# intel/pailliercryptolib

Measured on AMD Instinct MI355X. Metric: 2048-bit modexps/sec (encrypt+decrypt), higher is better.
Workload: dtype u64

## Files before the change

pailliercryptolib_amd/csrc/capi.cpp:

```cpp
#include "pgpu.h"

#include <hip/hip_runtime_api.h>

#include <algorithm>
#include <atomic>
#include <chrono>
#include <cstdio>
#include <cstdlib>
#include <cstring>
#include <deque>
#include <list>
#include <map>
#include <set>
#include <memory>
#include <mutex>
#include <string>
#include <vector>

#include "ipcl/bignum.h"
#include "kargs.hpp"
#include "launch.hpp"
#include "policy.hpp"
#include "runtime.hpp"

// ... 328 lines not shown
    const char* e = std::getenv("PGPU_FB_WINDOW");
    int v = e ? std::atoi(e) : kFbDefaultW;
    g_fb_window.store((v < 0 || v > kFbMaxW) ? kFbDefaultW : v);
    if (e) g_fb_window_explicit.store(true);
  }
  return g_fb_window.load();
}
int masked_fb_window() {
  static const int w = [] {
    const char* e = std::getenv("PGPU_FB_MASKED_WINDOW");
    return e ? std::max(1, std::min(kFbMaskedMaxW, std::atoi(e))) : 4;
  }();
  return w;
}
constexpr size_t kFbGrowAfter = 4096;

std::atomic<bool> g_timing{false};
struct TimerScope {
  rt::Device& d;
  hipStream_t s;
  bool on;
  rt::TimedLaunch t{};
  TimerScope(rt::Device& dev, hipStream_t st, int kind, int form = 0) : d(dev), s(st), on(g_timing.load()) {
    if (!on) return;
    t.kind = kind;
    t.form = form;
    t.stream = st;
    t.e0 = d.pool_event();
    t.e1 = d.pool_event();
    (void)hipEventRecord(t.e0, s);
  }
  void set_form(int form) { t.form = form; }
  void stop() {
    if (!on) return;
    (void)hipEventRecord(t.e1, s);
    std::lock_guard<std::mutex> lk(d.mu);
    if (d.timed.size() < 65536) d.timed.push_back(t);
  }
};

size_t modexp_waves(size_t count, int parity_waves, int ipw) {
  return parity_waves ? 2 * ((count / 2 + ipw - 1) / ipw) : (count + ipw - 1) / ipw;
}
unsigned blocks_for(size_t count, const GeoInfo& g) {
  return (unsigned)((count + (size_t)g.ipw() * pgpu::kWavesPerWG - 1) / ((size_t)g.ipw() * pgpu::kWavesPerWG));
}

GeoInfo latency_geo(const GeoInfo& geo) {
  static const bool allow = [] { const char* e = std::getenv("PGPU_LATENCY_GEO"); return !e || std::atoi(e) != 0; }();
  if (!allow) return geo;
  if (geo.G == 8 && geo.K == 9) return GeoInfo{16, 5};
  if (geo.G == 8 && geo.K == 14) return GeoInfo{16, 7};
  return geo;
}
bool use_latency_geo(const GeoInfo& lat, const GeoInfo& geo, size_t instances) {
  return lat.G != geo.G && (instances + lat.ipw() - 1) / lat.ipw() <= kSimds;
}

constexpr size_t kMinWavesForWide = 256 * 4;
GeoInfo launch_geo(const GeoInfo& geo, size_t count) {
  static const bool allow = [] { const char* e = std::getenv("PGPU_WIDE"); return !e || std::atoi(e) != 0; }();
  if (!allow || geo.K != 9 || geo.G < 4) return geo;
  GeoInfo wide{geo.G / 2, 18};
  size_t waves = (count + wide.ipw() - 1) / wide.ipw();
  static const size_t min_waves = [] {
    const char* e = std::getenv("PGPU_WIDE_MIN_WAVES");
    return e && std::atol(e) > 0 ? (size_t)std::atol(e) : kMinWavesForWide;
  }();
  return waves >= min_waves ? wide : geo;
}

std::atomic<int> g_row_source{-2};
bool use_regrows(const GeoInfo& geo, size_t waves) {
  int mode = g_row_source.load();
  if (mode == -2) {
    const char* e = std::getenv("PGPU_REGROWS");
    mode = e ? (std::atoi(e) != 0 ? 1 : 0) : -1;
    g_row_source.store(mode);
  }
  if (!pgpu::modexp_has_regrows(geo.G, geo.K)) return false;
  if (mode >= 0) return mode != 0;
  return waves <= kSimds;
}

uint64_t* g_wave_clocks = nullptr;

std::atomic<bool> g_packed_decrypt{[] {
  const char* e = std::getenv("PGPU_PACKED_DECRYPT");
  return !(e && std::atoi(e) == 0);
}()};
std::atomic<int> g_ct_gather{[] {
  const char* e = std::getenv("PGPU_CT_GATHER");
  return e && std::atoi(e) != 0 ? 1 : 0;
}()};
bool pair_rows_enabled() {
  static const bool on = [] {
    const char* e = std::getenv("PGPU_PAIR_ROWS");
    return !(e && std::atoi(e) == 0);
  }();
  return on;
}
std::atomic<int> g_hensel{-2};
bool hensel_enabled() {
  int mode = g_hensel.load();
  if (mode == -2) {
    const char* e = std::getenv("PGPU_HENSEL");
    mode = (e && std::atoi(e) == 0) ? 0 : 1;
    g_hensel.store(mode);
  }
  return mode != 0;
}

struct SchedRef {
  const uint16_t* p[2] = {nullptr, nullptr};
  int len[2] = {0, 0};
  int w = 0;
};
int run_modexp(rt::Device& d, pgpu::ModexpArgs& a, const GeoInfo& ctx_geo, hipStream_t s,
               const SchedRef* sched = nullptr, rt::StreamWork* held = nullptr) {
  const GeoInfo geo = launch_geo(ctx_geo, a.count);
  size_t entries;
  a.parity_waves = 0;
  if (sched && sched->p[0]) {
    a.parity_waves = a.nctx == 2;
    a.window = sched->w;
    for (int i = 0; i < 2; ++i) {
      a.sched[i] = sched->p[a.nctx == 2 ? i : 0];
      a.sched_len[i] = sched->len[a.nctx == 2 ? i : 0];
    }
    entries = (size_t)1 << (a.window - 1);
  } else {
    a.window = pick_window(a.exp_bits);
    entries = (size_t)1 << a.window;
  }
  const size_t waves = modexp_waves(a.count, a.parity_waves, geo.ipw());
  const size_t padded = (waves + pgpu::kWavesPerWG - 1) / pgpu::kWavesPerWG * pgpu::kWavesPerWG * geo.ipw();
  rt::StreamWork& w = held ? *held : d.work_for(s);
  std::unique_lock<std::mutex> lk(w.mu, std::defer_lock);
  if (!held) lk.lock();
  RC_TRY(w.table.ensure(padded * (entries + 1) * geo.L() * sizeof(uint32_t), s));
  a.table = (uint32_t*)w.table.p;
  a.wave_clocks = g_wave_clocks;
  TimerScope t(d, s, PGPU_KERNEL_MODEXP);
  const unsigned blocks = (unsigned)((waves + pgpu::kWavesPerWG - 1) / pgpu::kWavesPerWG);
  if (!pgpu::launch_modexp(geo.G, geo.K, use_regrows(geo, waves), a, blocks, s))
    return fail(PGPU_ERR_UNSUPPORTED, "modexp kernel geometry not compiled");
  HIP_TRY(hipGetLastError());
  t.stop();
  return PGPU_OK;
}

}

struct FbTable {
  void* p = nullptr;
  int w = 0, nwin = 0;
  hipEvent_t ready = nullptr;
  size_t bytes = 0;
  uint64_t tick = 0;
  int pins = 0;
  double build_ms = 0;
  hipEvent_t t0 = nullptr;
};
struct pgpu_pubkey {
  int n_words = 0;
  BigNumber n;
  bool djn = false;
  std::shared_ptr<ModCtx> nsq;
  rt::Replicated d_hs;
  rt::Replicated d_n;
  ExpSchedule sched_n;
  mutable std::mutex mu;
  mutable std::vector<std::list<FbTable>> fb;
  mutable size_t fb_elems = 0;
  struct PubForm {
    int H = 0, K = 0, chunk_words = 0, nchunks = 0;
    int n_words = 0;
    BigNumber n;
    rt::Replicated pub;
    rt::Replicated full;
    uint32_t n0inv = 0, n0inv_full = 0;
  };
  std::vector<std::shared_ptr<PubForm>> hforms;
  mutable std::vector<std::list<FbTable>> fbh;
  uint64_t gen = 0;
  ~pgpu_pubkey();
};

struct pgpu_privkey {
  uint64_t gen = 0;
  int n_words = 0;
  int pq_words = 0;
  GeoInfo geo_exp{};
  GeoInfo geo_crt{};
  std::shared_ptr<ModCtx> p2, q2;
  GeoInfo geo_lat{};
  std::shared_ptr<ModCtx> p2l, q2l;
  std::shared_ptr<ModCtx> cM, cQ;
  rt::Replicated d_exps;
  int exp_bits = 0;
  ExpSchedule sched[2];
  rt::Replicated d_crt32;
  rt::Replicated d_crt64;
  int nsq_rbits = 0;
  struct HenselSet {
    int H = 0, K = 0;
    int chunk_words = 0, nchunks = 0;
    rt::Replicated blob;
    uint32_t n0inv[2] = {0, 0};
    int pair_l2 = 0, pchunk_limbs = 0, pchunks = 0;
    int lb = pgpu::kLimbBits;
    size_t side_words() const { return (size_t)H * K * (6 + 4 * (size_t)nchunks + 3 * (size_t)pchunks); }
  };
  std::vector<std::unique_ptr<HenselSet>> hs;
  std::unique_ptr<HenselSet> hs_ps;
  std::shared_ptr<pgpu_pubkey::PubForm> conv_form;
};

struct pgpu_batch {
  size_t count = 0;
  int words = 0;
  int ndev = 1;
  bool replicated = false;
  std::vector<rt::DevMem> shard;
  std::shared_ptr<ModCtx> mont;
  int pair_l2 = 0;
  std::shared_ptr<const pgpu_pubkey::PubForm> pair_form;
  const uint32_t* prow(int d) const { return (const uint32_t*)shard[(size_t)d].p; }
  uint32_t* prow(int d) { return (uint32_t*)shard[(size_t)d].p; }
  uint64_t gen = 0;
  int lane = 0;
  uint64_t* ptr(int d) const { return (uint64_t*)shard[(size_t)d].p; }
  void bounds(int d, size_t* lo, size_t* hi) const {
    if (replicated) { *lo = 0; *hi = count; }
    else rt::shard_bounds(count, ndev, d, lo, hi);
  }
  struct XLane {
    hipEvent_t ready = nullptr;
    hipEvent_t reader[rt::kBatchLanes] = {};
  };
  mutable std::mutex xmu;
  mutable std::vector<XLane> xlane;
  ~pgpu_batch();
};

namespace {

std::atomic<int> g_next_thread_lane{0};
thread_local int t_batch_lane = -1;
thread_local bool t_lane_explicit = false;
std::atomic<int> g_host_adapt{[] { const char* e = std::getenv("PGPU_HOST_ADAPT"); return e && std::atoi(e) != 0 ? 1 : 0; }()};
bool host_adapt() { return g_host_adapt.load() != 0; }
int thread_batch_lane() {
  if (t_batch_lane < 0) t_batch_lane = g_next_thread_lane.fetch_add(1) % rt::kBatchLanes;
  return t_batch_lane;
}
int new_batch(size_t count, int words, std::unique_ptr<pgpu_batch>* out, int pair_l2 = 0, int lane = -1) {
  if (count == 0 || words <= 0) return fail(PGPU_ERR_INVALID_PARAM, "batch needs count > 0 and words > 0");
  std::unique_ptr<pgpu_batch> b(new pgpu_batch);
  b->count = count;
  b->words = words;
  b->gen = rt::pool_generation();
  b->lane = lane < 0 ? thread_batch_lane() : (lane % rt::kBatchLanes);
  b->replicated = count == 1 && rt::pool_size() > 1;
  b->ndev = b->replicated ? rt::pool_size() : rt::shard_devices(count);
  b->shard.resize((size_t)b->ndev);
  for (int d = 0; d < b->ndev; ++d) {
    size_t lo, hi;
    b->bounds(d, &lo, &hi);
    rt::Device& dev = rt::device(d);
    RC_TRY(b->shard[(size_t)d].alloc(dev, dev.bs(b->lane), (hi - lo) * (size_t)(pair_l2 ? pair_l2 : words) * 8));
  }
  b->pair_l2 = pair_l2;
  *out = std::move(b);
  return PGPU_OK;
}

bool same_domain(const std::shared_ptr<ModCtx>& batch_ctx, const std::shared_ptr<ModCtx>& key_ctx) {
  if (!batch_ctx || batch_ctx == key_ctx) return true;
  return batch_ctx->geo.L() == key_ctx->geo.L() && batch_ctx->geo.G == key_ctx->geo.G && batch_ctx->N == key_ctx->N;
}

int same_layout(const pgpu_batch* a, const pgpu_batch* b) {
  if (b->count == 1 && a->count != 1) return PGPU_OK;
  if (a->ndev != b->ndev || a->replicated != b->replicated)
    return fail(PGPU_ERR_INVALID_PARAM, "batches were sharded differently (pgpu_set_min_shard changed in between)");
  return PGPU_OK;
}

int lane_acquire(rt::Device& dev, const pgpu_batch* x, int lane) {
  if (!x || x->lane == lane) return PGPU_OK;
  hipEvent_t ready;
  {
    std::lock_guard<std::mutex> lk(x->xmu);
    if (x->xlane.size() < (size_t)rt::pool_size()) x->xlane.resize((size_t)rt::pool_size());
    pgpu_batch::XLane& xl = x->xlane[(size_t)dev.index];
    if (!xl.ready) {
      HIP_TRY(hipEventCreateWithFlags(&xl.ready, hipEventDisableTiming));
      HIP_TRY(hipEventRecord(xl.ready, dev.bs(x->lane)));
    }
    ready = xl.ready;
  }
  HIP_TRY(hipStreamWaitEvent(dev.bs(lane), ready, 0));
  return PGPU_OK;
}
int lane_release(rt::Device& dev, const pgpu_batch* x, int lane) {
  if (!x || x->lane == lane) return PGPU_OK;
  std::lock_guard<std::mutex> lk(x->xmu);
  if (x->xlane.size() < (size_t)rt::pool_size()) x->xlane.resize((size_t)rt::pool_size());
// ... 180 lines not shown
  a.chunk_words = f->chunk_words;
  a.nchunks = f->nchunks;
  a.exp = d_exp;
  a.exp_stride = exp_stride;
  a.exp_words = exp_words;
  a.exp_bits = exp_bits;
  size_t entries;
  if (sched && sched->p[0]) {
    a.sched = sched->p[0];
    a.sched_len = sched->len[0];
    a.window = sched->w;
    entries = (size_t)1 << (a.window - 1);
  } else {
    a.window = pick_window(exp_bits);
    entries = (size_t)1 << a.window;
  }
  a.final_mul = pgpu::FM_UNIT;
  a.ct_gather = (sched && sched->p[0]) ? 0 : g_ct_gather.load();
  a.out = d_out;
  a.out_stride = (size_t)sq.mod_words;
  a.count = count;
  const size_t ipw = 64 / (2 * (size_t)f->H);
  const size_t waves = (count + ipw - 1) / ipw;
  const unsigned blocks = (unsigned)((waves + pgpu::kWavesPerWG - 1) / pgpu::kWavesPerWG);
  rt::StreamWork& w = d.work_for(s);
  std::lock_guard<std::mutex> lk(w.mu);
  RC_TRY(w.table.ensure((size_t)blocks * pgpu::kWavesPerWG * ipw * entries * 2 * L2 * sizeof(uint32_t), s));
  a.table = (uint32_t*)w.table.p;
  TimerScope t(d, s, PGPU_KERNEL_MODEXP, PGPU_FORM_PAIRED);
  if (!pgpu::launch_hensel_modexp(f->H, f->K, a, blocks, s)) return fail(PGPU_ERR_UNSUPPORTED, "split-form modexp kernel not compiled");
  HIP_TRY(hipGetLastError());
  t.stop();
  return PGPU_OK;
}

int modexp_on(rt::Device& d, const uint64_t* d_base, size_t base_stride, const uint64_t* d_exp, size_t exp_stride,
              int exp_words, int exp_bits, const uint64_t* h_mod, int mod_words, uint64_t* d_out, size_t count,
              hipStream_t s, const SchedRef* sched, bool in_mont, bool out_mont, std::shared_ptr<ModCtx> ctx_in,
              size_t total_count = 0) {
  std::shared_ptr<ModCtx> ctx = ctx_in;
  if (!in_mont && !out_mont) {
    std::shared_ptr<SquareCtx> sq;
    RC_TRY(get_square_ctx(h_mod, mod_words, &sq));
    if (sq)
      return modexp_square_on(d, *sq, d_base, base_stride, d_exp, exp_stride, exp_words, exp_bits, d_out, count, s, sched,
                              std::max(count, total_count));
  }
  if (!ctx) RC_TRY(get_modctx(h_mod, mod_words, true, &ctx));
  GeoInfo run_geo = ctx->geo;
  const GeoInfo lat = latency_geo(ctx->geo);
  if (!in_mont && !out_mont && use_latency_geo(lat, ctx->geo, count)) {
    if (lat.L() != ctx->geo.L()) {
      std::vector<uint64_t> mw((size_t)mod_words);
      ctx->N.toLimbs64(mw.data(), mw.size());
      RC_TRY(get_modctx(mw.data(), mod_words, true, &ctx, true));
    }
    run_geo = lat;
  }
  pgpu::ModexpArgs a{};
  a.ctx[0] = a.ctx[1] = ctx->view(d.index, (in_mont ? VF_IN_MONT : 0) | (out_mont ? VF_OUT_MONT : 0));
  a.nctx = 1;
  a.base = d_base;
  a.base_stride = base_stride;
  a.base_words = mod_words;
  a.exp = d_exp;
  a.exp_stride = exp_stride;
  a.exp_per_ctx = 0;
  a.exp_words = exp_words;
  a.exp_bits = exp_bits;
  a.final_mul = out_mont ? pgpu::FM_CTX_CONST : pgpu::FM_UNIT;
  a.out = d_out;
  a.out_stride = (size_t)mod_words;
  a.count = count;
  return run_modexp(d, a, run_geo, s, sched);
}

std::mutex g_fb_mu;
std::set<const pgpu_pubkey*> g_fb_keys;
std::vector<size_t> g_fb_dev_bytes;
std::atomic<size_t> g_fb_dev_max{0}, g_fb_key_max{0};
std::atomic<uint64_t> g_fb_tick{0}, g_fb_evictions{0};
size_t fb_dev_max() {
  size_t v = g_fb_dev_max.load();
  if (v == 0) {
    const char* e = std::getenv("PGPU_FB_MAX_BYTES");
    v = e && std::atoll(e) > 0 ? (size_t)std::atoll(e) : (size_t)2 << 30;
    g_fb_dev_max.store(v);
  }
  return v;
}
size_t fb_key_max() {
  size_t v = g_fb_key_max.load();
  if (v == 0) {
    const char* e = std::getenv("PGPU_FB_KEY_MAX_BYTES");
    v = e && std::atoll(e) > 0 ? (size_t)std::atoll(e) : (size_t)512 << 20;
    g_fb_key_max.store(v);
  }
  return v;
}
size_t fb_table_bytes(int r_bits, int w, size_t entry_bytes) {
  return (size_t)std::max(1, (r_bits + w - 1) / w) * ((size_t)1 << w) * entry_bytes;
}
int fb_fit_window(int w_cfg, int r_bits, size_t entry_bytes) {
  int w = w_cfg;
  const size_t cap = std::min(fb_key_max(), fb_dev_max());
  while (w > 1 && fb_table_bytes(r_bits, w, entry_bytes) > cap) --w;
  return w;
}
void fb_free_table(FbTable& t) {
  if (t.ready) (void)hipEventDestroy(t.ready);
  if (t.t0) (void)hipEventDestroy(t.t0);
  if (t.p) (void)hipFree(t.p);
  t.p = nullptr;
}
void fb_make_room(int dev, size_t need) {
  if (g_fb_dev_bytes.size() <= (size_t)dev) g_fb_dev_bytes.resize((size_t)dev + 1, 0);
  while (g_fb_dev_bytes[(size_t)dev] + need > fb_dev_max()) {
    std::list<FbTable>* vlist = nullptr;
    std::list<FbTable>::iterator victim;
    for (const pgpu_pubkey* k : g_fb_keys)
      for (auto* lists : {&k->fb, &k->fbh}) {
        if (lists->size() <= (size_t)dev) continue;
        auto& l = (*lists)[(size_t)dev];
        for (auto it = l.begin(); it != l.end(); ++it)
          if (it->pins == 0 && (!vlist || it->tick < victim->tick)) {
            vlist = &l;
            victim = it;
          }
      }
    if (!vlist) return;
    g_fb_dev_bytes[(size_t)dev] -= std::min(g_fb_dev_bytes[(size_t)dev], victim->bytes);
    fb_free_table(*victim);
    vlist->erase(victim);
    g_fb_evictions.fetch_add(1);
  }
}
struct FbPin {
  FbTable* t = nullptr;
  FbPin() = default;
  FbPin(const FbPin&) = delete;
  FbPin& operator=(const FbPin&) = delete;
  ~FbPin() { release(); }
  void release() {
    if (!t) return;
    std::lock_guard<std::mutex> lk(g_fb_mu);
    --t->pins;
    t = nullptr;
  }
  const FbTable* operator->() const { return t; }
};

template <class Build>
int fb_table_get(const pgpu_pubkey* key, std::vector<std::list<FbTable>>& lists, rt::Device& d, int w, int nwin,
                 size_t entry_bytes, hipStream_t s, FbPin* out, Build build) {
  std::lock_guard<std::mutex> lk(g_fb_mu);
  if (lists.size() < (size_t)rt::pool_size()) lists.resize((size_t)rt::pool_size());
  auto& list = lists[(size_t)d.index];
  for (FbTable& t : list)
    if (t.w == w && t.nwin >= nwin) {
      HIP_TRY(hipStreamWaitEvent(s, t.ready, 0));
      t.tick = g_fb_tick.fetch_add(1) + 1;
      ++t.pins;
      out->t = &t;
      return PGPU_OK;
    }
  for (auto it = list.begin(); it != list.end();) {
    if (it->pins == 0 && (it->w <= kFbMaskedMaxW) == (w <= kFbMaskedMaxW)) {
      g_fb_dev_bytes.resize(std::max(g_fb_dev_bytes.size(), (size_t)d.index + 1), 0);
      g_fb_dev_bytes[(size_t)d.index] -= std::min(g_fb_dev_bytes[(size_t)d.index], it->bytes);
      fb_free_table(*it);
      it = list.erase(it);
    } else {
      ++it;
    }
  }
  FbTable t;
  t.w = w;
  t.nwin = nwin;
  t.bytes = (size_t)nwin * ((size_t)1 << w) * entry_bytes;
  fb_make_room(d.index, t.bytes);
  hipError_t e = hipMalloc(&t.p, t.bytes);
  if (e != hipSuccess) return fail(PGPU_ERR_HIP, std::string("fixed-base table: ") + hipGetErrorString(e));
  if (hipEventCreateWithFlags(&t.ready, hipEventDefault) != hipSuccess || hipEventCreateWithFlags(&t.t0, hipEventDefault) != hipSuccess) {
    fb_free_table(t);
    return fail(PGPU_ERR_HIP, "fixed-base table: event creation failed");
  }
  (void)hipEventRecord(t.t0, s);
  int rc = build(t);
  if (rc == PGPU_OK && hipGetLastError() != hipSuccess) rc = fail(PGPU_ERR_HIP, "fixed-base build launch failed");
  if (rc == PGPU_OK && hipEventRecord(t.ready, s) != hipSuccess) rc = fail(PGPU_ERR_HIP, "fixed-base table: event record failed");
  if (rc != PGPU_OK) {
    fb_free_table(t);
    return rc;
  }
  t.tick = g_fb_tick.fetch_add(1) + 1;
  t.pins = 1;
  g_fb_dev_bytes.resize(std::max(g_fb_dev_bytes.size(), (size_t)d.index + 1), 0);
  g_fb_dev_bytes[(size_t)d.index] += t.bytes;
  g_fb_keys.insert(key);
  list.push_back(t);
  out->t = &list.back();
  return PGPU_OK;
}

int fb_table_for(const pgpu_pubkey* key, rt::Device& d, int w, int nwin, hipStream_t s, FbPin* out) {
  const GeoInfo& geo = key->nsq->geo;
  return fb_table_get(key, key->fb, d, w, nwin, (size_t)geo.L() * sizeof(uint32_t), s, out, [&](FbTable& t) -> int {
    pgpu::FixedBaseBuildArgs b{};
    b.ctx = key->nsq->view(d.index);
    b.base = (const uint64_t*)key->d_hs.d[(size_t)d.index];
    b.table = (uint32_t*)t.p;
    b.nwin = nwin;
    b.w = w;
    if (!pgpu::launch_fb_build(geo.G, geo.K, b, blocks_for((size_t)nwin, geo), s))
      return fail(PGPU_ERR_UNSUPPORTED, "fixed-base build kernel geometry not compiled");
    return PGPU_OK;
  });
}

const pgpu_pubkey::PubForm* use_split_encrypt(const pgpu_pubkey* key, int m_words, size_t count) {
  if (key->hforms.empty() || !hensel_enabled() || 64 * m_words > key->n.BitSize()) return nullptr;
  const pgpu_pubkey::PubForm* f = key->hforms.back().get();
  if (!pgpu::hensel_fb_has(f->H, f->K)) return nullptr;
  if (g_hensel.load() >= 2) return f;
  const GeoInfo g = launch_geo(key->nsq->geo, count);
  const size_t ipw = 64 / (2 * (size_t)f->H);
  return (g.G <= 2 * f->H || (count + ipw - 1) / ipw >= kSimds) ? f : nullptr;
}
pgpu::HenselPubDev hensel_pub_view(const pgpu_pubkey::PubForm* f, int dev, bool base_mont = false) {
  const int L2 = f->H * f->K;
  const uint32_t* b = (const uint32_t*)f->pub.d[(size_t)dev];
  pgpu::HenselPubDev v{};
  v.nhat = b;
  v.n = b + L2;
  v.kr = b + 2 * L2;
  v.one = b + 3 * L2;
  v.conv = b + 5 * L2 + (base_mont ? (size_t)f->nchunks * 2 * L2 : 0);
  v.gm = b + (size_t)L2 * (5 + 4 * (size_t)f->nchunks);
  v.n0inv = f->n0inv;
  return v;
}
const pgpu_pubkey::PubForm* pair_form(const pgpu_pubkey* key) {
  if (key->hforms.empty() || !hensel_enabled() || !pair_rows_enabled()) return nullptr;
  const pgpu_pubkey::PubForm* f = key->hforms.back().get();
  return pgpu::pair_ops_has(f->H, f->K) ? f : nullptr;
}
int pair_l2(const pgpu_pubkey* key) {
  const pgpu_pubkey::PubForm* f = pair_form(key);
  return f ? f->H * f->K : 0;
}
std::shared_ptr<const pgpu_pubkey::PubForm> pair_form_shared(const pgpu_pubkey* key) {
  return pair_form(key) ? key->hforms.back() : nullptr;
}
pgpu::HenselFullDev hensel_full_view(const pgpu_pubkey* , const pgpu_pubkey::PubForm* f, int dev, bool out_mont) {
  const size_t LF = (size_t)2 * f->H * f->K;
  const uint32_t* b = (const uint32_t*)f->full.d[(size_t)dev];
  pgpu::HenselFullDev v{};
  v.n = b;
  v.nr = out_mont ? b + 2 * LF : b + LF;
  v.r2 = out_mont ? b + 3 * LF : nullptr;
  v.n0inv = f->n0inv_full;
  v.mod_words = 2 * f->n_words;
  return v;
}

const pgpu_pubkey::PubForm* split_modexp_form(const pgpu_pubkey* key, size_t count) {
  if (key->hforms.empty() || !hensel_enabled()) return nullptr;
  static const size_t max_waves = [] {
    const char* e = std::getenv("PGPU_SPLIT_MODEXP_MAX_WAVES");
    return e && std::atol(e) > 0 ? (size_t)std::atol(e) : ~(size_t)0;
  }();
  const pgpu_pubkey::PubForm* last = nullptr;
  for (const auto& f : key->hforms) {
    if (!pgpu::hensel_modexp_has(f->H, f->K)) continue;
    last = f.get();
    const size_t ipw = 64 / (2 * (size_t)f->H);
    if ((count + ipw - 1) / ipw <= kSimds) return last;
  }
  if (!last) return nullptr;
  const size_t ipw = 64 / (2 * (size_t)last->H);
  return (count + ipw - 1) / ipw > max_waves ? nullptr : last;
}
int wave_neighbours(rt::Device& dev, hipStream_t s) {
  int lane = -1;
  for (int k = 0; k < rt::kBatchLanes; ++k)
    if (dev.bs(k) == s) lane = k;
  if (lane < 0) return 0;
  static const int64_t window_ns = [] {
    const char* e = std::getenv("PGPU_LANE_ACTIVE_MS");
    return (int64_t)(e ? std::max(0, std::atoi(e)) : 50) * 1000000;
  }();
  const int64_t now = std::chrono::duration_cast<std::chrono::nanoseconds>(std::chrono::steady_clock::now().time_since_epoch()).count();
  dev.lane_fed_ns[lane].store(now, std::memory_order_relaxed);
  int busy = 0;
  for (int k = 0; k < rt::kBatchLanes; ++k) {
    if (k == lane) continue;
    const int64_t fed = std::max(dev.lane_fed_ns[k].load(std::memory_order_relaxed), dev.host_fed_ns[k].load(std::memory_order_relaxed));
    if ((fed != 0 && now - fed < window_ns) || hipStreamQuery(dev.bs(k)) == hipErrorNotReady) ++busy;
  }
  (void)hipGetLastError();
  return busy;
}
bool wave_n2_applies(const pgpu_pubkey::PubForm* form, size_t count) {
  const int L2 = form->H * form->K;
  return hensel_enabled() && pair_rows_enabled() && pgpu::hensel_modexp_wave_has(L2) && policy::modexp_wave_form_pays(count) &&
         pgpu::kLimbBits * L2 - (form->n.BitSize() + pgpu::kLimbBits) >= 10;
}
int modexp_split_on(rt::Device& d, const pgpu_pubkey* key, const pgpu_pubkey::PubForm* form, const uint64_t* d_base, size_t base_stride,
                    int base_words, bool base_mont, const uint64_t* d_exp, size_t exp_stride, int exp_words,
                    int exp_bits, const SchedRef* sched, int final_mul, const uint64_t* d_m, size_t m_stride,
                    int m_words, uint64_t* d_out, bool out_mont, size_t count, hipStream_t s,
                    const uint32_t* base_pair = nullptr, size_t base_pair_stride = 0, uint32_t* out_pair = nullptr) {
  const int H = form->H, K = form->K;
  pgpu::HenselModexpArgs a{};
  a.base_pair = base_pair;
  a.base_pair_stride = base_pair_stride;
  a.out_pair = out_pair;
  a.ctx = hensel_pub_view(form, d.index, base_mont);
  a.full = hensel_full_view(key, form, d.index, out_mont);
  a.base = d_base;
  a.base_stride = base_stride;
  a.base_words = base_words;
  a.chunk_words = form->chunk_words;
  a.nchunks = (base_words + form->chunk_words - 1) / form->chunk_words;
  a.exp = d_exp;
  a.exp_stride = exp_stride;
  a.exp_words = exp_words;
  a.exp_bits = exp_bits;
  size_t entries;
  if (sched && sched->p[0]) {
    a.sched = sched->p[0];
    a.sched_len = sched->len[0];
    a.window = sched->w;
    entries = (size_t)1 << (a.window - 1);
  } else {
    a.window = pick_window(exp_bits);
    entries = (size_t)1 << a.window;
  }
  a.final_mul = final_mul;
  a.ct_gather = (sched && sched->p[0]) ? 0 : g_ct_gather.load();
  a.fm_words = d_m;
  a.fm_stride = m_stride;
  a.fm_nwords = m_words;
  a.out = d_out;
  a.out_stride = (size_t)2 * key->n_words;
  a.count = count;
  if (base_pair && out_pair && !a.sched && final_mul == pgpu::FM_UNIT && wave_n2_applies(form, count) && a.window <= 5 &&
      (policy::wave_policy() == 2 || count * (size_t)(1 + wave_neighbours(d, s)) <= kSimds)) {
    TimerScope t(d, s, PGPU_KERNEL_MODEXP, PGPU_FORM_WAVE);
    if (!pgpu::launch_hensel_modexp_wave(H * K, a, s))
      return fail(PGPU_ERR_UNSUPPORTED, "wavefront-wide modexp kernel not compiled");
    HIP_TRY(hipGetLastError());
    t.stop();
    return PGPU_OK;
  }
  const bool seq = modexp_seq_form_pays(H, K, count) && base_pair && out_pair && !a.sched && final_mul == pgpu::FM_UNIT;
  const size_t ipw = seq ? 64 / (size_t)H : 64 / (2 * (size_t)H);
  const size_t waves = (count + ipw - 1) / ipw;
  const unsigned blocks = (unsigned)((waves + pgpu::kWavesPerWG - 1) / pgpu::kWavesPerWG);
  rt::StreamWork& w = d.work_for(s);
  std::lock_guard<std::mutex> lk(w.mu);
  RC_TRY(w.table.ensure((size_t)blocks * pgpu::kWavesPerWG * ipw * entries * 2 * H * K * sizeof(uint32_t), s));
  a.table = (uint32_t*)w.table.p;
  TimerScope t(d, s, PGPU_KERNEL_MODEXP, seq ? PGPU_FORM_SEQ : PGPU_FORM_PAIRED);
  if (seq) {
    if (!pgpu::launch_hensel_modexp_seq(H, K, a, blocks, s))
      return fail(PGPU_ERR_UNSUPPORTED, "sequential-halves modexp kernel not compiled");
  } else if (!pgpu::launch_hensel_modexp(H, K, a, blocks, s)) return fail(PGPU_ERR_UNSUPPORTED, "split-form modexp kernel not compiled");
  HIP_TRY(hipGetLastError());
  t.stop();
  return PGPU_OK;
}
int fb_table_for_split(const pgpu_pubkey* key, const pgpu_pubkey::PubForm* form, rt::Device& d, int w, int nwin,
                       hipStream_t s, FbPin* out) {
  const int H = form->H, K = form->K;
  return fb_table_get(key, key->fbh, d, w, nwin, (size_t)2 * H * K * sizeof(uint32_t), s, out, [&](FbTable& t) -> int {
    pgpu::HenselFbBuildArgs b{};
    b.ctx = hensel_pub_view(form, d.index);
    b.base = (const uint64_t*)key->d_hs.d[(size_t)d.index];
    b.base_words = 2 * key->n_words;
    b.chunk_words = form->chunk_words;
    b.nchunks = form->nchunks;
    b.table = (uint32_t*)t.p;
    b.nwin = nwin;
    b.w = w;
    const int ipw = 64 / (2 * H);
    const unsigned blocks = (unsigned)((((size_t)nwin + ipw - 1) / ipw + pgpu::kWavesPerWG - 1) / pgpu::kWavesPerWG);
    if (!pgpu::launch_hensel_fb_build(H, K, b, blocks, s))
      return fail(PGPU_ERR_UNSUPPORTED, "split-form fixed-base build kernel not compiled");
    return PGPU_OK;
  });
}

int encrypt_on(rt::Device& d, const pgpu_pubkey* key, const uint64_t* d_m, size_t m_stride, int m_words,
               const uint64_t* d_r, size_t r_stride, int r_words, int r_bits, uint64_t* d_c, size_t count,
               hipStream_t s, bool out_mont, size_t total_count, uint32_t* d_pair = nullptr, int busy_lanes = 0) {
  const int W = 2 * key->n_words;
  if (m_words <= 0 || m_words > W || m_stride < (size_t)m_words)
    return fail(PGPU_ERR_INVALID_PARAM, "plaintext width/stride invalid");
  if (r_words <= 0 || r_stride < (size_t)r_words)
    return fail(PGPU_ERR_INVALID_PARAM, "random width/stride invalid");
  if (key->djn && (r_bits < 0 || r_bits > 64 * r_words))
    return fail(PGPU_ERR_INVALID_PARAM, "r_bits/r_words inconsistent");
  const int vflags = out_mont ? VF_GM_MONT : VF_NONE;
  int fbw = fixed_base_window();
  const bool masked = key->djn && fbw > 0 && g_ct_gather.load() != 0;
  if (masked) fbw = masked_fb_window();
  if (key->djn && fbw > 0) {
    if (!masked) {
      std::lock_guard<std::mutex> lk(key->mu);
      if (fbw > 8 && !g_fb_window_explicit.load() && key->fb_elems + total_count < kFbGrowAfter) fbw = 8;
    }
    const GeoInfo& geo = key->nsq->geo;
    const pgpu_pubkey::PubForm* sform = d_pair ? pair_form(key) : use_split_encrypt(key, m_words, count);
    fbw = fb_fit_window(fbw, r_bits, sform ? (size_t)2 * sform->H * sform->K * sizeof(uint32_t) : (size_t)geo.L() * sizeof(uint32_t));
    const int nwin = std::max(1, (r_bits + fbw - 1) / fbw);
    FbPin tab;
    if (const pgpu_pubkey::PubForm* form = sform) {
      RC_TRY(fb_table_for_split(key, form, d, fbw, nwin, s, &tab));
      if (d_pair) {
        for (const auto& alt : key->hforms) {
          const size_t ipw_alt = 64 / (2 * (size_t)alt->H);
          if (alt->H * alt->K == form->H * form->K && alt->H > form->H && pgpu::hensel_fb_encrypt_has(alt->H, alt->K) &&
              (total_count + ipw_alt - 1) / ipw_alt <= kSimds) {
            form = alt.get();
            break;
          }
        }
      }
      pgpu::HenselFbArgs f{};
      f.ctx = hensel_pub_view(form, d.index);
      f.full = hensel_full_view(key, form, d.index, out_mont);
      f.table = (const uint32_t*)tab->p;
      f.nwin = nwin;
      f.w = fbw;
      f.exp = d_r;
      f.exp_stride = r_stride;
      f.exp_words = r_words;
      f.fm_words = d_m;
      f.fm_stride = m_stride;
      f.fm_nwords = m_words;
      f.out = d_c;
      f.out_stride = (size_t)W;
      f.count = count;
      f.out_pair = d_pair;
      f.ct_gather = masked ? 1 : 0;
      TimerScope t(d, s, PGPU_KERNEL_FB_ENCRYPT);
      if (d_pair && busy_lanes == 0 && wave_n2_applies(form, count) &&
          (policy::wave_policy() == 2 || count * (size_t)(1 + wave_neighbours(d, s)) <= kSimds)) {
        t.set_form(PGPU_FORM_WAVE);
        if (!pgpu::launch_hensel_fb_encrypt_wave(form->H * form->K, f, s))
          return fail(PGPU_ERR_UNSUPPORTED, "wavefront-wide fixed-base kernel not compiled");
        HIP_TRY(hipGetLastError());
        t.stop();
        return PGPU_OK;
      }
      const bool seq = d_pair && fb_encrypt_seq_pays(form->H, form->K, count, busy_lanes);
      t.set_form(seq ? PGPU_FORM_SEQ : PGPU_FORM_PAIRED);
      const int ipw = seq ? 64 / form->H : 64 / (2 * form->H);
      const unsigned blocks = (unsigned)(((count + ipw - 1) / ipw + pgpu::kWavesPerWG - 1) / pgpu::kWavesPerWG);
      if (seq) {
        const size_t seq_waves = (count + ipw - 1) / ipw;
        unsigned lds_pad = adaptive_cu_claim(seq_waves, busy_lanes);
        if (lds_pad && busy_lanes >= 3) lds_pad = pgpu::kLdsTotalFlag | 80000u;
        if (lds_pad) t.set_form(PGPU_FORM_SEQ | PGPU_FORM_CU_CLAIM);
        if (!pgpu::launch_hensel_fb_encrypt_seq(form->H, form->K, f, blocks, s, lds_pad))
          return fail(PGPU_ERR_UNSUPPORTED, "sequential-halves fixed-base kernel not compiled");
      } else if (!pgpu::launch_hensel_fb_encrypt(form->H, form->K, f, blocks, s))
        return fail(PGPU_ERR_UNSUPPORTED, "split-form fixed-base kernel not compiled");
      HIP_TRY(hipGetLastError());
      t.stop();
      return PGPU_OK;
    }
    RC_TRY(fb_table_for(key, d, fbw, nwin, s, &tab));
    pgpu::FixedBaseArgs f{};
    f.ctx = key->nsq->view(d.index, vflags);
    f.table = (const uint32_t*)tab->p;
    f.nwin = nwin;
    f.w = fbw;
    f.exp = d_r;
    f.exp_stride = r_stride;
    f.exp_words = r_words;
    f.fm_words = d_m;
    f.fm_stride = m_stride;
    f.fm_nwords = m_words;
    f.out = d_c;
    f.out_stride = (size_t)W;
    f.count = count;
    f.ct_gather = masked ? 1 : 0;
    TimerScope t(d, s, PGPU_KERNEL_FB_ENCRYPT);
    const GeoInfo lgeo = launch_geo(geo, count);
    if (!pgpu::launch_fb_encrypt(lgeo.G, lgeo.K, f, blocks_for(count, lgeo), s))
      return fail(PGPU_ERR_UNSUPPORTED, "fixed-base kernel geometry not compiled");
    HIP_TRY(hipGetLastError());
    t.stop();
    return PGPU_OK;
  }
  pgpu::ModexpArgs a{};
  a.ctx[0] = a.ctx[1] = key->nsq->view(d.index, vflags);
  a.nctx = 1;
  if (key->djn) {
    a.base = (const uint64_t*)key->d_hs.d[(size_t)d.index];
    a.base_stride = 0;
    a.base_words = W;
    a.exp = d_r;
    a.exp_stride = r_stride;
    a.exp_words = r_words;
    a.exp_bits = r_bits;
  } else {
    if (r_words > W) return fail(PGPU_ERR_INVALID_PARAM, "random wider than n^2");
    const pgpu_pubkey::PubForm* form = d_pair ? pair_form(key)
                                       : (64 * m_words <= key->n.BitSize() ? split_modexp_form(key, count) : nullptr);
    if (form) {
      SchedRef srn;
      if (key->sched_n.dev.bytes) {
        srn.p[0] = (const uint16_t*)key->sched_n.dev.d[(size_t)d.index];
        srn.len[0] = key->sched_n.len;
        srn.w = key->sched_n.w;
      }
      return modexp_split_on(d, key, form, d_r, r_stride, r_words, false,
                             (const uint64_t*)key->d_n.d[(size_t)d.index], 0, key->n_words, key->n.BitSize(),
                             srn.p[0] ? &srn : nullptr, pgpu::FM_PAILLIER_G, d_m, m_stride, m_words, d_c, out_mont,
                             count, s, nullptr, 0, d_pair);
    }
    a.base = d_r;
    a.base_stride = r_stride;
    a.base_words = r_words;
    a.exp = (const uint64_t*)key->d_n.d[(size_t)d.index];
    a.exp_stride = 0;
    a.exp_words = key->n_words;
    a.exp_bits = key->n.BitSize();
  }
  if (d_pair) return fail(PGPU_ERR_UNSUPPORTED, "pair-row output needs a split-form encrypt kernel");
  a.exp_per_ctx = 0;
  a.final_mul = pgpu::FM_PAILLIER_G;
  a.fm_words = d_m;
  a.fm_stride = m_stride;
  a.fm_nwords = m_words;
  a.out = d_c;
  a.out_stride = (size_t)W;
  a.count = count;
  SchedRef sr;
  if (!key->djn && key->sched_n.dev.bytes) {
    sr.p[0] = (const uint16_t*)key->sched_n.dev.d[(size_t)d.index];
    sr.len[0] = key->sched_n.len;
    sr.w = key->sched_n.w;
  }
  return run_modexp(d, a, key->nsq->geo, s, sr.p[0] ? &sr : nullptr);
}

const pgpu_privkey::HenselSet* pick_hensel(const pgpu_privkey* key, size_t count) {
  if (!hensel_enabled() || key->hs.empty()) return nullptr;
  const int mode = g_hensel.load();
  if (mode == 2) return key->hs.back().get();
  if (mode == 3) return key->hs.front().get();
  for (const auto& f : key->hs) {
    const size_t ipw = 64 / (2 * (size_t)f->H);
    if (2 * ((count + ipw - 1) / ipw) <= kSimds) return f.get();
  }
  return key->hs.back().get();
}

int busy_other_lanes(rt::Device& dev, int lane, bool force = false, size_t count = (size_t)-1) {
  const int rr_min = (!force && !t_lane_explicit) ? policy::rr_adapt() : 1;
  if (rr_min <= 0) return 0;
  static const int64_t window_ns = [] {
    const char* e = std::getenv("PGPU_LANE_ACTIVE_MS");
    return (int64_t)(e ? std::max(0, std::atoi(e)) : 50) * 1000000;
  }();
  const int64_t now = std::chrono::duration_cast<std::chrono::nanoseconds>(std::chrono::steady_clock::now().time_since_epoch()).count();
  dev.lane_fed_ns[lane % rt::kBatchLanes].store(now, std::memory_order_relaxed);
  int busy = 0;
  for (int k = 0; k < rt::kBatchLanes; ++k) {
    if (k == lane) continue;
    const int64_t fed = dev.lane_fed_ns[k].load(std::memory_order_relaxed);
    if ((fed != 0 && now - fed < window_ns) || hipStreamQuery(dev.bs(k)) == hipErrorNotReady) ++busy;
  }
  (void)hipGetLastError();
  if (!force && !t_lane_explicit && count < policy::kRrAdaptMinCount) return 0;
  return busy >= rr_min ? busy : 0;
}
int host_busy(rt::Device& dev, int lane, size_t count = (size_t)-1) {
  if (host_adapt()) return busy_other_lanes(dev, lane, true);
  const int k = policy::rr_adapt();
  if (k <= 0) return 0;
  static const int64_t window_ns = [] {
    const char* e = std::getenv("PGPU_LANE_ACTIVE_MS");
    return (int64_t)(e ? std::max(0, std::atoi(e)) : 50) * 1000000;
  }();
  const int64_t now = std::chrono::duration_cast<std::chrono::nanoseconds>(std::chrono::steady_clock::now().time_since_epoch()).count();
  dev.host_fed_ns[lane % rt::kBatchLanes].store(now, std::memory_order_relaxed);
  int busy = 0;
  for (int j = 0; j < rt::kBatchLanes; ++j) {
    if (j == lane % rt::kBatchLanes) continue;
    const int64_t fed = std::max(dev.host_fed_ns[j].load(std::memory_order_relaxed), dev.lane_fed_ns[j].load(std::memory_order_relaxed));
    if (fed != 0 && now - fed < window_ns) ++busy;
  }
  if (count < policy::kRrAdaptMinCount) return 0;
  return busy >= k ? busy : 0;
}

bool ps_form_pays(const pgpu_privkey* key, size_t count, int busy) {
  return key->hs_ps && hensel_enabled() && policy::ps_form_pays(count, busy, key->hs_ps->K);
}
bool wave_form_pays(const pgpu_privkey* key, size_t count, int busy) {
  return key->hs_ps && hensel_enabled() && pgpu::hensel_wave_has(key->hs_ps->K, key->hs_ps->lb) && policy::wave_form_pays(count, busy);
}
int words_to_pair_on(rt::Device& d, const pgpu_pubkey::PubForm* f, const uint64_t* words, size_t stride, int nwords,
                     bool src_mont, uint32_t* out, size_t count, hipStream_t s);
int decrypt_on(rt::Device& d, const pgpu_privkey* key, const uint64_t* d_c, uint64_t* d_m, size_t count,
               hipStream_t s, bool in_mont, const uint32_t* d_pair = nullptr, int in_pair_l2 = 0, int busy_lanes = 0) {
  const int nw = key->n_words;
  if (busy_lanes == 0 && key->hs_ps && hensel_enabled() && secret_policy() != PGPU_EXP_SLIDING &&
      (d_pair ? key->hs_ps->pair_l2 == in_pair_l2 : key->conv_form != nullptr)) {
    if (const size_t head = policy::ps_split_head(key->hs_ps->K, count)) {
      RC_TRY(decrypt_on(d, key, d_c, d_m, head, s, in_mont, d_pair, in_pair_l2, busy_lanes));
      return decrypt_on(d, key, d_c ? d_c + head * (size_t)2 * nw : nullptr, d_m + head * (size_t)nw, count - head, s, in_mont,
                        d_pair ? d_pair + head * (size_t)2 * in_pair_l2 : nullptr, in_pair_l2, busy_lanes);
    }
  }
  rt::StreamWork& w = d.work_for(s);
  std::lock_guard<std::mutex> lk(w.mu);
  RC_TRY(w.vbuf.ensure(2 * count * (size_t)nw * 8, s));
  const bool lat = use_latency_geo(key->geo_lat, key->geo_exp, 2 * count);
  const bool sliding = secret_policy() == PGPU_EXP_SLIDING && key->sched[0].dev.bytes;
  bool have_m = false;
  const pgpu_privkey::HenselSet* hset = pick_hensel(key, count);
// ... 917 lines not shown
```

pailliercryptolib_amd/csrc/hensel.hpp:

```cpp
#ifndef PAILLIERCRYPTOLIB_AMD_CSRC_HENSEL_HPP_
#define PAILLIERCRYPTOLIB_AMD_CSRC_HENSEL_HPP_

#include "kernels.hpp"

namespace pgpu {

template <int H, int K>
__device__ __forceinline__ void pair_row_source(uint32_t (&src)[K], const uint32_t (&v)[K]) {
#pragma unroll
  for (int j = 0; j < K; ++j) {
    if constexpr (H == 4)
      src[j] = (uint32_t)__builtin_amdgcn_update_dpp((int)v[j], (int)v[j], 0x114 , 0xf, 0xa, false);
    else
      src[j] = v[j];
  }
}
template <int H, int S>
__device__ __forceinline__ uint32_t pair_row(uint32_t src) {
  if constexpr (H == 8) return bcast_lane<16, S>(src);
  else return bcast_lane<4, S>(src);
}

template <int H, int K, bool SQR, bool UNITQ, int S>
__device__ __forceinline__ void pair_block(uint64_t (&LOWC)[K], uint64_t (&UPC)[K], const uint32_t (&mc)[K],
                                           const uint32_t (&md)[K], const uint32_t (&csrc)[K],
                                           const uint32_t (&asrc)[K], const uint32_t (&n)[K], uint32_t n0inv,
                                           uint32_t selB) {
  using GEO = Geo<H, K>;
  uint32_t crow[K];
#pragma unroll
  for (int r = 0; r < K; ++r) crow[r] = pair_row<H, S>(csrc[r]);
#pragma unroll
  for (int r = 0; r < K; ++r) {
#pragma unroll
    for (int j = 0; j < K; ++j) {
      const uint64_t p = (uint64_t)mc[j] * crow[r];
      if (r + j < K) LOWC[r + j] += p;
      else UPC[r + j - K] += p;
    }
  }
  if constexpr (!SQR) {
    uint32_t arow[K];
#pragma unroll
    for (int r = 0; r < K; ++r) arow[r] = pair_row<H, S>(asrc[r]);
#pragma unroll
    for (int r = 0; r < K; ++r) {
#pragma unroll
      for (int j = 0; j < K; ++j) {
        const uint64_t p = (uint64_t)md[j] * arow[r];
        if (r + j < K) LOWC[r + j] += p;
        else UPC[r + j - K] += p;
      }
    }
  }
  mont_reduce_rows<GEO, UNITQ, true, true>(LOWC, UPC, n, n0inv, selB);
}

template <int H, int K, bool SQR, bool UNITQ, int S>
__device__ __forceinline__ void pair_blocks(uint64_t (&c0)[K], uint64_t (&c1)[K], const uint32_t (&mc)[K],
                                            const uint32_t (&md)[K], const uint32_t (&csrc)[K],
                                            const uint32_t (&asrc)[K], const uint32_t (&n)[K], uint32_t n0inv,
                                            uint32_t selB) {
  if constexpr (S < H) {
    pair_block<H, K, SQR, UNITQ, S>(c0, c1, mc, md, csrc, asrc, n, n0inv, selB);
    pair_block<H, K, SQR, UNITQ, S + 1>(c1, c0, mc, md, csrc, asrc, n, n0inv, selB);
    pair_blocks<H, K, SQR, UNITQ, S + 2>(c0, c1, mc, md, csrc, asrc, n, n0inv, selB);
  }
}
template <int H, int K, bool SQR, bool UNITQ>
__device__ __forceinline__ void pairmul(uint32_t (&r)[K], const uint32_t (&own)[K], const uint32_t (&m)[K],
                                        const uint32_t (&n)[K], uint32_t n0inv, uint32_t halfB, uint32_t selB) {
  static_assert(3 * K + 6 < 64, "a column of half B receives 3K products (+ relaxed limbs): must stay below 2^64");
  static_assert(H == 2 || H == 4 || H == 8, "two halves inside one 16-lane DPP row");
  using GEO = Geo<H, K>;
  uint64_t c0[K], c1[K];
  uint32_t mc[K], md[K], csrc[K], asrc[K];
  const uint32_t maskB = 0u - halfB;
  pair_row_source<H, K>(asrc, own);
  if constexpr (!SQR) pair_row_source<H, K>(csrc, m);
#pragma unroll
  for (int j = 0; j < K; ++j) {
    c0[j] = 0;
    c1[j] = 0;
    mc[j] = SQR ? own[j] << halfB : own[j];
    md[j] = SQR ? 0 : m[j] & maskB;
  }
  if constexpr (SQR) pair_blocks<H, K, SQR, UNITQ, 0>(c0, c1, mc, md, asrc, asrc, n, n0inv, selB);
  else pair_blocks<H, K, SQR, UNITQ, 0>(c0, c1, mc, md, csrc, asrc, n, n0inv, selB);
  montmul_finish<GEO>(r, c0);
}

template <class GEO>
__device__ __forceinline__ uint32_t sub_limbs(uint32_t (&d)[GEO::K], const uint32_t (&r)[GEO::K],
                                              const uint32_t (&s)[GEO::K], int x, int lane) {
  constexpr int K = GEO::K, G = GEO::G;
  const int top_lane = (lane / G) * G + (G - 1);
  uint32_t b = 0;
#pragma unroll
  for (int j = 0; j < K; ++j) {
    uint32_t t = r[j] - s[j] - b;
    d[j] = t & kLimbMask;
    b = t >> 31;
  }
  uint32_t top_borrow = b;
  for (;;) {
    uint32_t bin = dpp_from_prev(b);
    if (x == 0) bin = 0;
    if (__ballot(bin != 0) == 0) break;
    b = bin;
#pragma unroll
    for (int j = 0; j < K; ++j) {
      uint32_t t = d[j] - b;
      d[j] = t & kLimbMask;
      b = t >> 31;
    }
    top_borrow |= b;
  }
  return (uint32_t)__shfl((int)top_borrow, top_lane);
}

template <int H, int K, int MINW = (K <= 14 ? 2 : 1)>
__global__ __launch_bounds__(kWGThreads, MINW) void hensel_decrypt_kernel(HenselArgs A) {
  using HG = Geo<H, K>;
  constexpr int GS = 2 * H, IPW = kWave / GS, L2 = H * K, LQ = 2 * H * K, W64 = HG::W64;
  raise_wave_priority();
  __shared__ uint32_t bl_[kWavesPerWG][IPW][L2];
  __shared__ uint64_t io_[kWavesPerWG][IPW][W64 + 1];
  const int lane = threadIdx.x % kWave, wv = threadIdx.x / kWave;
  auto& bl = bl_[wv];
  auto& io = io_[wv];
  const int grp = lane / GS, xg = lane % GS, x = xg % H;
  const uint32_t halfB = (uint32_t)(xg / H);
  uint32_t selB = xg == H ? 1u : 0u;
  asm("" : "+v"(selB));
  const size_t wave_id = (size_t)blockIdx.x * kWavesPerWG + wv;
  const int side = __builtin_amdgcn_readfirstlane((int)(wave_id & 1));
  const size_t first_elem = (wave_id >> 1) * IPW;
  size_t elem = first_elem + grp;
  if (elem >= A.count) elem = A.count - 1;
#define HCTX(field) (side ? A.ctx[1].field : A.ctx[0].field)

  uint32_t n[K], own[K], mreg[K];
#pragma unroll
  for (int j = 0; j < K; ++j) n[j] = HCTX(nhat)[x * K + j];
  uint32_t n0inv = 0;

  const bool sched_mode = A.sched[0] != nullptr;
  const uint16_t* sch = side ? A.sched[1] : A.sched[0];
  const int nsteps = side ? A.sched_len[1] : A.sched_len[0];
  const int w = A.window;
  const int tsize = sched_mode ? 1 << (w - 1) : 1 << w;
  uint32_t* tbl = A.table + (wave_id * IPW + grp) * (size_t)tsize * LQ + xg * K;
  const uint64_t* ep = A.exp + (size_t)side * A.exp_stride;
  const int nwin = (A.exp_bits + w - 1) / w;
  auto digit = [&](int i) -> int {
    int bit = i * w;
    int word = bit >> 6, sh = bit & 63;
    uint64_t v = (word < A.exp_words) ? ep[word] >> sh : 0;
    if (sh + w > 64 && word + 1 < A.exp_words) v |= ep[word + 1] << (64 - sh);
    return (int)(v & (uint64_t)(tsize - 1));
  };

  uint32_t acc[K];
#pragma unroll
  for (int j = 0; j < K; ++j) acc[j] = 0;
  if (A.ct_pair) {
    const uint32_t* row = A.ct_pair + elem * A.ct_pair_stride + (size_t)halfB * A.pair_l2;
    const uint32_t* pconv = HCTX(pconv);
    const uint32_t* pcb = HCTX(pcb);
    const int trips = A.pchunks + ((sched_mode && tsize > 1) ? 1 : 0);
#pragma unroll 1
    for (int i = 0; i < trips; ++i) {
      if (i < A.pchunks) {
        const int first = i * A.pchunk_limbs;
        uint32_t z[K], cb[K], tb[K];
#pragma unroll
        for (int j = 0; j < K; ++j) {
          const int li = x * K + j;
          z[j] = (li < A.pchunk_limbs && first + li < A.pair_l2) ? row[first + li] : 0u;
          cb[j] = pcb[(size_t)i * L2 + x * K + j];
          mreg[j] = pconv[(size_t)i * LQ + xg * K + j];
          own[j] = halfB ? 0u : z[j];
        }
        montmul_reg<HG, false, true>(tb, z, cb, n, 0);
        pairmul<H, K, false, true>(own, own, mreg, n, n0inv, halfB, selB);
#pragma unroll
        for (int j = 0; j < K; ++j) own[j] += halfB ? tb[j] : 0u;
        add_normalise<HG>(acc, own);
      } else {
#pragma unroll
        for (int j = 0; j < K; ++j) own[j] = mreg[j] = acc[j];
        pairmul<H, K, false, true>(own, own, mreg, n, n0inv, halfB, selB);
      }
    }
  } else {
    const uint64_t* row = A.ct + elem * A.ct_stride;
    const uint32_t* conv = HCTX(conv);
    const int trips = A.nchunks + ((sched_mode && tsize > 1) ? 1 : 0);
#pragma unroll 1
    for (int i = 0; i < trips; ++i) {
      if (i < A.nchunks) {
        wave_lds_sync();
        const int first = i * A.chunk_words;
        const int words = min(A.chunk_words, A.ct_words - first);
        for (int t = xg; t <= W64; t += GS) io[grp][t] = (t < words) ? row[first + t] : 0;
        wave_lds_sync();
#pragma unroll
        for (int j = 0; j < K; ++j) {
          own[j] = halfB ? 0u : limb_from_words(io[grp], x * K + j);
          mreg[j] = conv[(size_t)i * LQ + xg * K + j];
        }
      } else {
#pragma unroll
        for (int j = 0; j < K; ++j) own[j] = mreg[j] = acc[j];
      }
      pairmul<H, K, false, true>(own, own, mreg, n, n0inv, halfB, selB);
      if (i < A.nchunks) add_normalise<HG>(acc, own);
    }
  }

  {
    int e;
    if (sched_mode) {
#pragma unroll
      for (int j = 0; j < K; ++j) {
        tbl[j] = acc[j];
        mreg[j] = own[j];
        own[j] = acc[j];
      }
      e = 1;
    } else {
#pragma unroll
      for (int j = 0; j < K; ++j) {
        tbl[LQ + j] = acc[j];
        tbl[j] = HCTX(one)[xg * K + j];
        mreg[j] = own[j] = acc[j];
      }
      e = 2;
    }
#pragma unroll 1
    for (; e < tsize; ++e) {
      pairmul<H, K, false, true>(own, own, mreg, n, n0inv, halfB, selB);
#pragma unroll
      for (int j = 0; j < K; ++j) tbl[(size_t)e * LQ + j] = own[j];
    }
  }

  int win;
  bool any = true;
  if (sched_mode) {
    if (nsteps == 0) any = false;
    win = 1;
  } else {
    if (nwin == 0) any = false;
    win = nwin - 2;
  }
  if (any) {
    const int d0 = sched_mode ? (__builtin_amdgcn_readfirstlane((int)sch[0]) & 63) - 1 : digit(nwin - 1);
    load_table_entry<K>(own, tbl, d0, tsize, LQ, A.ct_gather != 0);
  } else {
#pragma unroll
    for (int j = 0; j < K; ++j) own[j] = HCTX(one)[xg * K + j];
  }
#ifndef PGPU_PHASE_PAD
#define PGPU_PHASE_PAD 0
#endif
  if constexpr ((PGPU_PHASE_PAD & 2) != 0) asm volatile(".p2align 6");
  if constexpr ((PGPU_PHASE_PAD & 1) != 0) asm volatile("s_nop 0");
#pragma unroll 1
  for (;;) {
    int nsq, idx;
    if (sched_mode) {
      if (!any || win >= nsteps) break;
      const int st = __builtin_amdgcn_readfirstlane((int)sch[win++]);
      nsq = st >> 6;
      idx = (st & 63) - 1;
    } else {
      if (!any || win < 0) break;
      nsq = w;
      idx = digit(win--);
    }
    const bool mul = !sched_mode || idx >= 0;
    if (mul) load_table_entry<K>(mreg, tbl, idx, tsize, LQ, A.ct_gather != 0);
#pragma unroll 1
    for (int i = 0; i < nsq; ++i) pairmul<H, K, true, true>(own, own, own, n, n0inv, halfB, selB);
    if (mul) pairmul<H, K, false, true>(own, own, mreg, n, n0inv, halfB, selB);
  }

  {
#pragma unroll
    for (int j = 0; j < K; ++j) {
      n[j] = HCTX(n)[x * K + j];
      mreg[j] = HCTX(kr)[x * K + j];
    }
    n0inv = HCTX(n0inv);
    uint32_t kb[K];
    montmul_reg<HG, false, false>(kb, own, mreg, n, n0inv);
#pragma unroll
    for (int j = 0; j < K; ++j) {
      if (halfB) own[j] = kb[j];
      mreg[j] = halfB ? 0u : HCTX(h)[x * K + j];
    }
    pairmul<H, K, false, false>(own, own, mreg, n, n0inv, halfB, selB);
  }
  full_normalise<HG>(own, x);
  uint32_t d[K];
  const uint32_t below = sub_limbs<HG>(d, own, n, x, lane);
  const uint32_t jflag = (uint32_t)__shfl((int)(below ^ 1u), (lane / GS) * GS);
  if (!below) {
#pragma unroll
    for (int j = 0; j < K; ++j) own[j] = d[j];
  }
  (void)sub_limbs<HG>(d, n, own, x, lane);
  if (x == 0) d[0] += jflag;
  full_normalise<HG>(d, x);
  const uint32_t small = sub_limbs<HG>(own, d, n, x, lane);
  if (small) {
#pragma unroll
    for (int j = 0; j < K; ++j) own[j] = d[j];
  }
  wave_lds_sync();
  if (halfB) {
#pragma unroll
    for (int j = 0; j < K; ++j) bl[grp][x * K + j] = own[j];
  }
  wave_lds_sync();
  const int ow = A.out_words;
  for (int t = lane; t < IPW * ow; t += kWave) {
    const int gg = t / ow, ww = t % ow;
    const size_t oe = first_elem + gg;
    if (oe < A.count) A.out[(2 * oe + side) * A.out_stride + ww] = ww < W64 ? word_from_limbs(bl[gg], L2, ww) : 0;
  }
#undef HCTX
}

template <int D>
__device__ __forceinline__ uint32_t dpp_from_above(uint32_t v) {
  return (uint32_t)__builtin_amdgcn_update_dpp(0, (int)v, 0x100 + D , 0xf, 0xf, true);
}

template <int K>
__device__ __forceinline__ void load_pair_row(uint32_t (&v)[K], const uint32_t* __restrict__ row, int xg) {
  const uint32_t* p = row + xg * K;
  if constexpr (K % 2 == 0) {
    const uint2* q = reinterpret_cast<const uint2*>(p);
#pragma unroll
    for (int j = 0; j < K / 2; ++j) {
      const uint2 t = q[j];
      v[2 * j] = t.x;
      v[2 * j + 1] = t.y;
    }
  } else {
#pragma unroll
    for (int j = 0; j < K; ++j) v[j] = p[j];
  }
}
template <int K>
__device__ __forceinline__ void store_pair_row(uint32_t* __restrict__ row, const uint32_t (&v)[K], int xg) {
  uint32_t* p = row + xg * K;
  if constexpr (K % 2 == 0) {
    uint2* q = reinterpret_cast<uint2*>(p);
#pragma unroll
    for (int j = 0; j < K / 2; ++j) q[j] = make_uint2(v[2 * j], v[2 * j + 1]);
  } else {
#pragma unroll
    for (int j = 0; j < K; ++j) p[j] = v[j];
  }
}

template <int H, int K>
__device__ __forceinline__ void pair_times_gm(uint32_t (&own)[K], const HenselPubDev& C, const uint64_t* mwords, int x,
                                              uint32_t halfB) {
  using HG = Geo<H, K>;
  uint32_t n[K], mv[K], cg[K], u[K], av[K], v[K];
#pragma unroll
  for (int j = 0; j < K; ++j) {
    n[j] = C.n[x * K + j];
    cg[j] = C.gm[x * K + j];
    mv[j] = limb_from_words(mwords, x * K + j);
  }
  montmul_reg<HG, false, false>(u, mv, cg, n, C.n0inv);
#pragma unroll
  for (int j = 0; j < K; ++j) {
    const uint32_t below = dpp_from_below<H>(own[j]);
    av[j] = halfB ? below : own[j];
  }
  montmul_reg<HG, false, false>(v, u, av, n, C.n0inv);
#pragma unroll
  for (int j = 0; j < K; ++j) v[j] = halfB ? v[j] : 0u;
  add_normalise<HG>(own, v);
}

template <int H, int K>
__device__ __forceinline__ void pair_from_words(uint32_t (&own)[K], const uint64_t* row, int nwords, int chunk_words,
                                                int nchunks, const uint32_t* conv, uint64_t* iorow,
                                                const uint32_t (&n)[K], uint32_t halfB, uint32_t selB, int xg) {
  using HG = Geo<H, K>;
  constexpr int GS = 2 * H, LQ = 2 * H * K, W64 = HG::W64;
  const int x = xg % H;
  uint32_t acc[K], mreg[K];
#pragma unroll
  for (int j = 0; j < K; ++j) acc[j] = 0;
#pragma unroll 1
  for (int i = 0; i < nchunks; ++i) {
    wave_lds_sync();
    const int first = i * chunk_words;
    const int words = min(chunk_words, nwords - first);
    for (int t = xg; t <= W64; t += GS) iorow[t] = (t < words) ? row[first + t] : 0;
    wave_lds_sync();
#pragma unroll
    for (int j = 0; j < K; ++j) {
      own[j] = halfB ? 0u : limb_from_words(iorow, x * K + j);
      mreg[j] = conv[(size_t)i * LQ + xg * K + j];
    }
    pairmul<H, K, false, true>(own, own, mreg, n, 0, halfB, selB);
    add_normalise<HG>(acc, own);
  }
#pragma unroll
  for (int j = 0; j < K; ++j) own[j] = acc[j];
}

template <int H, int K>
__device__ __forceinline__ void pair_exit_store(uint32_t (&own)[K], const HenselPubDev& C, const HenselFullDev& F,
                                                bool with_gm, const uint64_t* fm_words, size_t fm_stride, int fm_nwords,
                                                uint64_t* out, size_t out_stride, size_t first_inst, size_t count,
                                                uint32_t (*bl)[2 * H * K], uint64_t (*io)[Geo<2 * H, K>::W64 + 1],
                                                uint32_t (*rows)[2 * H * K], int lane, int grp, int xg, uint32_t halfB,
                                                uint32_t selB) {
  using HG = Geo<H, K>;
  using FG = Geo<2 * H, K>;
  constexpr int GS = 2 * H;
  const int x = xg % H;
  for (int t = lane; t < FG::L; t += kWave) {
    rows[0][t] = F.nr[t];
    rows[1][t] = F.r2 ? F.r2[t] : 0;
  }
  if (with_gm) stage_words<FG>(io, fm_words, fm_stride, 0, fm_nwords, first_inst, count, 1, lane);
  uint32_t n[K], mreg[K];
#pragma unroll
  for (int j = 0; j < K; ++j) {
    n[j] = C.n[x * K + j];
    mreg[j] = C.kr[x * K + j];
  }
  const uint32_t n0inv = C.n0inv;
  {
    uint32_t kb[K];
    montmul_reg<HG, false, false>(kb, own, mreg, n, n0inv);
#pragma unroll
    for (int j = 0; j < K; ++j)
      if (halfB) own[j] = kb[j];
  }
  wave_lds_sync();
  uint32_t d[K], e[K];
  if (with_gm) {
#pragma unroll
    for (int j = 0; j < K; ++j) {
      e[j] = limb_from_words(io[grp], x * K + j);
      d[j] = 2 * n[j];
    }
    full_normalise<HG>(d, x);
    (void)sub_limbs<HG>(mreg, d, e, x, lane);
  } else {
#pragma unroll
    for (int j = 0; j < K; ++j) mreg[j] = 0;
  }
#pragma unroll
  for (int j = 0; j < K; ++j)
    if (!halfB) mreg[j] = (xg == 0 && j == 0) ? 1u : 0u;
  pairmul<H, K, false, false>(own, own, mreg, n, n0inv, halfB, selB);
  full_normalise<HG>(own, x);
  const uint32_t below = sub_limbs<HG>(d, own, n, x, lane);
  const uint32_t jflag = (uint32_t)__shfl((int)(below ^ 1u), (lane / GS) * GS);
  if (!below) {
#pragma unroll
    for (int j = 0; j < K; ++j) own[j] = d[j];
  }
  (void)sub_limbs<HG>(d, n, own, x, lane);
  if (x == 0) d[0] += jflag;
  full_normalise<HG>(d, x);
  const uint32_t small = sub_limbs<HG>(e, d, n, x, lane);
  uint32_t X[K], Y[K], nf[K];
#pragma unroll
  for (int j = 0; j < K; ++j) {
    const uint32_t bc = small ? d[j] : e[j];
    const uint32_t down = dpp_from_above<H>(bc);
    X[j] = halfB ? 0u : own[j];
    Y[j] = halfB ? 0u : down;
    nf[j] = F.n[xg * K + j];
  }
  wave_lds_sync();
  uint32_t t[K];
  montmul<FG, false, false>(t, Y, rows[0], nf, F.n0inv);
  if (F.r2) {
    uint32_t u[K];
    montmul<FG, false, false>(u, X, rows[1], nf, F.n0inv);
    add_normalise<FG>(t, u);
  } else {
    add_normalise<FG>(t, X);
  }
  store_canonical<FG>(t, nf, F.mod_words, bl, io, out, out_stride, first_inst, count, lane, grp, xg);
}

template <int H, int K>
__global__ __launch_bounds__(kWGThreads, K <= 14 ? 2 : 1) void hensel_fb_build_kernel(HenselFbBuildArgs A) {
  using HG = Geo<H, K>;
  constexpr int GS = 2 * H, IPW = kWave / GS, LQ = 2 * H * K, W64 = HG::W64;
  __shared__ uint64_t io_[kWavesPerWG][IPW][W64 + 1];
  const int lane = threadIdx.x % kWave, wv = threadIdx.x / kWave;
  auto& io = io_[wv];
  const int grp = lane / GS, xg = lane % GS, x = xg % H;
  const uint32_t halfB = (uint32_t)(xg / H);
  uint32_t selB = xg == H ? 1u : 0u;
  asm("" : "+v"(selB));
  const size_t first_inst = ((size_t)blockIdx.x * kWavesPerWG + wv) * IPW;
  size_t inst = first_inst + grp;
  const bool live = inst < (size_t)A.nwin;
  if (!live) inst = (size_t)A.nwin - 1;
  uint32_t n[K], own[K], mreg[K];
#pragma unroll
  for (int j = 0; j < K; ++j) n[j] = A.ctx.nhat[x * K + j];
  pair_from_words<H, K>(own, A.base, A.base_words, A.chunk_words, A.nchunks, A.ctx.conv, io[grp], n, halfB, selB, xg);
  const int tsize = 1 << A.w;
  const int my_sq = A.w * (int)inst;
  size_t last = first_inst + IPW - 1;
  if (last >= (size_t)A.nwin) last = (size_t)A.nwin - 1;
  const int wave_sq = A.w * (int)last;
#pragma unroll 1
  for (int step = 1; step <= wave_sq; ++step) {
    uint32_t r[K];
    pairmul<H, K, true, true>(r, own, own, n, 0, halfB, selB);
    if (step <= my_sq) {
#pragma unroll
      for (int j = 0; j < K; ++j) own[j] = r[j];
    }
  }
  uint32_t* row = A.table + inst * (size_t)tsize * LQ + xg * K;
  if (live) {
#pragma unroll
    for (int j = 0; j < K; ++j) {
      row[j] = A.ctx.one[xg * K + j];
      row[LQ + j] = own[j];
    }
  }
#pragma unroll
  for (int j = 0; j < K; ++j) mreg[j] = own[j];
#pragma unroll 1
  for (int d = 2; d < tsize; ++d) {
    pairmul<H, K, false, true>(own, own, mreg, n, 0, halfB, selB);
    if (live) {
#pragma unroll
      for (int j = 0; j < K; ++j) row[(size_t)d * LQ + j] = own[j];
    }
  }
}

template <int H, int K>
__global__ __launch_bounds__(kWGThreads, K <= 14 ? 2 : 1) void hensel_fb_encrypt_kernel(HenselFbArgs A) {
  using HG = Geo<H, K>;
  using FG = Geo<2 * H, K>;
  constexpr int GS = 2 * H, IPW = kWave / GS, LQ = 2 * H * K;
  raise_wave_priority();
  __shared__ uint32_t bl_[kWavesPerWG][IPW][FG::L];
  __shared__ uint64_t io_[kWavesPerWG][IPW][FG::W64 + 1];
  __shared__ uint32_t rows_[kWavesPerWG][2][FG::L];
  const int lane = threadIdx.x % kWave, wv = threadIdx.x / kWave;
  auto& bl = bl_[wv];
  auto& io = io_[wv];
  auto& rows = rows_[wv];
  const int grp = lane / GS, xg = lane % GS, x = xg % H;
  const uint32_t halfB = (uint32_t)(xg / H);
  uint32_t selB = xg == H ? 1u : 0u;
  asm("" : "+v"(selB));
  const size_t first_inst = ((size_t)blockIdx.x * kWavesPerWG + wv) * IPW;
  size_t inst = first_inst + grp;
  if (inst >= A.count) inst = A.count - 1;
  uint32_t n[K], own[K], mreg[K], nxt[K];
#pragma unroll
  for (int j = 0; j < K; ++j) n[j] = A.ctx.nhat[x * K + j];
  const int w = A.w, tsize = 1 << w;
  const uint64_t* ep = A.exp + inst * A.exp_stride;
  auto digit = [&](int i) -> int {
    int bit = i * w;
    int word = bit >> 6, sh = bit & 63;
    uint64_t v = (word < A.exp_words) ? ep[word] >> sh : 0;
    if (sh + w > 64 && word + 1 < A.exp_words) v |= ep[word + 1] << (64 - sh);
    return (int)(v & (uint64_t)(tsize - 1));
  };
  auto load_entry = [&](uint32_t (&dst)[K], int i) {
    load_table_entry<K>(dst, A.table + (size_t)i * tsize * LQ + xg * K, digit(i), tsize, LQ, A.ct_gather != 0);
  };
  load_entry(own, 0);
  if (A.nwin > 1) load_entry(mreg, 1);
#pragma unroll 1
  for (int i = 1; i < A.nwin; ++i) {
    if (i + 1 < A.nwin) load_entry(nxt, i + 1);
    pairmul<H, K, false, true>(own, own, mreg, n, 0, halfB, selB);
#pragma unroll
    for (int j = 0; j < K; ++j) mreg[j] = nxt[j];
  }
  if (A.out_pair) {
    stage_words<FG>(io, A.fm_words, A.fm_stride, 0, A.fm_nwords, first_inst, A.count, 1, lane);
    wave_lds_sync();
    pair_times_gm<H, K>(own, A.ctx, io[grp], x, halfB);
    if (first_inst + grp < A.count) store_pair_row<K>(A.out_pair + inst * (size_t)LQ, own, xg);
    return;
  }
  pair_exit_store<H, K>(own, A.ctx, A.full, true, A.fm_words, A.fm_stride, A.fm_nwords, A.out, A.out_stride, first_inst,
                        A.count, bl, io, rows, lane, grp, xg, halfB, selB);
}

#ifndef PGPU_HM_WAVES18
#define PGPU_HM_WAVES18 2
#endif
template <int H, int K>
__global__ __launch_bounds__(kWGThreads, K <= 14 ? 2 : PGPU_HM_WAVES18) void hensel_modexp_kernel(HenselModexpArgs A) {
  using HG = Geo<H, K>;
  using FG = Geo<2 * H, K>;
  constexpr int GS = 2 * H, IPW = kWave / GS, LQ = 2 * H * K;
  raise_wave_priority();
  __shared__ uint32_t bl_[kWavesPerWG][IPW][FG::L];
  __shared__ uint64_t io_[kWavesPerWG][IPW][FG::W64 + 1];
  __shared__ uint32_t rows_[kWavesPerWG][2][FG::L];
  const int lane = threadIdx.x % kWave, wv = threadIdx.x / kWave;
  auto& bl = bl_[wv];
  auto& io = io_[wv];
  auto& rows = rows_[wv];
  const int grp = lane / GS, xg = lane % GS, x = xg % H;
  const uint32_t halfB = (uint32_t)(xg / H);
  uint32_t selB = xg == H ? 1u : 0u;
  asm("" : "+v"(selB));
  const size_t wave_id = (size_t)blockIdx.x * kWavesPerWG + wv;
  const size_t first_inst = wave_id * IPW;
  size_t inst = first_inst + grp;
  if (inst >= A.count) inst = A.count - 1;
  uint32_t n[K], own[K], mreg[K];
#pragma unroll
  for (int j = 0; j < K; ++j) n[j] = A.ctx.nhat[x * K + j];

  const bool sched_mode = A.sched != nullptr;
  const uint16_t* sch = A.sched;
  const int nsteps = A.sched_len;
  const int w = A.window;
  const int tsize = sched_mode ? 1 << (w - 1) : 1 << w;
  uint32_t* tbl = A.table + (wave_id * IPW + grp) * (size_t)tsize * LQ + xg * K;
  const uint64_t* ep = A.exp + inst * A.exp_stride;
  const int nwin = (A.exp_bits + w - 1) / w;
  auto digit = [&](int i) -> int {
    int bit = i * w;
    int word = bit >> 6, sh = bit & 63;
    uint64_t v = (word < A.exp_words) ? ep[word] >> sh : 0;
    if (sh + w > 64 && word + 1 < A.exp_words) v |= ep[word + 1] << (64 - sh);
    return (int)(v & (uint64_t)(tsize - 1));
  };

  if (A.base_pair) load_pair_row<K>(own, A.base_pair + inst * A.base_pair_stride, xg);
  else pair_from_words<H, K>(own, A.base + inst * A.base_stride, A.base_words, A.chunk_words, A.nchunks, A.ctx.conv,
                             io[grp], n, halfB, selB, xg);
  {
    int e;
    if (sched_mode) {
#pragma unroll
      for (int j = 0; j < K; ++j) tbl[j] = own[j];
      if (tsize > 1) pairmul<H, K, false, true>(mreg, own, own, n, 0, halfB, selB);
      e = 1;
    } else {
#pragma unroll
      for (int j = 0; j < K; ++j) {
        tbl[LQ + j] = own[j];
        tbl[j] = A.ctx.one[xg * K + j];
        mreg[j] = own[j];
      }
      e = 2;
    }
#pragma unroll 1
    for (; e < tsize; ++e) {
      pairmul<H, K, false, true>(own, own, mreg, n, 0, halfB, selB);
#pragma unroll
      for (int j = 0; j < K; ++j) tbl[(size_t)e * LQ + j] = own[j];
    }
  }
  int win;
  bool any = true;
  if (sched_mode) {
    if (nsteps == 0) any = false;
    win = 1;
  } else {
    if (nwin == 0) any = false;
    win = nwin - 2;
  }
  if (any) {
    const int d0 = sched_mode ? (__builtin_amdgcn_readfirstlane((int)sch[0]) & 63) - 1 : digit(nwin - 1);
    load_table_entry<K>(own, tbl, d0, tsize, LQ, A.ct_gather != 0);
  } else {
#pragma unroll
    for (int j = 0; j < K; ++j) own[j] = A.ctx.one[xg * K + j];
  }
#pragma unroll 1
  for (;;) {
    int nsq, idx;
    if (sched_mode) {
      if (!any || win >= nsteps) break;
      const int st = __builtin_amdgcn_readfirstlane((int)sch[win++]);
      nsq = st >> 6;
      idx = (st & 63) - 1;
    } else {
      if (!any || win < 0) break;
      nsq = w;
      idx = digit(win--);
    }
    const bool mul = !sched_mode || idx >= 0;
    if (mul) load_table_entry<K>(mreg, tbl, idx, tsize, LQ, A.ct_gather != 0);
#pragma unroll 1
    for (int i = 0; i < nsq; ++i) pairmul<H, K, true, true>(own, own, own, n, 0, halfB, selB);
    if (mul) pairmul<H, K, false, true>(own, own, mreg, n, 0, halfB, selB);
  }
  if (A.out_pair) {
    if (A.final_mul == FM_PAILLIER_G) {
      wave_lds_sync();
      stage_words<FG>(io, A.fm_words, A.fm_stride, 0, A.fm_nwords, first_inst, A.count, 1, lane);
      wave_lds_sync();
      pair_times_gm<H, K>(own, A.ctx, io[grp], xg % H, halfB);
    }
    if (first_inst + grp < A.count) store_pair_row<K>(A.out_pair + inst * (size_t)LQ, own, xg);
    return;
  }
  pair_exit_store<H, K>(own, A.ctx, A.full, A.final_mul == FM_PAILLIER_G, A.fm_words, A.fm_stride, A.fm_nwords, A.out,
                        A.out_stride, first_inst, A.count, bl, io, rows, lane, grp, xg, halfB, selB);
}

template <int H, int K>
__global__ __launch_bounds__(kWGThreads, 2) void pair_ops_kernel(PairOpsArgs A) {
  using HG = Geo<H, K>;
  using FG = Geo<2 * H, K>;
  constexpr int GS = 2 * H, IPW = kWave / GS, LQ = 2 * H * K;
  raise_wave_priority();
  __shared__ uint32_t bl_[kWavesPerWG][IPW][FG::L];
  __shared__ uint64_t io_[kWavesPerWG][IPW][FG::W64 + 1];
  __shared__ uint32_t rows_[kWavesPerWG][2][FG::L];
  const int lane = threadIdx.x % kWave, wv = threadIdx.x / kWave;
  auto& bl = bl_[wv];
  auto& io = io_[wv];
  auto& rows = rows_[wv];
  const int grp = lane / GS, xg = lane % GS, x = xg % H;
  const uint32_t halfB = (uint32_t)(xg / H);
  uint32_t selB = xg == H ? 1u : 0u;
  asm("" : "+v"(selB));
  const size_t first_inst = ((size_t)blockIdx.x * kWavesPerWG + wv) * IPW;
  size_t inst = first_inst + grp;
  const bool live = inst < A.count;
  if (!live) inst = A.count - 1;
  uint32_t own[K];
  if (A.op == PO_MUL) {
    uint32_t n[K], mreg[K];
    load_pair_row<K>(own, A.a + inst * (size_t)LQ, xg);
    load_pair_row<K>(mreg, A.b + inst * A.b_stride, xg);
#pragma unroll
    for (int j = 0; j < K; ++j) n[j] = A.ctx.nhat[x * K + j];
    pairmul<H, K, false, true>(own, own, mreg, n, 0, halfB, selB);
    if (live) store_pair_row<K>(A.out + inst * (size_t)LQ, own, xg);
  } else if (A.op == PO_TIMES_GM) {
    load_pair_row<K>(own, A.a + inst * (size_t)LQ, xg);
// ... 22 lines not shown
```

pailliercryptolib_amd/csrc/hensel_seq.hpp:

```cpp
#ifndef PAILLIERCRYPTOLIB_AMD_CSRC_HENSEL_SEQ_HPP_
#define PAILLIERCRYPTOLIB_AMD_CSRC_HENSEL_SEQ_HPP_

#include "hensel_q.hpp"

namespace pgpu {

template <int G, int K, bool SQR, bool UNITQ, int S, bool QLDS = false>
__device__ __forceinline__ void seq_a_blocks(uint64_t (&c0)[K], uint64_t (&c1)[K], const uint32_t (&a)[K],
                                             const uint32_t (&a2)[K], const uint32_t (&n)[K], uint32_t n0inv,
                                             const uint32_t (&m)[K], uint32_t (&qd)[QLDS ? 1 : G][K], uint32_t* qs = nullptr) {
  using HG = Geo<G, K>;
  if constexpr (S < G) {
    uint32_t b[K];
#pragma unroll
    for (int r = 0; r < K; ++r) b[r] = bcast_lane<G, S>(m[r]);
#pragma unroll
    for (int r = 0; r < K; ++r) {
#pragma unroll
      for (int j = 0; j < K; ++j) {
        uint64_t p;
        if constexpr (SQR) {
          if (j > r) continue;
          p = (uint64_t)(j < r ? a2[j] : a[j]) * b[r];
        } else {
          p = (uint64_t)a[j] * b[r];
        }
        if (r + j < K) c0[r + j] += p;
        else c1[r + j - K] += p;
      }
    }
    if constexpr (QLDS) {
      uint32_t qrec[K];
      mont_reduce_rows_q<HG, UNITQ, 1>(c0, c1, n, n0inv, qrec, 0u);
      ab_store20<K>(qs + S * kAbPad, qrec);
    } else {
      mont_reduce_rows_q<HG, UNITQ, 1>(c0, c1, n, n0inv, qd[S], 0u);
    }
    seq_a_blocks<G, K, SQR, UNITQ, S + 1, QLDS>(c1, c0, a, a2, n, n0inv, m, qd, qs);
  }
}

template <int G, int K, bool SQR, bool UNITQ, int S, bool QLDS = false>
__device__ __forceinline__ void seq_b_blocks(uint64_t (&c0)[K], uint64_t (&c1)[K], const uint32_t (&mc)[K],
                                             const uint32_t (&md)[K], const uint32_t (&a)[K], const uint32_t (&c)[K],
                                             const uint32_t (&n)[K], uint32_t n0inv, uint32_t (&qd)[QLDS ? 1 : G][K],
                                             uint32_t sel0, const uint32_t* qs = nullptr) {
  using HG = Geo<G, K>;
  if constexpr (S < G) {
    uint32_t row[K];
#pragma unroll
    for (int r = 0; r < K; ++r) row[r] = bcast_lane<G, S>(SQR ? a[r] : c[r]);
#pragma unroll
    for (int r = 0; r < K; ++r) {
#pragma unroll
      for (int j = 0; j < K; ++j) {
        const uint64_t p = (uint64_t)mc[j] * row[r];
        if (r + j < K) c0[r + j] += p;
        else c1[r + j - K] += p;
      }
    }
    if constexpr (!SQR) {
#pragma unroll
      for (int r = 0; r < K; ++r) row[r] = bcast_lane<G, S>(a[r]);
#pragma unroll
      for (int r = 0; r < K; ++r) {
#pragma unroll
        for (int j = 0; j < K; ++j) {
          const uint64_t p = (uint64_t)md[j] * row[r];
          if (r + j < K) c0[r + j] += p;
          else c1[r + j - K] += p;
        }
      }
    }
    if constexpr (QLDS) {
      uint32_t qin[K];
      ab_load20<K>(qin, qs + S * kAbPad);
      mont_reduce_rows_q<HG, UNITQ, 2>(c0, c1, n, n0inv, qin, sel0);
    } else {
      mont_reduce_rows_q<HG, UNITQ, 2>(c0, c1, n, n0inv, qd[S], sel0);
    }
    seq_b_blocks<G, K, SQR, UNITQ, S + 1, QLDS>(c1, c0, mc, md, a, c, n, n0inv, qd, sel0, qs);
  }
}

template <int G, int K, bool SQR, bool UNITQ, bool QLDS = false>
__device__ __forceinline__ void seq_pairmul(uint32_t (&a)[K], uint32_t (&b)[K], const uint32_t (&c)[K],
                                            const uint32_t (&d)[K], const uint32_t (&n)[K], uint32_t n0inv, uint32_t sel0,
                                            uint32_t* qs = nullptr, uint32_t* ts = nullptr) {
  static_assert(3 * K + 6 < 64, "a column receives 3K products (+ relaxed limbs): must stay below 2^64");
  static_assert(G % 2 == 0, "blocks alternate between the two accumulator sets and end in the first");
  using HG = Geo<G, K>;
  uint32_t qd[QLDS ? 1 : G][K];
  uint32_t t[K];
  {
    uint64_t c0[K], c1[K];
    uint32_t a2[K];
#pragma unroll
    for (int j = 0; j < K; ++j) {
      c0[j] = 0;
      c1[j] = 0;
      a2[j] = SQR ? a[j] << 1 : 0;
    }
    seq_a_blocks<G, K, SQR, UNITQ, 0, QLDS>(c0, c1, a, a2, n, n0inv, c, qd, qs);
    montmul_finish<HG>(t, c0);
    if constexpr (QLDS) {
      if (ts) ab_store20<K>(ts, t);
    }
  }
  {
    uint64_t c0[K], c1[K];
    uint32_t mc[K], md[K];
#pragma unroll
    for (int j = 0; j < K; ++j) {
      c0[j] = 0;
      c1[j] = 0;
      mc[j] = SQR ? b[j] << 1 : b[j];
      md[j] = SQR ? 0u : d[j];
    }
    seq_b_blocks<G, K, SQR, UNITQ, 0, QLDS>(c0, c1, mc, md, a, c, n, n0inv, qd, sel0, qs);
    montmul_finish<HG>(b, c0);
  }
  if constexpr (QLDS) {
    if (ts) {
      ab_load20<K>(a, ts);
      return;
    }
  }
#pragma unroll
  for (int j = 0; j < K; ++j) a[j] = t[j];
}

template <int G, int K, int MINW = 2>
__global__ __launch_bounds__(kWGThreads, MINW) void hensel_decrypt_seq_kernel(HenselArgs A) {
  using HG = Geo<G, K>;
  constexpr int IPW = kWave / G, L2 = G * K, LQ = 2 * L2, W64 = HG::W64;
  raise_wave_priority();
  __shared__ uint32_t bl_[kWavesPerWG][IPW][L2];
  const int lane = threadIdx.x % kWave, wv = threadIdx.x / kWave;
  auto& bl = bl_[wv];
  const int grp = lane / G, x = lane % G;
  uint32_t sel0 = x == 0 ? 1u : 0u;
  asm("" : "+v"(sel0));
  const size_t wave_id = (size_t)blockIdx.x * kWavesPerWG + wv;
  const int side = __builtin_amdgcn_readfirstlane((int)(wave_id & 1));
  const size_t first_elem = (wave_id >> 1) * IPW;
  size_t elem = first_elem + grp;
  if (elem >= A.count) elem = A.count - 1;
#define HCTX(field) (side ? A.ctx[1].field : A.ctx[0].field)
  uint32_t n[K], a[K], b[K], ma[K], mb[K];
#pragma unroll
  for (int j = 0; j < K; ++j) n[j] = HCTX(nhat)[x * K + j];
  const int w = A.window, tsize = 1 << w;
  uint32_t* tbl = A.table + (wave_id * IPW + grp) * (size_t)tsize * LQ + x * K;
  const uint64_t* ep = A.exp + (size_t)side * A.exp_stride;
  const int nwin = (A.exp_bits + w - 1) / w;
  auto digit = [&](int i) -> int {
    int bit = i * w;
    int word = bit >> 6, sh = bit & 63;
    uint64_t v = (word < A.exp_words) ? ep[word] >> sh : 0;
    if (sh + w > 64 && word + 1 < A.exp_words) v |= ep[word + 1] << (64 - sh);
    return (int)(v & (uint64_t)(tsize - 1));
  };
  const bool gather = A.ct_gather != 0;

  {
    const uint32_t* row = A.ct_pair + elem * A.ct_pair_stride;
    uint32_t acc_a[K], acc_b[K];
#pragma unroll
    for (int j = 0; j < K; ++j) acc_a[j] = acc_b[j] = 0;
#pragma unroll 1
    for (int i = 0; i < A.pchunks; ++i) {
      const int first = i * A.pchunk_limbs;
      uint32_t zb[K], cb[K], tb[K];
#pragma unroll
      for (int j = 0; j < K; ++j) {
        const int li = x * K + j;
        const bool in = li < A.pchunk_limbs && first + li < A.pair_l2;
        a[j] = in ? row[first + li] : 0u;
        zb[j] = in ? row[A.pair_l2 + first + li] : 0u;
        b[j] = 0;
        cb[j] = HCTX(pcb)[(size_t)i * L2 + x * K + j];
        ma[j] = HCTX(pconv)[(size_t)i * LQ + x * K + j];
        mb[j] = HCTX(pconv)[(size_t)i * LQ + L2 + x * K + j];
      }
      montmul_reg<HG, false, true>(tb, zb, cb, n, 0);
      seq_pairmul<G, K, false, true>(a, b, ma, mb, n, 0, sel0);
#pragma unroll
      for (int j = 0; j < K; ++j) b[j] += tb[j];
      add_normalise<HG>(acc_a, a);
      add_normalise<HG>(acc_b, b);
    }
#pragma unroll
    for (int j = 0; j < K; ++j) {
      a[j] = ma[j] = acc_a[j];
      b[j] = mb[j] = acc_b[j];
    }
  }
#pragma unroll
  for (int j = 0; j < K; ++j) {
    tbl[(size_t)LQ + j] = a[j];
    tbl[(size_t)LQ + L2 + j] = b[j];
    tbl[j] = HCTX(one)[x * K + j];
    tbl[L2 + j] = HCTX(one)[L2 + x * K + j];
  }
#pragma unroll 1
  for (int e = 2; e < tsize; ++e) {
    seq_pairmul<G, K, false, true>(a, b, ma, mb, n, 0, sel0);
#pragma unroll
    for (int j = 0; j < K; ++j) {
      tbl[(size_t)e * LQ + j] = a[j];
      tbl[(size_t)e * LQ + L2 + j] = b[j];
    }
  }
  int win = nwin - 2;
  if (nwin > 0) {
    const int d0 = digit(nwin - 1);
    load_table_entry<K>(a, tbl, d0, tsize, LQ, gather);
    load_table_entry<K>(b, tbl + L2, d0, tsize, LQ, gather);
  } else {
#pragma unroll
    for (int j = 0; j < K; ++j) {
      a[j] = HCTX(one)[x * K + j];
      b[j] = HCTX(one)[L2 + x * K + j];
    }
  }
#pragma unroll 1
  for (; nwin > 0 && win >= 0; --win) {
    const int idx = digit(win);
    load_table_entry<K>(ma, tbl, idx, tsize, LQ, gather);
    load_table_entry<K>(mb, tbl + L2, idx, tsize, LQ, gather);
#pragma unroll 1
    for (int i = 0; i < w; ++i) seq_pairmul<G, K, true, true>(a, b, a, b, n, 0, sel0);
    seq_pairmul<G, K, false, true>(a, b, ma, mb, n, 0, sel0);
  }
  uint32_t np[K];
#pragma unroll
  for (int j = 0; j < K; ++j) {
    np[j] = HCTX(n)[x * K + j];
    ma[j] = HCTX(kr)[x * K + j];
  }
  const uint32_t n0 = HCTX(n0inv);
  {
    uint32_t kb[K];
    montmul_reg<HG, false, false>(kb, b, ma, np, n0);
#pragma unroll
    for (int j = 0; j < K; ++j) {
      b[j] = kb[j];
      ma[j] = HCTX(h)[x * K + j];
      mb[j] = 0;
    }
  }
  seq_pairmul<G, K, false, false>(a, b, ma, mb, np, n0, sel0);
  full_normalise<HG>(a, x);
  uint32_t d[K];
  const uint32_t below_a = sub_limbs<HG>(d, a, np, x, lane);
  const uint32_t jflag = below_a ^ 1u;
  full_normalise<HG>(b, x);
  const uint32_t below = sub_limbs<HG>(d, b, np, x, lane);
  if (!below) {
#pragma unroll
    for (int j = 0; j < K; ++j) b[j] = d[j];
  }
  (void)sub_limbs<HG>(d, np, b, x, lane);
  if (x == 0) d[0] += jflag;
  full_normalise<HG>(d, x);
  const uint32_t small = sub_limbs<HG>(b, d, np, x, lane);
  if (small) {
#pragma unroll
    for (int j = 0; j < K; ++j) b[j] = d[j];
  }
  wave_lds_sync();
#pragma unroll
// ... 13 lines not shown
  constexpr int IPW = kWave / G, L2 = G * K, LQ = 2 * L2;
  raise_wave_priority();
  __shared__ __attribute__((aligned(16))) uint32_t qs_[kWavesPerWG][IPW][G * kAbPad];
  __shared__ __attribute__((aligned(16))) uint32_t ts_[kWavesPerWG][kWave][kAbPad];
  const int lane = threadIdx.x % kWave, wv = threadIdx.x / kWave;
  const int grp = lane / G, x = lane % G;
  uint32_t* qs = qs_[wv][grp];
  uint32_t* ts = ts_[wv][lane];
  uint32_t sel0 = x == 0 ? 1u : 0u;
  asm("" : "+v"(sel0));
  const size_t wave_id = (size_t)blockIdx.x * kWavesPerWG + wv;
  const size_t first_inst = wave_id * IPW;
  size_t inst = first_inst + grp;
  if (inst >= A.count) inst = A.count - 1;
  uint32_t n[K], a[K], b[K], ma[K], mb[K];
#pragma unroll
  for (int j = 0; j < K; ++j) n[j] = A.ctx.nhat[x * K + j];
  const int w = A.window, tsize = 1 << w;
  uint32_t* tbl = A.table + (wave_id * IPW + grp) * (size_t)tsize * LQ + x * K;
  const uint64_t* ep = A.exp + inst * A.exp_stride;
  const int nwin = (A.exp_bits + w - 1) / w;
  auto digit = [&](int i) -> int {
    int bit = i * w;
    int word = bit >> 6, sh = bit & 63;
    uint64_t v = (word < A.exp_words) ? ep[word] >> sh : 0;
    if (sh + w > 64 && word + 1 < A.exp_words) v |= ep[word + 1] << (64 - sh);
    return (int)(v & (uint64_t)(tsize - 1));
  };
  const bool gather = A.ct_gather != 0;
  {
    const uint32_t* row = A.base_pair + inst * A.base_pair_stride;
    load_pair_row<K>(a, row, x);
    load_pair_row<K>(b, row + L2, x);
  }
#pragma unroll
  for (int j = 0; j < K; ++j) {
    ma[j] = a[j];
    mb[j] = b[j];
    tbl[(size_t)LQ + j] = a[j];
    tbl[(size_t)LQ + L2 + j] = b[j];
    tbl[j] = A.ctx.one[x * K + j];
    tbl[L2 + j] = A.ctx.one[L2 + x * K + j];
  }
#pragma unroll 1
  for (int e = 2; e < tsize; ++e) {
    seq_pairmul<G, K, false, true, true>(a, b, ma, mb, n, 0, sel0, qs, ts);
#pragma unroll
    for (int j = 0; j < K; ++j) {
      tbl[(size_t)e * LQ + j] = a[j];
      tbl[(size_t)e * LQ + L2 + j] = b[j];
    }
  }
  int win = nwin - 2;
  if (nwin > 0) {
    const int d0 = digit(nwin - 1);
    load_table_entry<K>(a, tbl, d0, tsize, LQ, gather);
    load_table_entry<K>(b, tbl + L2, d0, tsize, LQ, gather);
  } else {
#pragma unroll
    for (int j = 0; j < K; ++j) {
      a[j] = A.ctx.one[x * K + j];
      b[j] = A.ctx.one[L2 + x * K + j];
    }
  }
#pragma unroll 1
  for (; nwin > 0 && win >= 0; --win) {
    const int idx = digit(win);
    load_table_entry<K>(ma, tbl, idx, tsize, LQ, gather);
    load_table_entry<K>(mb, tbl + L2, idx, tsize, LQ, gather);
#pragma unroll 1
    for (int i = 0; i < w; ++i) seq_pairmul<G, K, true, true, true>(a, b, a, b, n, 0, sel0, qs, ts);
    seq_pairmul<G, K, false, true, true>(a, b, ma, mb, n, 0, sel0, qs, ts);
  }
  if (first_inst + grp < A.count) {
    uint32_t* out = A.out_pair + inst * (size_t)LQ;
    store_pair_row<K>(out, a, x);
    store_pair_row<K>(out + L2, b, x);
  }
}

template <int G, int K>
__global__ __launch_bounds__(kWGThreads, 2) void pair_mul_seq_kernel(PairOpsArgs A) {
  constexpr int IPW = kWave / G, L2 = G * K, LQ = 2 * L2;
  raise_wave_priority();
  __shared__ __attribute__((aligned(16))) uint32_t qs_[kWavesPerWG][IPW][G * kAbPad];
  __shared__ __attribute__((aligned(16))) uint32_t ts_[kWavesPerWG][kWave][kAbPad];
  const int lane = threadIdx.x % kWave, wv = threadIdx.x / kWave;
  const int grp = lane / G, x = lane % G;
  uint32_t* qs = qs_[wv][grp];
  uint32_t* ts = ts_[wv][lane];
  uint32_t sel0 = x == 0 ? 1u : 0u;
  asm("" : "+v"(sel0));
  size_t inst = ((size_t)blockIdx.x * kWavesPerWG + wv) * IPW + grp;
  const bool live = inst < A.count;
  if (!live) inst = A.count - 1;
  uint32_t n[K], a[K], b[K], c[K], d[K];
  const uint32_t* ra = A.a + inst * (size_t)LQ;
  const uint32_t* rb = A.b + inst * A.b_stride;
  load_pair_row<K>(a, ra, x);
  load_pair_row<K>(b, ra + L2, x);
  load_pair_row<K>(c, rb, x);
  load_pair_row<K>(d, rb + L2, x);
#pragma unroll
  for (int j = 0; j < K; ++j) n[j] = A.ctx.nhat[x * K + j];
  seq_pairmul<G, K, false, true, true>(a, b, c, d, n, 0, sel0, qs, ts);
  if (live) {
    uint32_t* out = A.out + inst * (size_t)LQ;
    store_pair_row<K>(out, a, x);
    store_pair_row<K>(out + L2, b, x);
  }
}

template <int G, int K, int MINW = 2>
__global__ __launch_bounds__(kWGThreads, MINW) void hensel_fb_encrypt_seq_kernel(HenselFbArgs A) {
  using HG = Geo<G, K>;
  constexpr int IPW = kWave / G, L2 = G * K, LQ = 2 * L2;
  raise_wave_priority();
  __shared__ __attribute__((aligned(16))) uint32_t qs_[kWavesPerWG][IPW][G * kAbPad];
  __shared__ __attribute__((aligned(16))) uint32_t ts_[kWavesPerWG][kWave][kAbPad];
  __shared__ uint64_t io_[kWavesPerWG][IPW][HG::W64 + 1];
  const int lane = threadIdx.x % kWave, wv = threadIdx.x / kWave;
  const int grp = lane / G, x = lane % G;
  uint32_t* qs = qs_[wv][grp];
  uint32_t* ts = ts_[wv][lane];
  auto& io = io_[wv];
  uint32_t sel0 = x == 0 ? 1u : 0u;
  asm("" : "+v"(sel0));
  const size_t first_inst = ((size_t)blockIdx.x * kWavesPerWG + wv) * IPW;
  size_t inst = first_inst + grp;
  if (inst >= A.count) inst = A.count - 1;
  uint32_t n[K], a[K], b[K], ma[K], mb[K];
#pragma unroll
  for (int j = 0; j < K; ++j) n[j] = A.ctx.nhat[x * K + j];
  const int w = A.w, tsize = 1 << w;
  const uint64_t* ep = A.exp + inst * A.exp_stride;
  auto digit = [&](int i) -> int {
    int bit = i * w;
    int word = bit >> 6, sh = bit & 63;
    uint64_t v = (word < A.exp_words) ? ep[word] >> sh : 0;
    if (sh + w > 64 && word + 1 < A.exp_words) v |= ep[word + 1] << (64 - sh);
    return (int)(v & (uint64_t)(tsize - 1));
  };
  auto load_entry = [&](uint32_t (&da)[K], uint32_t (&db)[K], int i) {
    if (A.ct_gather) {
      const uint32_t* wb = A.table + (size_t)i * tsize * LQ + x * K;
      load_table_entry<K>(da, wb, digit(i), tsize, LQ, true);
      load_table_entry<K>(db, wb + L2, digit(i), tsize, LQ, true);
      return;
    }
    const uint32_t* e = A.table + ((size_t)i * tsize + digit(i)) * LQ;
    load_pair_row<K>(da, e, x);
    load_pair_row<K>(db, e + L2, x);
  };
  load_entry(a, b, 0);
  if (A.nwin > 1) load_entry(ma, mb, 1);
#pragma unroll 1
  for (int i = 1; i < A.nwin; ++i) {
    uint32_t na[K], nb[K];
    if (i + 1 < A.nwin) load_entry(na, nb, i + 1);
    seq_pairmul<G, K, false, true, true>(a, b, ma, mb, n, 0, sel0, qs, ts);
#pragma unroll
    for (int j = 0; j < K; ++j) {
      ma[j] = na[j];
      mb[j] = nb[j];
    }
  }
  stage_words<HG>(io, A.fm_words, A.fm_stride, 0, A.fm_nwords, first_inst, A.count, 1, lane);
  wave_lds_sync();
  {
    uint32_t mv[K], u[K], v[K];
#pragma unroll
    for (int j = 0; j < K; ++j) {
      n[j] = A.ctx.n[x * K + j];
      ma[j] = A.ctx.gm[x * K + j];
      mv[j] = limb_from_words(io[grp], x * K + j);
    }
    montmul_reg<HG, false, false>(u, mv, ma, n, A.ctx.n0inv);
    montmul_reg<HG, false, false>(v, u, a, n, A.ctx.n0inv);
    add_normalise<HG>(b, v);
  }
  if (first_inst + grp < A.count) {
    uint32_t* out = A.out_pair + inst * (size_t)LQ;
    store_pair_row<K>(out, a, x);
    store_pair_row<K>(out + L2, b, x);
  }
}

}

#endif
```

pailliercryptolib_amd/csrc/hensel_wave_n2.hpp:

```cpp
#ifndef PAILLIERCRYPTOLIB_AMD_CSRC_HENSEL_WAVE_N2_HPP_
#define PAILLIERCRYPTOLIB_AMD_CSRC_HENSEL_WAVE_N2_HPP_

#include "hensel_wave.hpp"

namespace pgpu {

template <int LPL>
struct WaveCtxN {
  uint32_t nl[LPL];
  uint32_t e0, maskv, onev;
};

template <int LPL, int I>
__device__ __forceinline__ uint32_t wvn_limb(const uint32_t (&x)[LPL]) {
  return (uint32_t)__builtin_amdgcn_readlane((int)x[I % LPL], I / LPL);
}

template <int LPL, int LB>
__device__ __forceinline__ void wvn_finish(uint32_t (&r)[LPL], const uint64_t (&acc)[LPL]) {
  r[0] = ((uint32_t)acc[0] & ((1u << LB) - 1)) + wv_up((uint32_t)(acc[LPL - 1] >> LB));
#pragma unroll
  for (int j = 1; j < LPL; ++j) r[j] = ((uint32_t)acc[j] & ((1u << LB) - 1)) + (uint32_t)(acc[j - 1] >> LB);
}

#define WV_PIN __builtin_amdgcn_sched_barrier(0)
template <int L2, int LPL, int LB, bool SQR, bool WIDEQ>
__device__ __forceinline__ void wvn_pairop(uint32_t (&a)[LPL], uint32_t (&b)[LPL], const uint32_t (&cm)[LPL],
                                           const uint32_t (&dm)[LPL], const WaveCtxN<LPL>& c) {
  uint64_t acc1[LPL], acc2[LPL];
  uint32_t m1[LPL], m2[LPL], a0[LPL], b0[LPL], lo1[LPL], lo2[LPL];
#pragma unroll
  for (int j = 0; j < LPL; ++j) {
    acc1[j] = acc2[j] = 0;
    a0[j] = a[j];
    b0[j] = b[j];
    m1[j] = SQR ? a[j] : cm[j];
    m2[j] = SQR ? b[j] << 1 : dm[j];
    lo1[j] = lo2[j] = 0;
  }
  uint32_t sa[L2 + 2], sb[L2 + 2];
  sa[0] = wvn_limb<LPL, 0>(a0);
  sa[1] = wvn_limb<LPL, (L2 > 1 ? 1 : 0)>(a0);
  if constexpr (!SQR) {
    sb[0] = wvn_limb<LPL, 0>(b0);
    sb[1] = wvn_limb<LPL, (L2 > 1 ? 1 : 0)>(b0);
  }
  WV_PIN;
#pragma unroll
  for (int j = 0; j < LPL; ++j) wv_mac(acc1[j], sa[0], m1[j]);
  WV_PIN;
  ps_static_for<L2>([&](auto ic) __attribute__((always_inline)) {
    constexpr int i = decltype(ic)::value;
    uint32_t q1, t1 = 0;
    if constexpr (WIDEQ) {
      q1 = (uint32_t)__builtin_amdgcn_readfirstlane((int)(uint32_t)acc1[0]);
      asm volatile("" : "+v"(acc2[0]) : "s"(q1));
    } else {
      t1 = (uint32_t)acc1[0] & c.maskv;
    }
    WV_PIN;
    if constexpr (i > 0) {
#pragma unroll
      for (int j = 0; j < LPL; ++j) wv_mac(acc2[j], lo2[(j + 1) % LPL], c.onev);
      WV_PIN;
    }
    if constexpr (!WIDEQ) {
      q1 = (uint32_t)__builtin_amdgcn_readfirstlane((int)t1);
      asm volatile("" : "+v"(acc2[0]) : "s"(q1));
      WV_PIN;
    }
#pragma unroll
    for (int j = 0; j < LPL; ++j) wv_mac(acc2[j], sa[i], m2[j]);
    WV_PIN;
    if constexpr (!SQR) {
#pragma unroll
      for (int j = 0; j < LPL; ++j) wv_mac(acc2[j], sb[i], m1[j]);
      WV_PIN;
    }
    wv_mac(acc2[0], q1, c.e0);
    WV_PIN;
#pragma unroll
    for (int j = 0; j < LPL; ++j) wv_mac(acc1[j], q1, c.nl[j]);
    WV_PIN;
    uint32_t q2, t2 = 0;
    if constexpr (WIDEQ) {
      q2 = (uint32_t)__builtin_amdgcn_readfirstlane((int)(uint32_t)acc2[0]);
      asm volatile("" : "+v"(acc1[0]) : "s"(q2));
    } else {
      t2 = (uint32_t)acc2[0] & c.maskv;
    }
    WV_PIN;
    if constexpr (i + 2 < L2) {
      sa[i + 2] = wvn_limb<LPL, (i + 2 < L2 ? i + 2 : 0)>(a0);
      if constexpr (!SQR) sb[i + 2] = wvn_limb<LPL, (i + 2 < L2 ? i + 2 : 0)>(b0);
    }
    WV_PIN;
    if constexpr (!WIDEQ) {
      q2 = (uint32_t)__builtin_amdgcn_readfirstlane((int)t2);
      asm volatile("" : "+v"(acc1[0]) : "s"(q2));
      WV_PIN;
    }
    lo1[0] = wv_down_and((uint32_t)acc1[0], c.maskv);
#pragma unroll
    for (int j = 1; j < LPL; ++j) lo1[j] = (uint32_t)acc1[j] & c.maskv;
    WV_PIN;
#pragma unroll
    for (int j = 0; j < LPL; ++j) acc1[j] >>= LB;
    WV_PIN;
#pragma unroll
    for (int j = 0; j < LPL; ++j) wv_mac(acc2[j], q2, c.nl[j]);
    WV_PIN;
#pragma unroll
    for (int j = 0; j < LPL; ++j) wv_mac(acc1[j], lo1[(j + 1) % LPL], c.onev);
    WV_PIN;
    if constexpr (i + 1 < L2) {
#pragma unroll
      for (int j = 0; j < LPL; ++j) wv_mac(acc1[j], sa[i + 1], m1[j]);
      WV_PIN;
    }
    lo2[0] = wv_down_and((uint32_t)acc2[0], c.maskv);
#pragma unroll
    for (int j = 1; j < LPL; ++j) lo2[j] = (uint32_t)acc2[j] & c.maskv;
    WV_PIN;
#pragma unroll
    for (int j = 0; j < LPL; ++j) acc2[j] >>= LB;
    WV_PIN;
  });
#pragma unroll
  for (int j = 0; j < LPL; ++j) wv_mac(acc2[j], lo2[(j + 1) % LPL], c.onev);
  wvn_finish<LPL, LB>(a, acc1);
  wvn_finish<LPL, LB>(b, acc2);
}
#undef WV_PIN

template <int LPL>
constexpr size_t wvn_table_words(size_t entries) { return entries * 2 * LPL * kWave; }

template <int L2, int LPL, bool WIDEQ>
__global__ __launch_bounds__(kWGThreads, 1) void hensel_modexp_wave_kernel(HenselModexpArgs A) {
  constexpr int LB = kLimbBits, NL = L2 / LPL;
  static_assert(L2 % LPL == 0 && NL < kWave, "LPL limbs per lane and a zero lane above them");
  raise_wave_priority();
  extern __shared__ uint32_t wvn_tbl_[];
  const int lane = threadIdx.x % kWave, wv = threadIdx.x / kWave;
  const size_t inst = (size_t)blockIdx.x * kWavesPerWG + wv;
  if (inst >= A.count) return;
  const bool in = lane < NL;
  const int lk = in ? lane : 0;
  WaveCtxN<LPL> c;
#pragma unroll
  for (int j = 0; j < LPL; ++j) c.nl[j] = in ? A.ctx.nhat[lk * LPL + j] : 0u;
  c.e0 = lane == 0 ? 1u : 0u;
  c.maskv = (1u << LB) - 1;
  c.onev = 1;
  asm("" : "+v"(c.maskv), "+v"(c.onev), "+v"(c.e0));
  const int w = A.window, tsize = 1 << w;
  uint32_t* tbl = wvn_tbl_ + (size_t)wv * wvn_table_words<LPL>((size_t)tsize) + lane;
  const uint64_t* ep = A.exp + inst * A.exp_stride;
  const int nwin = (A.exp_bits + w - 1) / w;
  auto digit = [&](int i) -> int {
    int bit = i * w;
    int word = bit >> 6, sh = bit & 63;
    uint64_t v = (word < A.exp_words) ? ep[word] >> sh : 0;
    if (sh + w > 64 && word + 1 < A.exp_words) v |= ep[word + 1] << (64 - sh);
    return __builtin_amdgcn_readfirstlane((int)(v & (uint64_t)(tsize - 1)));
  };
  const bool gather = A.ct_gather != 0;
  auto entry_load = [&](uint32_t (&x)[LPL], uint32_t (&y)[LPL], int e) {
    if (!gather) {
#pragma unroll
      for (int j = 0; j < LPL; ++j) {
        x[j] = tbl[((size_t)e * 2 * LPL + j) * kWave];
        y[j] = tbl[((size_t)e * 2 * LPL + LPL + j) * kWave];
      }
      return;
    }
    uint32_t ev = (uint32_t)e;
    asm("" : "+v"(ev));
#pragma unroll
    for (int j = 0; j < LPL; ++j) x[j] = y[j] = 0;
    for (int t = 0; t < tsize; ++t) {
      const bool sel = ev == (uint32_t)t;
#pragma unroll
      for (int j = 0; j < LPL; ++j) {
        const uint32_t tx = tbl[((size_t)t * 2 * LPL + j) * kWave], ty = tbl[((size_t)t * 2 * LPL + LPL + j) * kWave];
        x[j] = sel ? tx : x[j];
        y[j] = sel ? ty : y[j];
      }
    }
  };
  auto entry_store = [&](int e, const uint32_t (&x)[LPL], const uint32_t (&y)[LPL]) {
#pragma unroll
    for (int j = 0; j < LPL; ++j) {
      tbl[((size_t)e * 2 * LPL + j) * kWave] = x[j];
      tbl[((size_t)e * 2 * LPL + LPL + j) * kWave] = y[j];
    }
  };
  uint32_t a[LPL], b[LPL], ba[LPL], bb[LPL];
  {
    const uint32_t* row = A.base_pair + inst * A.base_pair_stride;
#pragma unroll
    for (int j = 0; j < LPL; ++j) {
      a[j] = ba[j] = in ? row[lk * LPL + j] : 0u;
      b[j] = bb[j] = in ? row[L2 + lk * LPL + j] : 0u;
    }
  }
  entry_store(1, a, b);
  {
    uint32_t oa[LPL], ob[LPL];
#pragma unroll
    for (int j = 0; j < LPL; ++j) {
      oa[j] = in ? A.ctx.one[lk * LPL + j] : 0u;
      ob[j] = in ? A.ctx.one[L2 + lk * LPL + j] : 0u;
    }
    entry_store(0, oa, ob);
  }
#pragma unroll 1
  for (int e = 2; e < tsize; ++e) {
    wvn_pairop<L2, LPL, LB, false, WIDEQ>(a, b, ba, bb, c);
    entry_store(e, a, b);
  }
  entry_load(a, b, nwin > 0 ? digit(nwin - 1) : 0);
  uint32_t ma[LPL], mb[LPL];
#pragma unroll 1
  for (int win = nwin - 2; win >= 1; --win) {
    const int d = digit(win);
#pragma unroll 1
    for (int i = 0; i < w; ++i) wvn_pairop<L2, LPL, LB, true, WIDEQ>(a, b, a, b, c);
    entry_load(ma, mb, d);
    wvn_pairop<L2, LPL, LB, false, WIDEQ>(a, b, ma, mb, c);
  }
  if (nwin >= 2) {
    const int d = digit(0);
#pragma unroll 1
    for (int i = 0; i < w; ++i) wvn_pairop<L2, LPL, LB, true, WIDEQ>(a, b, a, b, c);
    entry_load(ma, mb, d);
  } else {
    entry_load(ma, mb, 0);
  }
  wvn_pairop<L2, LPL, LB, false, false>(a, b, ma, mb, c);
  if (in) {
    uint32_t* out = A.out_pair + inst * (size_t)(2 * L2);
#pragma unroll
    for (int j = 0; j < LPL; ++j) {
      out[lk * LPL + j] = a[j];
      out[L2 + lk * LPL + j] = b[j];
    }
  }
}

template <int L2, int LPL, int LB>
__device__ __forceinline__ void wvn_montmul_true(uint32_t (&r)[LPL], const uint32_t (&x)[LPL], const uint32_t (&y)[LPL],
                                                 const uint32_t (&n)[LPL], uint32_t n0inv, uint32_t maskv, uint32_t onev) {
  uint64_t acc[LPL];
#pragma unroll
  for (int j = 0; j < LPL; ++j) acc[j] = 0;
  ps_static_for<L2>([&](auto ic) __attribute__((always_inline)) {
    constexpr int i = decltype(ic)::value;
    const uint32_t sx = wvn_limb<LPL, i>(x);
#pragma unroll
    for (int j = 0; j < LPL; ++j) wv_mac(acc[j], sx, y[j]);
    const uint32_t q = (uint32_t)__builtin_amdgcn_readfirstlane((int)(((uint32_t)acc[0] * n0inv) & maskv));
#pragma unroll
    for (int j = 0; j < LPL; ++j) wv_mac(acc[j], q, n[j]);
    uint32_t lo[LPL];
    lo[0] = wv_down_and((uint32_t)acc[0], maskv);
#pragma unroll
    for (int j = 1; j < LPL; ++j) lo[j] = (uint32_t)acc[j] & maskv;
#pragma unroll
    for (int j = 0; j < LPL; ++j) {
      acc[j] >>= LB;
      wv_mac(acc[j], lo[(j + 1) % LPL], onev);
    }
  });
  wvn_finish<LPL, LB>(r, acc);
}

template <int L2, int LPL, bool WIDEQ>
__global__ __launch_bounds__(kWGThreads, 1) void hensel_fb_encrypt_wave_kernel(HenselFbArgs A) {
  constexpr int LB = kLimbBits, NL = L2 / LPL;
  static_assert(L2 % LPL == 0 && NL < kWave, "LPL limbs per lane and a zero lane above them");
  raise_wave_priority();
  const int lane = threadIdx.x % kWave, wv = threadIdx.x / kWave;
  const size_t inst = (size_t)blockIdx.x * kWavesPerWG + wv;
  if (inst >= A.count) return;
  const bool in = lane < NL;
  const int lk = in ? lane : 0;
  WaveCtxN<LPL> c;
#pragma unroll
  for (int j = 0; j < LPL; ++j) c.nl[j] = in ? A.ctx.nhat[lk * LPL + j] : 0u;
  c.e0 = lane == 0 ? 1u : 0u;
  c.maskv = (1u << LB) - 1;
  c.onev = 1;
  asm("" : "+v"(c.maskv), "+v"(c.onev), "+v"(c.e0));
  const int w = A.w, tsize = 1 << w;
  const uint64_t* ep = A.exp + inst * A.exp_stride;
  auto digit = [&](int i) -> int {
    int bit = i * w;
    int word = bit >> 6, sh = bit & 63;
    uint64_t v = (word < A.exp_words) ? ep[word] >> sh : 0;
    if (sh + w > 64 && word + 1 < A.exp_words) v |= ep[word + 1] << (64 - sh);
    return __builtin_amdgcn_readfirstlane((int)(v & (uint64_t)(tsize - 1)));
  };
  const bool gather = A.ct_gather != 0;
  auto load_entry = [&](uint32_t (&x)[LPL], uint32_t (&y)[LPL], int i) {
    const uint32_t* win = A.table + (size_t)i * tsize * (2 * L2);
    const int d = digit(i);
    if (!gather) {
      const uint32_t* row = win + (size_t)d * (2 * L2);
#pragma unroll
      for (int j = 0; j < LPL; ++j) {
        x[j] = in ? row[lk * LPL + j] : 0u;
        y[j] = in ? row[L2 + lk * LPL + j] : 0u;
      }
      return;
    }
    uint32_t dv = (uint32_t)d;
    asm("" : "+v"(dv));
#pragma unroll
    for (int j = 0; j < LPL; ++j) x[j] = y[j] = 0;
    for (int t = 0; t < tsize; ++t) {
      const uint32_t* row = win + (size_t)t * (2 * L2);
      const bool sel = dv == (uint32_t)t;
#pragma unroll
      for (int j = 0; j < LPL; ++j) {
        const uint32_t tx = in ? row[lk * LPL + j] : 0u, ty = in ? row[L2 + lk * LPL + j] : 0u;
        x[j] = sel ? tx : x[j];
        y[j] = sel ? ty : y[j];
      }
    }
  };
  uint32_t a[LPL], b[LPL], ma[LPL], mb[LPL], na[LPL], nb[LPL];
  load_entry(a, b, 0);
  if (A.nwin > 1) load_entry(ma, mb, 1);
#pragma unroll 1
  for (int i = 1; i + 1 < A.nwin; ++i) {
    load_entry(na, nb, i + 1);
    wvn_pairop<L2, LPL, LB, false, WIDEQ>(a, b, ma, mb, c);
#pragma unroll
    for (int j = 0; j < LPL; ++j) {
      ma[j] = na[j];
      mb[j] = nb[j];
    }
  }
  if (A.nwin > 1) wvn_pairop<L2, LPL, LB, false, false>(a, b, ma, mb, c);
  {
    uint32_t nt[LPL], gm[LPL], mv[LPL], u[LPL], v[LPL];
    const uint64_t* mw = A.fm_words + inst * A.fm_stride;
#pragma unroll
    for (int j = 0; j < LPL; ++j) {
      nt[j] = in ? A.ctx.n[lk * LPL + j] : 0u;
      gm[j] = in ? A.ctx.gm[lk * LPL + j] : 0u;
      const int bit = (lk * LPL + j) * LB, word = bit >> 6, sh = bit & 63;
      uint64_t val = (in && word < A.fm_nwords) ? mw[word] >> sh : 0;
      if (in && sh > 64 - LB && word + 1 < A.fm_nwords) val |= mw[word + 1] << (64 - sh);
      mv[j] = (uint32_t)val & c.maskv;
    }
    wvn_montmul_true<L2, LPL, LB>(u, mv, gm, nt, A.ctx.n0inv, c.maskv, c.onev);
    wvn_montmul_true<L2, LPL, LB>(v, u, a, nt, A.ctx.n0inv, c.maskv, c.onev);
    uint32_t cy[LPL];
#pragma unroll
    for (int j = 0; j < LPL; ++j) {
      b[j] += v[j];
      cy[j] = b[j] >> LB;
      b[j] &= c.maskv;
    }
    b[0] += wv_up(cy[LPL - 1]);
#pragma unroll
    for (int j = 1; j < LPL; ++j) b[j] += cy[j - 1];
  }
  if (in) {
    uint32_t* out = A.out_pair + inst * (size_t)(2 * L2);
#pragma unroll
    for (int j = 0; j < LPL; ++j) {
      out[lk * LPL + j] = a[j];
      out[L2 + lk * LPL + j] = b[j];
    }
  }
}

}

#endif
```

pailliercryptolib_amd/csrc/k_hensel.hip:

```cpp
#include "hensel_seq.hpp"
#include "launch.hpp"
#if defined(PGPU_PART) && (PGPU_PART == 31 || PGPU_PART == 33 || PGPU_PART == 34)
#include "hensel_ps.hpp"
#endif
#if defined(PGPU_PART) && PGPU_PART == 35
#include "hensel_wave.hpp"
#endif
#if defined(PGPU_PART) && (PGPU_PART == 36 || PGPU_PART == 37)
#include "hensel_wave_n2.hpp"
#endif
#if defined(PGPU_PART) && PGPU_PART >= 38 && PGPU_PART <= 40
#include "hensel_matvec.hpp"
#endif

#ifndef PGPU_PART
#error "compile with -DPGPU_PART=0..40 (15 and 30 are retired)"
#endif

namespace pgpu {

#define PGPU_HENSEL_ONE(h, k)                                                                             \
  if (H == h && K == k) {                                                                                 \
    hipLaunchKernelGGL((hensel_decrypt_kernel<h, k>), dim3(blocks), dim3(kWGThreads), PGPU_PLACE_PAD((hensel_decrypt_kernel<h, k>), blocks), s, a);           \
    return true;                                                                                          \
  }

#if PGPU_PART == 0
bool launch_hensel_part0(int H, int K, const HenselArgs& a, unsigned blocks, hipStream_t s) {
  PGPU_HENSEL_ONE(2, 19) PGPU_HENSEL_ONE(2, 10) PGPU_HENSEL_ONE(4, 5)
  return false;
}
#elif PGPU_PART == 1
bool launch_hensel_part1(int H, int K, const HenselArgs& a, unsigned blocks, hipStream_t s) {
#if PGPU_WITH_4096
  PGPU_HENSEL_ONE(4, 18)
#endif
  PGPU_HENSEL_ONE(4, 14) PGPU_HENSEL_ONE(4, 10)
  return false;
}
#elif PGPU_PART == 3 || PGPU_PART == 4 || PGPU_PART == 10 || PGPU_PART == 22
#if PGPU_PART == 22
#define PGPU_FB_H 8
#define PGPU_FB_K 18
#define PGPU_FB_NAME(f) f##_part22
#elif PGPU_PART == 3
#define PGPU_FB_H 4
#define PGPU_FB_K 18
#define PGPU_FB_NAME(f) f##_part3
#elif PGPU_PART == 4
#define PGPU_FB_H 8
#define PGPU_FB_K 14
#define PGPU_FB_NAME(f) f##_part4
#else
#define PGPU_FB_H 2
#define PGPU_FB_K 19
#define PGPU_FB_NAME(f) f##_part10
#endif
bool PGPU_FB_NAME(launch_hensel_fb_build)(int H, int K, const HenselFbBuildArgs& a, unsigned blocks, hipStream_t s) {
  if (H == PGPU_FB_H && K == PGPU_FB_K) {
    hipLaunchKernelGGL((hensel_fb_build_kernel<PGPU_FB_H, PGPU_FB_K>), dim3(blocks), dim3(kWGThreads), 0, s, a);
    return true;
  }
  return false;
}
bool PGPU_FB_NAME(launch_hensel_fb_encrypt)(int H, int K, const HenselFbArgs& a, unsigned blocks, hipStream_t s) {
  if (H == PGPU_FB_H && K == PGPU_FB_K) {
    hipLaunchKernelGGL((hensel_fb_encrypt_kernel<PGPU_FB_H, PGPU_FB_K>), dim3(blocks), dim3(kWGThreads), PGPU_PLACE_PAD((hensel_fb_encrypt_kernel<PGPU_FB_H, PGPU_FB_K>), blocks), s, a);
    return true;
  }
  return false;
}
#elif PGPU_PART == 11 || PGPU_PART == 12 || PGPU_PART == 13 || PGPU_PART == 24 || PGPU_PART == 25
#if PGPU_PART == 25
#define PGPU_PO_H 8
#define PGPU_PO_K 9
#define PGPU_PO_NAME launch_pair_ops_part25
#elif PGPU_PART == 24
#define PGPU_PO_H 8
#define PGPU_PO_K 18
#define PGPU_PO_NAME launch_pair_ops_part24
#elif PGPU_PART == 11
#define PGPU_PO_H 4
#define PGPU_PO_K 18
#define PGPU_PO_NAME launch_pair_ops_part11
#elif PGPU_PART == 12
#define PGPU_PO_H 2
#define PGPU_PO_K 19
#define PGPU_PO_NAME launch_pair_ops_part12
#else
#define PGPU_PO_H 8
#define PGPU_PO_K 14
#define PGPU_PO_NAME launch_pair_ops_part13
#endif
bool PGPU_PO_NAME(int H, int K, const PairOpsArgs& a, unsigned blocks, hipStream_t s) {
  if (H == PGPU_PO_H && K == PGPU_PO_K) {
    hipLaunchKernelGGL((pair_ops_kernel<PGPU_PO_H, PGPU_PO_K>), dim3(blocks), dim3(kWGThreads), 0, s, a);
    return true;
  }
  return false;
}
#elif PGPU_PART == 16
bool launch_hensel_seq_part16(int G, int K, const HenselArgs& a, unsigned blocks, hipStream_t s, unsigned lds_pad) {
  if (G == 4 && K == 14) {
    const bool once = PGPU_LDS_ATTR_ONCE((hensel_decrypt_seq_kernel<4, 14>), 128 * 1024);
    if (lds_pad && !once) return false;
    hipLaunchKernelGGL((hensel_decrypt_seq_kernel<4, 14>), dim3(blocks), dim3(kWGThreads), lds_pad, s, a);
    return true;
  }
  return false;
}
#elif PGPU_PART == 17
bool launch_hensel_seq_part17(int G, int K, const HenselArgs& a, unsigned blocks, hipStream_t s, unsigned lds_pad) {
  if (G == 2 && K == 19) {
    const bool once = PGPU_LDS_ATTR_ONCE((hensel_decrypt_seq_kernel<2, 19>), 128 * 1024);
    if (lds_pad && !once) return false;
    hipLaunchKernelGGL((hensel_decrypt_seq_kernel<2, 19>), dim3(blocks), dim3(kWGThreads), lds_pad, s, a);
    return true;
  }
  return false;
}
#elif PGPU_PART == 32
bool launch_hensel_seq_w1_part32(int G, int K, const HenselArgs& a, unsigned blocks, hipStream_t s, unsigned lds_pad) {
  if (G == 2 && K == 19 && lds_pad) {
    const bool once = PGPU_LDS_ATTR_ONCE((hensel_decrypt_seq_kernel<2, 19, 1>), 128 * 1024);
    if (!once) return false;
    hipLaunchKernelGGL((hensel_decrypt_seq_kernel<2, 19, 1>), dim3(blocks), dim3(kWGThreads), lds_pad, s, a);
    return true;
  }
  return false;
}
#elif PGPU_PART == 18
bool launch_hensel_modexp_seq_part18(int G, int K, const HenselModexpArgs& a, unsigned blocks, hipStream_t s) {
  if (G == 4 && K == 18) {
    hipLaunchKernelGGL((hensel_modexp_seq_kernel<4, 18>), dim3(blocks), dim3(kWGThreads), 0, s, a);
    return true;
  }
  return false;
}
#elif PGPU_PART == 19
bool launch_pair_mul_seq_part19(int G, int K, const PairOpsArgs& a, unsigned blocks, hipStream_t s) {
  if (G == 4 && K == 18) {
    hipLaunchKernelGGL((pair_mul_seq_kernel<4, 18>), dim3(blocks), dim3(kWGThreads), 0, s, a);
    return true;
  }
  return false;
}
#elif PGPU_PART == 20
bool launch_hensel_fb_encrypt_seq_part20(int G, int K, const HenselFbArgs& a, unsigned blocks, hipStream_t s, unsigned lds_pad) {
  if (G == 4 && K == 18) {
    unsigned dyn = lds_pad;
    static const unsigned own = [] {
      hipFuncAttributes fa{};
      return hipFuncGetAttributes(&fa, (const void*)hensel_fb_encrypt_seq_kernel<4, 18>) == hipSuccess ? (unsigned)fa.sharedSizeBytes : 0u;
    }();
    if (lds_pad & kLdsTotalFlag) {
      const unsigned total = lds_pad & ~kLdsTotalFlag;
      dyn = own && total > own ? total - own : 0;
    }
    const bool once = PGPU_LDS_ATTR_ONCE((hensel_fb_encrypt_seq_kernel<4, 18>), 96 * 1024);
    const bool once1 = PGPU_LDS_ATTR_ONCE((hensel_fb_encrypt_seq_kernel<4, 18, 1>), 96 * 1024);
    if (dyn && (!once || !once1)) return false;
    static const bool w1 = [] { const char* e = getenv("PGPU_SEQ_W1"); return !e || atoi(e) != 0; }();
    if (w1 && dyn + own > 82000u && !(lds_pad & kLdsTotalFlag))
      hipLaunchKernelGGL((hensel_fb_encrypt_seq_kernel<4, 18, 1>), dim3(blocks), dim3(kWGThreads), dyn, s, a);
    else
      hipLaunchKernelGGL((hensel_fb_encrypt_seq_kernel<4, 18>), dim3(blocks), dim3(kWGThreads), dyn, s, a);
    return true;
  }
  return false;
}
#elif PGPU_PART == 21
bool launch_hensel_fb_encrypt_seq_part21(int G, int K, const HenselFbArgs& a, unsigned blocks, hipStream_t s) {
  if (G == 8 && K == 14) {
    hipLaunchKernelGGL((hensel_fb_encrypt_seq_kernel<8, 14>), dim3(blocks), dim3(kWGThreads), 0, s, a);
    return true;
  }
  return false;
}
#elif PGPU_PART == 26
bool launch_hensel_modexp_seq_part26(int G, int K, const HenselModexpArgs& a, unsigned blocks, hipStream_t s) {
  if (G == 8 && K == 14) {
    hipLaunchKernelGGL((hensel_modexp_seq_kernel<8, 14>), dim3(blocks), dim3(kWGThreads), 0, s, a);
    return true;
  }
  return false;
}
#elif PGPU_PART == 27
bool launch_pair_mul_seq_part27(int G, int K, const PairOpsArgs& a, unsigned blocks, hipStream_t s) {
  if (G == 8 && K == 14) {
    hipLaunchKernelGGL((pair_mul_seq_kernel<8, 14>), dim3(blocks), dim3(kWGThreads), 0, s, a);
    return true;
  }
  if (G == 2 && K == 19) {
    hipLaunchKernelGGL((pair_mul_seq_kernel<2, 19>), dim3(blocks), dim3(kWGThreads), 0, s, a);
    return true;
  }
  return false;
}
#elif PGPU_PART == 28
bool launch_hensel_modexp_seq_part28(int G, int K, const HenselModexpArgs& a, unsigned blocks, hipStream_t s) {
  if (G == 2 && K == 19) {
    hipLaunchKernelGGL((hensel_modexp_seq_kernel<2, 19>), dim3(blocks), dim3(kWGThreads), 0, s, a);
    return true;
  }
  return false;
}
bool launch_hensel_fb_encrypt_seq_part28(int G, int K, const HenselFbArgs& a, unsigned blocks, hipStream_t s) {
  if (G == 2 && K == 19) {
    hipLaunchKernelGGL((hensel_fb_encrypt_seq_kernel<2, 19>), dim3(blocks), dim3(kWGThreads), 0, s, a);
    return true;
  }
  return false;
}
// ... 213 lines not shown
```

pailliercryptolib_amd/csrc/kargs.hpp:

```cpp
#ifndef PAILLIERCRYPTOLIB_AMD_CSRC_KARGS_HPP_
#define PAILLIERCRYPTOLIB_AMD_CSRC_KARGS_HPP_

#include <stddef.h>
#include <stdint.h>

namespace pgpu {

constexpr int kWave = 64;
constexpr int kLimbBits = 29;
constexpr uint32_t kLimbMask = (1u << kLimbBits) - 1;
constexpr int kWavesPerWG = 4;
constexpr int kWGThreads = kWave * kWavesPerWG;

struct ModCtxDev {
  const uint32_t* n;
  const uint32_t* r2;
  const uint32_t* one;
  const uint32_t* r2s;
  const uint32_t* fc;
  const uint32_t* nr;
  const uint64_t* n64;
  const uint32_t* nhat;
  const uint32_t* gadd;
  uint32_t n0inv;
  int mod_words;
};

enum FinalMul : int {
  FM_UNIT = 0,
  FM_CTX_CONST = 1,
  FM_PAILLIER_G = 2
};

struct ModexpArgs {
  ModCtxDev ctx[2];
  int nctx;
  const uint64_t* base;
  size_t base_stride;
  int base_words;
  const uint64_t* exp;
  size_t exp_stride;
  int exp_per_ctx;
  int exp_words;
  int exp_bits;
  int window;
  const uint16_t* sched[2];
  int sched_len[2];
  int parity_waves;
  int final_mul;
  const uint64_t* fm_words;
  size_t fm_stride;
  int fm_nwords;
  uint64_t* out;
  size_t out_stride;
  uint32_t* table;
  size_t count;
  uint64_t* wave_clocks;
};

struct ModmulArgs {
  ModCtxDev ctx;
  const uint64_t* a;
  size_t a_stride;
  const uint64_t* b;
  size_t b_stride;
  int in_words;
  uint64_t* out;
  size_t count;
  int mode;
  int b_words;
};

enum ModmulMode : int {
  MM_PLAIN = 0,
  MM_SINGLE = 1,
  MM_BY_R2 = 2,
  MM_BY_ONE = 3,
  MM_GM = 4
};

struct CrtArgs {
  ModCtxDev ctxM;
  ModCtxDev ctxQ;
  const uint32_t* cp;
  const uint32_t* cq;
  const uint32_t* pinvR;
  const uint32_t* pRM;
  const uint64_t* hp64;
  const uint64_t* hq64;
  const uint64_t* p2_64;
  const uint64_t* q2_64;
  const uint64_t* q64;
  const uint64_t* v;
  int vw;
  int have_m;
  uint64_t* out;
  int out_words;
  size_t count;
};

struct HenselCtxDev {
  const uint32_t* nhat;
  const uint32_t* n;
  const uint32_t* one;
  const uint32_t* conv;
  const uint32_t* h;
  const uint32_t* kr;
  uint32_t n0inv;
  const uint32_t* pconv;
  const uint32_t* pcb;
};

struct HenselArgs {
  HenselCtxDev ctx[2];
  const uint64_t* ct;
  size_t ct_stride;
  int ct_words;
  int chunk_words;
  int nchunks;
  const uint64_t* exp;
  size_t exp_stride;
  int exp_words;
  int exp_bits;
  int window;
  const uint16_t* sched[2];
  int sched_len[2];
  uint64_t* out;
  size_t out_stride;
  int out_words;
  uint32_t* table;
  size_t count;
  int ct_gather;
  const uint32_t* ct_pair;
  size_t ct_pair_stride;
  int pair_l2;
  int pchunk_limbs, pchunks;
};

struct HenselPubDev {
  const uint32_t* nhat;
  const uint32_t* n;
  const uint32_t* kr;
  const uint32_t* one;
  const uint32_t* conv;
  const uint32_t* gm;
  uint32_t n0inv;
};

struct HenselFbBuildArgs {
  HenselPubDev ctx;
  const uint64_t* base;
  int base_words;
  int chunk_words;
  int nchunks;
  uint32_t* table;
  int nwin;
  int w;
};

struct HenselFullDev {
  const uint32_t* n;
  const uint32_t* nr;
  const uint32_t* r2;
  uint32_t n0inv;
  int mod_words;
};

struct HenselFbArgs {
  HenselPubDev ctx;
  HenselFullDev full;
  const uint32_t* table;
  int nwin;
  int w;
  const uint64_t* exp;
  size_t exp_stride;
  int exp_words;
  const uint64_t* fm_words;
  size_t fm_stride;
  int fm_nwords;
  uint64_t* out;
  size_t out_stride;
  size_t count;
  uint32_t* out_pair;
  int ct_gather;
};

struct HenselModexpArgs {
  HenselPubDev ctx;
  HenselFullDev full;
  const uint64_t* base;
  size_t base_stride;
  int base_words;
  int chunk_words;
  int nchunks;
  const uint64_t* exp;
  size_t exp_stride;
  int exp_words;
  int exp_bits;
  int window;
  const uint16_t* sched;
  int sched_len;
  int final_mul;
  const uint64_t* fm_words;
  size_t fm_stride;
  int fm_nwords;
  uint64_t* out;
  size_t out_stride;
  uint32_t* table;
  size_t count;
  int ct_gather;
  const uint32_t* base_pair;
  size_t base_pair_stride;
  uint32_t* out_pair;
};

enum PairOp : int {
  PO_MUL = 0,
  PO_TIMES_GM = 1,
  PO_FROM_WORDS = 2,
  PO_TO_WORDS = 3
};
struct PairOpsArgs {
  HenselPubDev ctx;
  HenselFullDev full;
  int op;
  const uint32_t* a;
  const uint32_t* b;
  size_t b_stride;
  const uint64_t* words;
  size_t words_stride;
  int nwords;
  int chunk_words, nchunks;
  uint32_t* out;
  uint64_t* out_words;
  size_t out_stride;
  size_t count;
};

struct MatvecArgs {
  HenselPubDev ctx;
  const uint32_t* x;
  uint32_t* table;
  const uint64_t* w;
  size_t w_stride;
  int w_words;
  int e_bits;
  int window;
  int slices;
  size_t rows, cols;
  uint32_t* out;
};

struct FixedBaseArgs {
  ModCtxDev ctx;
  const uint32_t* table;
  int nwin;
  int w;
  const uint64_t* exp;
  size_t exp_stride;
  int exp_words;
  const uint64_t* fm_words;
  size_t fm_stride;
  int fm_nwords;
  uint64_t* out;
  size_t out_stride;
  size_t count;
  int ct_gather;
};

struct FixedBaseBuildArgs {
  ModCtxDev ctx;
  const uint64_t* base;
  uint32_t* table;
  int nwin;
  int w;
};

}

#endif
```

pailliercryptolib_amd/csrc/launch.hpp:

```cpp
#ifndef PAILLIERCRYPTOLIB_AMD_CSRC_LAUNCH_HPP_
#define PAILLIERCRYPTOLIB_AMD_CSRC_LAUNCH_HPP_

#include <hip/hip_runtime_api.h>

#include "kargs.hpp"

#include <algorithm>
#include <atomic>
#include <cstdlib>
#include <mutex>

#ifndef PGPU_WITH_4096
#define PGPU_WITH_4096 0
#endif

namespace pgpu {

inline bool lds_attr_once(const void* fn, int bytes, std::atomic<uint64_t>& done) {
  int dev = -1;
  if (hipGetDevice(&dev) != hipSuccess || dev < 0 || dev >= 64) return false;
  const uint64_t bit = (uint64_t)1 << dev;
  if (done.load(std::memory_order_acquire) & bit) return true;
  static std::mutex mu;
  std::lock_guard<std::mutex> lk(mu);
  if (done.load(std::memory_order_acquire) & bit) return true;
  if (hipFuncSetAttribute(fn, hipFuncAttributeMaxDynamicSharedMemorySize, bytes) != hipSuccess) {
    (void)hipGetLastError();
    return false;
  }
  done.fetch_or(bit, std::memory_order_release);
  return true;
}
#define PGPU_LDS_ATTR_ONCE(kernel_expr, bytes)                                        \
  ([]() -> bool {                                                                    \
    static std::atomic<uint64_t> done_{0};                                           \
    return ::pgpu::lds_attr_once((const void*)(kernel_expr), (bytes), done_);        \
  }())

inline int place_pad_limit() {
  static const int limit = [] {
    const char* e = std::getenv("PGPU_PLACE_PAD");
    return e ? std::max(0, std::atoi(e)) : 192;
  }();
  return limit;
}
inline unsigned place_pad(const void* fn, unsigned blocks, std::atomic<uint64_t>& done, std::atomic<int>& pad_bytes) {
  const int limit = place_pad_limit();
  if (limit == 0) return 0;
  int pad = pad_bytes.load(std::memory_order_acquire);
  if (pad < 0) {
    hipFuncAttributes fa{};
    if (hipFuncGetAttributes(&fa, fn) != hipSuccess) {
      (void)hipGetLastError();
      return 0;
    }
    const int want = 81 * 1024, have = (int)fa.sharedSizeBytes;
    pad = have >= want ? 0 : ((want - have + 1023) / 1024) * 1024;
    pad_bytes.store(pad, std::memory_order_release);
  }
  if (pad == 0 || !lds_attr_once(fn, pad, done)) return 0;
  return blocks <= (unsigned)limit ? (unsigned)pad : 0;
}
#define PGPU_PLACE_PAD(kernel_expr, blocks)                                                      \
  ([&]() -> unsigned {                                                                          \
    static std::atomic<uint64_t> done_{0};                                                      \
    static std::atomic<int> pad_{-1};                                                           \
    return ::pgpu::place_pad((const void*)(kernel_expr), (blocks), done_, pad_);                \
  }())

bool launch_modexp_part0(int G, int K, const ModexpArgs& a, unsigned blocks, hipStream_t s);
bool launch_modexp_part1(int G, int K, const ModexpArgs& a, unsigned blocks, hipStream_t s);
bool launch_modexp_part2(int G, int K, const ModexpArgs& a, unsigned blocks, hipStream_t s);
bool launch_modexp_part3(int G, int K, const ModexpArgs& a, unsigned blocks, hipStream_t s);
bool launch_modexp_reg_part4(int G, int K, const ModexpArgs& a, unsigned blocks, hipStream_t s);
bool launch_modexp_reg_part5(int G, int K, const ModexpArgs& a, unsigned blocks, hipStream_t s);
bool launch_modexp_reg_part6(int G, int K, const ModexpArgs& a, unsigned blocks, hipStream_t s);
bool launch_modexp_reg_part7(int G, int K, const ModexpArgs& a, unsigned blocks, hipStream_t s);
inline bool modexp_has_regrows(int G, int K) { return G == 2 || G == 4 || (G == 16 && K <= 7); }
inline bool launch_modexp(int G, int K, bool regrows, const ModexpArgs& a, unsigned blocks, hipStream_t s) {
  if (regrows)
    return launch_modexp_reg_part4(G, K, a, blocks, s) || launch_modexp_reg_part5(G, K, a, blocks, s) ||
           launch_modexp_reg_part6(G, K, a, blocks, s) || launch_modexp_reg_part7(G, K, a, blocks, s);
  return launch_modexp_part0(G, K, a, blocks, s) || launch_modexp_part1(G, K, a, blocks, s) ||
         launch_modexp_part2(G, K, a, blocks, s) || launch_modexp_part3(G, K, a, blocks, s);
}

inline bool hensel_has(int H, int K) {
  return (H == 2 && (K == 10 || K == 19)) || (H == 4 && (K == 5 || K == 10 || K == 14 || (PGPU_WITH_4096 && K == 18))) ||
         (H == 8 && (K == 3 || K == 5 || K == 7 || (PGPU_WITH_4096 && K == 9)));
}
bool launch_hensel_part0(int H, int K, const HenselArgs& a, unsigned blocks, hipStream_t s);
bool launch_hensel_part1(int H, int K, const HenselArgs& a, unsigned blocks, hipStream_t s);
bool launch_hensel_part2(int H, int K, const HenselArgs& a, unsigned blocks, hipStream_t s);
bool launch_hensel_part7(int H, int K, const HenselArgs& a, unsigned blocks, hipStream_t s);
inline bool launch_hensel(int H, int K, bool packed, const HenselArgs& a, unsigned blocks, hipStream_t s) {
  if (packed && launch_hensel_part7(H, K, a, blocks, s)) return true;
  return launch_hensel_part0(H, K, a, blocks, s) || launch_hensel_part1(H, K, a, blocks, s) ||
         launch_hensel_part2(H, K, a, blocks, s);
}

inline bool hensel_fb_has(int H, int K) {
  return (H == 2 && K == 19) || (H == 4 && K == 18) || (H == 8 && (K == 14 || (PGPU_WITH_4096 && K == 18)));
}
bool launch_hensel_fb_build_part3(int H, int K, const HenselFbBuildArgs& a, unsigned blocks, hipStream_t s);
bool launch_hensel_fb_build_part4(int H, int K, const HenselFbBuildArgs& a, unsigned blocks, hipStream_t s);
bool launch_hensel_fb_build_part10(int H, int K, const HenselFbBuildArgs& a, unsigned blocks, hipStream_t s);
bool launch_hensel_fb_build_part22(int H, int K, const HenselFbBuildArgs& a, unsigned blocks, hipStream_t s);
bool launch_hensel_fb_encrypt_part22(int H, int K, const HenselFbArgs& a, unsigned blocks, hipStream_t s);
bool launch_hensel_fb_encrypt_part3(int H, int K, const HenselFbArgs& a, unsigned blocks, hipStream_t s);
bool launch_hensel_fb_encrypt_part4(int H, int K, const HenselFbArgs& a, unsigned blocks, hipStream_t s);
bool launch_hensel_fb_encrypt_part10(int H, int K, const HenselFbArgs& a, unsigned blocks, hipStream_t s);
inline bool launch_hensel_fb_build(int H, int K, const HenselFbBuildArgs& a, unsigned blocks, hipStream_t s) {
  return launch_hensel_fb_build_part3(H, K, a, blocks, s) || launch_hensel_fb_build_part4(H, K, a, blocks, s) ||
         launch_hensel_fb_build_part10(H, K, a, blocks, s)
#if PGPU_WITH_4096
         || launch_hensel_fb_build_part22(H, K, a, blocks, s)
#endif
      ;
}
bool launch_hensel_fb_encrypt_part14(int H, int K, const HenselFbArgs& a, unsigned blocks, hipStream_t s);
inline bool hensel_fb_encrypt_has(int H, int K) { return hensel_fb_has(H, K) || (H == 8 && K == 9); }
inline bool launch_hensel_fb_encrypt(int H, int K, const HenselFbArgs& a, unsigned blocks, hipStream_t s) {
  return launch_hensel_fb_encrypt_part3(H, K, a, blocks, s) || launch_hensel_fb_encrypt_part4(H, K, a, blocks, s) ||
         launch_hensel_fb_encrypt_part10(H, K, a, blocks, s) || launch_hensel_fb_encrypt_part14(H, K, a, blocks, s)
#if PGPU_WITH_4096
         || launch_hensel_fb_encrypt_part22(H, K, a, blocks, s)
#endif
      ;
}

inline bool hensel_modexp_has(int H, int K) {
  return (H == 4 && (K == 18 || K == 10)) || (H == 8 && (K == 9 || K == 5 || K == 14 || (PGPU_WITH_4096 && K == 18))) || (H == 2 && K == 19);
}
bool launch_hensel_modexp_part5(int H, int K, const HenselModexpArgs& a, unsigned blocks, hipStream_t s);
bool launch_hensel_modexp_part6(int H, int K, const HenselModexpArgs& a, unsigned blocks, hipStream_t s);
bool launch_hensel_modexp_part8(int H, int K, const HenselModexpArgs& a, unsigned blocks, hipStream_t s);
bool launch_hensel_modexp_part9(int H, int K, const HenselModexpArgs& a, unsigned blocks, hipStream_t s);
bool launch_hensel_modexp_part23(int H, int K, const HenselModexpArgs& a, unsigned blocks, hipStream_t s);
inline bool launch_hensel_modexp(int H, int K, const HenselModexpArgs& a, unsigned blocks, hipStream_t s) {
  return launch_hensel_modexp_part5(H, K, a, blocks, s) || launch_hensel_modexp_part6(H, K, a, blocks, s) ||
         launch_hensel_modexp_part8(H, K, a, blocks, s) || launch_hensel_modexp_part9(H, K, a, blocks, s)
#if PGPU_WITH_4096
         || launch_hensel_modexp_part23(H, K, a, blocks, s)
#endif
      ;
}

inline bool pair_ops_has(int H, int K) {
  return (H == 2 && K == 19) || (H == 4 && K == 18) || (H == 8 && (K == 14 || (PGPU_WITH_4096 && K == 18)));
}
inline bool pair_ops_alt_has(int H, int K) { return H == 8 && K == 9; }
bool launch_pair_ops_part25(int H, int K, const PairOpsArgs& a, unsigned blocks, hipStream_t s);
bool launch_pair_ops_part11(int H, int K, const PairOpsArgs& a, unsigned blocks, hipStream_t s);
bool launch_pair_ops_part12(int H, int K, const PairOpsArgs& a, unsigned blocks, hipStream_t s);
bool launch_pair_ops_part13(int H, int K, const PairOpsArgs& a, unsigned blocks, hipStream_t s);
bool launch_pair_ops_part24(int H, int K, const PairOpsArgs& a, unsigned blocks, hipStream_t s);
inline bool launch_pair_ops(int H, int K, const PairOpsArgs& a, unsigned blocks, hipStream_t s) {
  return launch_pair_ops_part11(H, K, a, blocks, s) || launch_pair_ops_part12(H, K, a, blocks, s) ||
         launch_pair_ops_part13(H, K, a, blocks, s) || launch_pair_ops_part25(H, K, a, blocks, s)
#if PGPU_WITH_4096
         || launch_pair_ops_part24(H, K, a, blocks, s)
#endif
      ;
}

inline bool hensel_seq_has(int G, int K) { return (G == 4 && K == 14) || (G == 2 && (K == 19 || K == 10)); }
bool launch_hensel_seq_part16(int G, int K, const HenselArgs& a, unsigned blocks, hipStream_t s, unsigned lds_pad);
bool launch_hensel_seq_part17(int G, int K, const HenselArgs& a, unsigned blocks, hipStream_t s, unsigned lds_pad);
bool launch_hensel_seq_part29(int G, int K, const HenselArgs& a, unsigned blocks, hipStream_t s, unsigned lds_pad);
bool launch_hensel_seq_w1_part32(int G, int K, const HenselArgs& a, unsigned blocks, hipStream_t s, unsigned lds_pad);
inline bool launch_hensel_seq(int G, int K, const HenselArgs& a, unsigned blocks, hipStream_t s, unsigned lds_pad = 0,
                              bool one_per_simd = false) {
  if (one_per_simd && launch_hensel_seq_w1_part32(G, K, a, blocks, s, lds_pad)) return true;
  return launch_hensel_seq_part16(G, K, a, blocks, s, lds_pad) || launch_hensel_seq_part17(G, K, a, blocks, s, lds_pad) ||
         launch_hensel_seq_part29(G, K, a, blocks, s, lds_pad);
}

inline bool hensel_ps_has(int K, int lb) { return ((K == 38 || K == 56) && lb == 28) || (K == 19 && lb == 29); }
bool launch_hensel_ps_part31(int K, int lb, const HenselArgs& a, unsigned blocks, hipStream_t s, unsigned lds_pad);
bool launch_hensel_ps_part33(int K, int lb, const HenselArgs& a, unsigned blocks, hipStream_t s, unsigned lds_pad);
bool launch_hensel_ps_part34(int K, int lb, const HenselArgs& a, unsigned blocks, hipStream_t s, unsigned lds_pad);
inline bool launch_hensel_ps(int K, int lb, const HenselArgs& a, unsigned blocks, hipStream_t s, unsigned lds_pad = 0) {
  return launch_hensel_ps_part31(K, lb, a, blocks, s, lds_pad) || launch_hensel_ps_part33(K, lb, a, blocks, s, lds_pad) ||
         launch_hensel_ps_part34(K, lb, a, blocks, s, lds_pad);
}
inline bool hensel_wave_has(int K, int lb) { return (K == 38 && lb == 28) || (K == 56 && lb == 28) || (K == 19 && lb == 29); }
inline size_t hensel_wave_pair_words(int K) { return 2 * (size_t)K; }
bool launch_hensel_wave_part35(int K, int lb, bool wide_digits, const HenselArgs& a, hipStream_t s);
inline bool launch_hensel_wave(int K, int lb, bool wide_digits, const HenselArgs& a, hipStream_t s) {
  return launch_hensel_wave_part35(K, lb, wide_digits, a, s);
}
inline bool hensel_modexp_wave_has(int L2) { return L2 == 72 || L2 == 112 || L2 == 38; }
bool launch_hensel_modexp_wave_part36(int L2, const HenselModexpArgs& a, hipStream_t s);
bool launch_hensel_modexp_wave_part37(int L2, const HenselModexpArgs& a, hipStream_t s);
inline bool launch_hensel_modexp_wave(int L2, const HenselModexpArgs& a, hipStream_t s) {
  return launch_hensel_modexp_wave_part36(L2, a, s) || launch_hensel_modexp_wave_part37(L2, a, s);
}
bool launch_hensel_fb_encrypt_wave_part36(int L2, const HenselFbArgs& a, hipStream_t s);
bool launch_hensel_fb_encrypt_wave_part37(int L2, const HenselFbArgs& a, hipStream_t s);
inline bool launch_hensel_fb_encrypt_wave(int L2, const HenselFbArgs& a, hipStream_t s) {
  return launch_hensel_fb_encrypt_wave_part36(L2, a, s) || launch_hensel_fb_encrypt_wave_part37(L2, a, s);
}
inline size_t hensel_ps_table_words(int K, size_t entries) { return entries * 2 * (size_t)((K + 3) / 4) * 64 * 4; }

inline bool hensel_modexp_seq_has(int G, int K) { return (G == 4 && K == 18) || (G == 8 && K == 14) || (G == 2 && K == 19); }
bool launch_hensel_modexp_seq_part18(int G, int K, const HenselModexpArgs& a, unsigned blocks, hipStream_t s);
bool launch_hensel_modexp_seq_part26(int G, int K, const HenselModexpArgs& a, unsigned blocks, hipStream_t s);
bool launch_hensel_modexp_seq_part28(int G, int K, const HenselModexpArgs& a, unsigned blocks, hipStream_t s);
inline bool launch_hensel_modexp_seq(int G, int K, const HenselModexpArgs& a, unsigned blocks, hipStream_t s) {
  return launch_hensel_modexp_seq_part18(G, K, a, blocks, s) || launch_hensel_modexp_seq_part26(G, K, a, blocks, s) ||
         launch_hensel_modexp_seq_part28(G, K, a, blocks, s);
}

inline bool pair_mul_seq_has(int G, int K) { return (G == 4 && K == 18) || (G == 8 && K == 14) || (G == 2 && K == 19); }
bool launch_pair_mul_seq_part19(int G, int K, const PairOpsArgs& a, unsigned blocks, hipStream_t s);
bool launch_pair_mul_seq_part27(int G, int K, const PairOpsArgs& a, unsigned blocks, hipStream_t s);
inline bool launch_pair_mul_seq(int G, int K, const PairOpsArgs& a, unsigned blocks, hipStream_t s) {
  return launch_pair_mul_seq_part19(G, K, a, blocks, s) || launch_pair_mul_seq_part27(G, K, a, blocks, s);
}

inline bool matvec_has(int G, int K) { return (G == 4 && K == 18) || (G == 8 && K == 14) || (G == 2 && K == 19); }
bool launch_matvec_part38(int G, int K, bool table, const MatvecArgs& a, unsigned blocks, hipStream_t s);
bool launch_matvec_part39(int G, int K, bool table, const MatvecArgs& a, unsigned blocks, hipStream_t s);
bool launch_matvec_part40(int G, int K, bool table, const MatvecArgs& a, unsigned blocks, hipStream_t s);
inline bool launch_matvec_table(int G, int K, const MatvecArgs& a, unsigned blocks, hipStream_t s) {
  return launch_matvec_part38(G, K, true, a, blocks, s) || launch_matvec_part39(G, K, true, a, blocks, s) ||
         launch_matvec_part40(G, K, true, a, blocks, s);
}
inline bool launch_matvec(int G, int K, const MatvecArgs& a, unsigned blocks, hipStream_t s) {
  return launch_matvec_part38(G, K, false, a, blocks, s) || launch_matvec_part39(G, K, false, a, blocks, s) ||
         launch_matvec_part40(G, K, false, a, blocks, s);
}

inline bool hensel_fb_encrypt_seq_has(int G, int K) { return (G == 4 && K == 18) || (G == 8 && K == 14) || (G == 2 && K == 19); }
bool launch_hensel_fb_encrypt_seq_part28(int G, int K, const HenselFbArgs& a, unsigned blocks, hipStream_t s);
bool launch_hensel_fb_encrypt_seq_part20(int G, int K, const HenselFbArgs& a, unsigned blocks, hipStream_t s, unsigned lds_pad);
bool launch_hensel_fb_encrypt_seq_part21(int G, int K, const HenselFbArgs& a, unsigned blocks, hipStream_t s);
constexpr unsigned kLdsTotalFlag = 0x80000000u;
inline bool launch_hensel_fb_encrypt_seq(int G, int K, const HenselFbArgs& a, unsigned blocks, hipStream_t s, unsigned lds_pad = 0) {
  return launch_hensel_fb_encrypt_seq_part20(G, K, a, blocks, s, lds_pad) || launch_hensel_fb_encrypt_seq_part21(G, K, a, blocks, s) ||
         launch_hensel_fb_encrypt_seq_part28(G, K, a, blocks, s);
}

bool launch_modmul(int G, int K, const ModmulArgs& a, unsigned blocks, hipStream_t s);
bool launch_crt(int G, int K, const CrtArgs& a, unsigned blocks, hipStream_t s, unsigned lds_total = 0);
bool launch_fb_build(int G, int K, const FixedBaseBuildArgs& a, unsigned blocks, hipStream_t s);
bool launch_fb_encrypt(int G, int K, const FixedBaseArgs& a, unsigned blocks, hipStream_t s);

}

#endif
```

Measured before the change: 5.807 million.

## Store split-form fixed-base table in unit-factor form to drop cross-term products

```diff
diff --git a/pailliercryptolib_amd/csrc/capi.cpp b/pailliercryptolib_amd/csrc/capi.cpp
--- a/pailliercryptolib_amd/csrc/capi.cpp
+++ b/pailliercryptolib_amd/csrc/capi.cpp
@@ -504,9 +504,11 @@
 
 }
 
+enum FbForm : int { FB_FORM_FULL = 0, FB_FORM_UNIT_FACTOR = 1 };
 struct FbTable {
   void* p = nullptr;
   int w = 0, nwin = 0;
+  int form = FB_FORM_FULL;
   hipEvent_t ready = nullptr;
   size_t bytes = 0;
   uint64_t tick = 0;
@@ -993,7 +995,7 @@
 
 template <class Build>
 int fb_table_get(const pgpu_pubkey* key, std::vector<std::list<FbTable>>& lists, rt::Device& d, int w, int nwin,
-                 size_t entry_bytes, hipStream_t s, FbPin* out, Build build) {
+                 size_t entry_bytes, size_t scratch_bytes, hipStream_t s, FbPin* out, Build build) {
   std::lock_guard<std::mutex> lk(g_fb_mu);
   if (lists.size() < (size_t)rt::pool_size()) lists.resize((size_t)rt::pool_size());
   auto& list = lists[(size_t)d.index];
@@ -1019,7 +1021,7 @@
   t.w = w;
   t.nwin = nwin;
   t.bytes = (size_t)nwin * ((size_t)1 << w) * entry_bytes;
-  fb_make_room(d.index, t.bytes);
+  fb_make_room(d.index, t.bytes + scratch_bytes);
   hipError_t e = hipMalloc(&t.p, t.bytes);
   if (e != hipSuccess) return fail(PGPU_ERR_HIP, std::string("fixed-base table: ") + hipGetErrorString(e));
   if (hipEventCreateWithFlags(&t.ready, hipEventDefault) != hipSuccess || hipEventCreateWithFlags(&t.t0, hipEventDefault) != hipSuccess) {
@@ -1046,7 +1048,7 @@
 
 int fb_table_for(const pgpu_pubkey* key, rt::Device& d, int w, int nwin, hipStream_t s, FbPin* out) {
   const GeoInfo& geo = key->nsq->geo;
-  return fb_table_get(key, key->fb, d, w, nwin, (size_t)geo.L() * sizeof(uint32_t), s, out, [&](FbTable& t) -> int {
+  return fb_table_get(key, key->fb, d, w, nwin, (size_t)geo.L() * sizeof(uint32_t), 0, s, out, [&](FbTable& t) -> int {
     pgpu::FixedBaseBuildArgs b{};
     b.ctx = key->nsq->view(d.index);
     b.base = (const uint64_t*)key->d_hs.d[(size_t)d.index];
@@ -1215,7 +1217,17 @@
 int fb_table_for_split(const pgpu_pubkey* key, const pgpu_pubkey::PubForm* form, rt::Device& d, int w, int nwin,
                        hipStream_t s, FbPin* out) {
   const int H = form->H, K = form->K;
-  return fb_table_get(key, key->fbh, d, w, nwin, (size_t)2 * H * K * sizeof(uint32_t), s, out, [&](FbTable& t) -> int {
+  const int L2 = H * K;
+  const int seg_len = std::max(2, std::min(1 << w, 1024)), nseg = (1 << w) / seg_len;
+  const size_t ntot = (size_t)nwin * nseg, rowl = ntot * L2;
+  const size_t pre_bytes = ((size_t)nwin << w) * L2 * sizeof(uint32_t), io_bytes = 2 * rowl * sizeof(uint32_t);
+  return fb_table_get(key, key->fbh, d, w, nwin, (size_t)2 * H * K * sizeof(uint32_t), pre_bytes + io_bytes, s, out, [&](FbTable& t) -> int {
+    struct Scratch {
+      void* p = nullptr;
+      ~Scratch() { if (p) (void)hipFree(p); }
+    } pre, io;
+    HIP_TRY(hipMalloc(&pre.p, pre_bytes));
+    HIP_TRY(hipMalloc(&io.p, io_bytes));
     pgpu::HenselFbBuildArgs b{};
     b.ctx = hensel_pub_view(form, d.index);
     b.base = (const uint64_t*)key->d_hs.d[(size_t)d.index];
@@ -1225,10 +1237,54 @@
     b.table = (uint32_t*)t.p;
     b.nwin = nwin;
     b.w = w;
+    b.seg_len = seg_len;
+    b.prefix = (uint32_t*)pre.p;
+    b.total = (uint32_t*)io.p;
     const int ipw = 64 / (2 * H);
     const unsigned blocks = (unsigned)((((size_t)nwin + ipw - 1) / ipw + pgpu::kWavesPerWG - 1) / pgpu::kWavesPerWG);
     if (!pgpu::launch_hensel_fb_build(H, K, b, blocks, s))
       return fail(PGPU_ERR_UNSUPPORTED, "split-form fixed-base build kernel not compiled");
+    std::vector<uint32_t> h(rowl);
+    HIP_TRY(hipMemcpyAsync(h.data(), b.total, rowl * sizeof(uint32_t), hipMemcpyDeviceToHost, s));
+    HIP_TRY(hipStreamSynchronize(s));
+    const BigNumber& n = form->n;
+    const BigNumber scale = ((pow2(L2 * pgpu::kLimbBits) % n) * (n - BigNumber((Ipp32u)form->n0inv) % n)) % n;
+    std::vector<uint64_t> words(((size_t)L2 * pgpu::kLimbBits + 63) / 64 + 1);
+    std::vector<BigNumber> tot(ntot), before(ntot);
+    BigNumber acc((Ipp32u)1);
+    for (size_t i = 0; i < ntot; ++i) {
+      std::fill(words.begin(), words.end(), 0);
+      for (int j = 0; j < L2; ++j) {
+        const size_t bit = (size_t)j * pgpu::kLimbBits;
+        const uint64_t v = h[i * L2 + j];
+        words[bit >> 6] |= v << (bit & 63);
+        if ((bit & 63) + pgpu::kLimbBits > 64) words[(bit >> 6) + 1] |= v >> (64 - (bit & 63));
+      }
+      tot[i] = BigNumber::fromLimbs64(words.data(), words.size()) % n;
+      if (tot[i].isZero()) return fail(PGPU_ERR_INVALID_PARAM, "fixed-base table: hs is not a unit modulo n");
+      before[i] = acc;
+      acc = (acc * tot[i]) % n;
+    }
+    BigNumber inv = n.InverseMul(acc);
+    for (size_t i = ntot; i-- > 0;) {
+      to_limbs29((((inv * before[i]) % n) * scale) % n, L2, h.data() + i * L2);
+      inv = (inv * tot[i]) % n;
+    }
+    pgpu::HenselFbUnitArgs u{};
+    u.n = b.ctx.n;
+    u.n0inv = b.ctx.n0inv;
+    u.table = b.table;
+    u.nwin = nwin;
+    u.w = w;
+    u.seg_len = seg_len;
+    u.prefix = b.prefix;
+    u.uinit = (uint32_t*)io.p + rowl;
+    HIP_TRY(hipMemcpyAsync((void*)u.uinit, h.data(), rowl * sizeof(uint32_t), hipMemcpyHostToDevice, s));
+    const unsigned blocks1 = (unsigned)(((ntot + ipw - 1) / ipw + pgpu::kWavesPerWG - 1) / pgpu::kWavesPerWG);
+    if (!pgpu::launch_hensel_fb_unit_factor(H, K, u, blocks1, s))
+      return fail(PGPU_ERR_UNSUPPORTED, "split-form fixed-base build kernel not compiled");
+    HIP_TRY(hipStreamSynchronize(s));
+    t.form = FB_FORM_UNIT_FACTOR;
     return PGPU_OK;
   });
 }
@@ -1259,6 +1315,7 @@
     FbPin tab;
     if (const pgpu_pubkey::PubForm* form = sform) {
       RC_TRY(fb_table_for_split(key, form, d, fbw, nwin, s, &tab));
+      if (tab->form != FB_FORM_UNIT_FACTOR) return fail(PGPU_ERR_UNSUPPORTED, "split-form encrypt needs a unit-factor table");
       if (d_pair) {
         for (const auto& alt : key->hforms) {
           const size_t ipw_alt = 64 / (2 * (size_t)alt->H);
@@ -1314,6 +1371,7 @@
       return PGPU_OK;
     }
     RC_TRY(fb_table_for(key, d, fbw, nwin, s, &tab));
+    if (tab->form != FB_FORM_FULL) return fail(PGPU_ERR_UNSUPPORTED, "full-width encrypt needs a table of residues");
     pgpu::FixedBaseArgs f{};
     f.ctx = key->nsq->view(d.index, vflags);
     f.table = (const uint32_t*)tab->p;
diff --git a/pailliercryptolib_amd/csrc/hensel.hpp b/pailliercryptolib_amd/csrc/hensel.hpp
--- a/pailliercryptolib_amd/csrc/hensel.hpp
+++ b/pailliercryptolib_amd/csrc/hensel.hpp
@@ -21,7 +21,7 @@
   else return bcast_lane<4, S>(src);
 }
 
-template <int H, int K, bool SQR, bool UNITQ, int S>
+template <int H, int K, bool SQR, bool UNITQ, int S, bool DZ = false>
 __device__ __forceinline__ void pair_block(uint64_t (&LOWC)[K], uint64_t (&UPC)[K], const uint32_t (&mc)[K],
                                            const uint32_t (&md)[K], const uint32_t (&csrc)[K],
                                            const uint32_t (&asrc)[K], const uint32_t (&n)[K], uint32_t n0inv,
@@ -39,7 +39,7 @@
       else UPC[r + j - K] += p;
     }
   }
-  if constexpr (!SQR) {
+  if constexpr (!SQR && !DZ) {
     uint32_t arow[K];
 #pragma unroll
     for (int r = 0; r < K; ++r) arow[r] = pair_row<H, S>(asrc[r]);
@@ -56,37 +56,43 @@
   mont_reduce_rows<GEO, UNITQ, true, true>(LOWC, UPC, n, n0inv, selB);
 }
 
-template <int H, int K, bool SQR, bool UNITQ, int S>
+template <int H, int K, bool SQR, bool UNITQ, int S, bool DZ = false>
 __device__ __forceinline__ void pair_blocks(uint64_t (&c0)[K], uint64_t (&c1)[K], const uint32_t (&mc)[K],
                                             const uint32_t (&md)[K], const uint32_t (&csrc)[K],
                                             const uint32_t (&asrc)[K], const uint32_t (&n)[K], uint32_t n0inv,
                                             uint32_t selB) {
   if constexpr (S < H) {
-    pair_block<H, K, SQR, UNITQ, S>(c0, c1, mc, md, csrc, asrc, n, n0inv, selB);
-    pair_block<H, K, SQR, UNITQ, S + 1>(c1, c0, mc, md, csrc, asrc, n, n0inv, selB);
-    pair_blocks<H, K, SQR, UNITQ, S + 2>(c0, c1, mc, md, csrc, asrc, n, n0inv, selB);
-  }
-}
-template <int H, int K, bool SQR, bool UNITQ>
+    pair_block<H, K, SQR, UNITQ, S, DZ>(c0, c1, mc, md, csrc, asrc, n, n0inv, selB);
+    pair_block<H, K, SQR, UNITQ, S + 1, DZ>(c1, c0, mc, md, csrc, asrc, n, n0inv, selB);
+    pair_blocks<H, K, SQR, UNITQ, S + 2, DZ>(c0, c1, mc, md, csrc, asrc, n, n0inv, selB);
+  }
+}
+template <int H, int K, bool SQR, bool UNITQ, bool DZ = false>
 __device__ __forceinline__ void pairmul(uint32_t (&r)[K], const uint32_t (&own)[K], const uint32_t (&m)[K],
                                         const uint32_t (&n)[K], uint32_t n0inv, uint32_t halfB, uint32_t selB) {
+  static_assert(!(SQR && DZ), "a squaring has no zero operand");
   static_assert(3 * K + 6 < 64, "a column of half B receives 3K products (+ relaxed limbs): must stay below 2^64");
   static_assert(H == 2 || H == 4 || H == 8, "two halves inside one 16-lane DPP row");
   using GEO = Geo<H, K>;
   uint64_t c0[K], c1[K];
   uint32_t mc[K], md[K], csrc[K], asrc[K];
   const uint32_t maskB = 0u - halfB;
-  pair_row_source<H, K>(asrc, own);
+  if constexpr (!DZ) {
+    pair_row_source<H, K>(asrc, own);
+  } else {
+#pragma unroll
+    for (int j = 0; j < K; ++j) asrc[j] = 0;
+  }
   if constexpr (!SQR) pair_row_source<H, K>(csrc, m);
 #pragma unroll
   for (int j = 0; j < K; ++j) {
     c0[j] = 0;
     c1[j] = 0;
     mc[j] = SQR ? own[j] << halfB : own[j];
-    md[j] = SQR ? 0 : m[j] & maskB;
+    md[j] = (SQR || DZ) ? 0 : m[j] & maskB;
   }
   if constexpr (SQR) pair_blocks<H, K, SQR, UNITQ, 0>(c0, c1, mc, md, asrc, asrc, n, n0inv, selB);
-  else pair_blocks<H, K, SQR, UNITQ, 0>(c0, c1, mc, md, csrc, asrc, n, n0inv, selB);
+  else pair_blocks<H, K, SQR, UNITQ, 0, DZ>(c0, c1, mc, md, csrc, asrc, n, n0inv, selB);
   montmul_finish<GEO>(r, c0);
 }
 
@@ -369,15 +375,14 @@
 }
 
 template <int H, int K>
-__device__ __forceinline__ void pair_times_gm(uint32_t (&own)[K], const HenselPubDev& C, const uint64_t* mwords, int x,
-                                              uint32_t halfB) {
+__device__ __forceinline__ void pair_times_gm_limbs(uint32_t (&own)[K], const HenselPubDev& C, const uint32_t (&mv)[K], int x,
+                                                    uint32_t halfB) {
   using HG = Geo<H, K>;
-  uint32_t n[K], mv[K], cg[K], u[K], av[K], v[K];
+  uint32_t n[K], cg[K], u[K], av[K], v[K];
 #pragma unroll
   for (int j = 0; j < K; ++j) {
     n[j] = C.n[x * K + j];
     cg[j] = C.gm[x * K + j];
-    mv[j] = limb_from_words(mwords, x * K + j);
   }
   montmul_reg<HG, false, false>(u, mv, cg, n, C.n0inv);
 #pragma unroll
@@ -389,6 +394,14 @@
 #pragma unroll
   for (int j = 0; j < K; ++j) v[j] = halfB ? v[j] : 0u;
   add_normalise<HG>(own, v);
+}
+template <int H, int K>
+__device__ __forceinline__ void pair_times_gm(uint32_t (&own)[K], const HenselPubDev& C, const uint64_t* mwords, int x,
+                                              uint32_t halfB) {
+  uint32_t mv[K];
+#pragma unroll
+  for (int j = 0; j < K; ++j) mv[j] = limb_from_words(mwords, x * K + j);
+  pair_times_gm_limbs<H, K>(own, C, mv, x, halfB);
 }
 
 template <int H, int K>
@@ -504,7 +517,7 @@
 template <int H, int K>
 __global__ __launch_bounds__(kWGThreads, K <= 14 ? 2 : 1) void hensel_fb_build_kernel(HenselFbBuildArgs A) {
   using HG = Geo<H, K>;
-  constexpr int GS = 2 * H, IPW = kWave / GS, LQ = 2 * H * K, W64 = HG::W64;
+  constexpr int GS = 2 * H, IPW = kWave / GS, L2 = H * K, LQ = 2 * H * K, W64 = HG::W64;
   __shared__ uint64_t io_[kWavesPerWG][IPW][W64 + 1];
   const int lane = threadIdx.x % kWave, wv = threadIdx.x / kWave;
   auto& io = io_[wv];
@@ -516,11 +529,18 @@
   size_t inst = first_inst + grp;
   const bool live = inst < (size_t)A.nwin;
   if (!live) inst = (size_t)A.nwin - 1;
-  uint32_t n[K], own[K], mreg[K];
+  const int tsize = 1 << A.w;
+  const int seg_len = A.seg_len, nseg = tsize / seg_len;
+  uint32_t* row = A.table + inst * (size_t)tsize * LQ + xg * K;
+  uint32_t* pre = A.prefix + inst * (size_t)tsize * L2 + x * K;
+  uint32_t nt[K];
+#pragma unroll
+  for (int j = 0; j < K; ++j) nt[j] = A.ctx.n[x * K + j];
+  const uint32_t n0t = A.ctx.n0inv;
+  uint32_t n[K], own[K], mreg[K], pr[K];
 #pragma unroll
   for (int j = 0; j < K; ++j) n[j] = A.ctx.nhat[x * K + j];
   pair_from_words<H, K>(own, A.base, A.base_words, A.chunk_words, A.nchunks, A.ctx.conv, io[grp], n, halfB, selB, xg);
-  const int tsize = 1 << A.w;
   const int my_sq = A.w * (int)inst;
   size_t last = first_inst + IPW - 1;
   if (last >= (size_t)A.nwin) last = (size_t)A.nwin - 1;
@@ -534,22 +554,109 @@
       for (int j = 0; j < K; ++j) own[j] = r[j];
     }
   }
-  uint32_t* row = A.table + inst * (size_t)tsize * LQ + xg * K;
+  const bool keepA = live && !halfB;
+#pragma unroll
+  for (int j = 0; j < K; ++j) mreg[j] = A.ctx.one[xg * K + j];
+  montmul_reg<HG, false, false>(pr, mreg, own, nt, n0t);
   if (live) {
 #pragma unroll
     for (int j = 0; j < K; ++j) {
-      row[j] = A.ctx.one[xg * K + j];
+      row[j] = mreg[j];
       row[LQ + j] = own[j];
     }
   }
+  if (keepA) {
+#pragma unroll
+    for (int j = 0; j < K; ++j) {
+      pre[j] = mreg[j];
+      pre[L2 + j] = pr[j];
+    }
+  }
 #pragma unroll
   for (int j = 0; j < K; ++j) mreg[j] = own[j];
+  auto put_total = [&](int seg) {
+    uint32_t c[K];
+#pragma unroll
+    for (int j = 0; j < K; ++j) c[j] = pr[j];
+    full_normalise<HG>(c, x);
+    if (keepA) {
+#pragma unroll
+      for (int j = 0; j < K; ++j) A.total[(inst * nseg + seg) * (size_t)L2 + x * K + j] = c[j];
+    }
+  };
 #pragma unroll 1
   for (int d = 2; d < tsize; ++d) {
     pairmul<H, K, false, true>(own, own, mreg, n, 0, halfB, selB);
+    if ((d & (seg_len - 1)) == 0) {
+      put_total(d / seg_len - 1);
+#pragma unroll
+      for (int j = 0; j < K; ++j) pr[j] = own[j];
+    } else {
+      uint32_t t[K];
+      montmul_reg<HG, false, false>(t, pr, own, nt, n0t);
+#pragma unroll
+      for (int j = 0; j < K; ++j) pr[j] = t[j];
+    }
     if (live) {
 #pragma unroll
       for (int j = 0; j < K; ++j) row[(size_t)d * LQ + j] = own[j];
+    }
+    if (keepA) {
+#pragma unroll
+      for (int j = 0; j < K; ++j) pre[(size_t)d * L2 + j] = pr[j];
+    }
+  }
+  put_total(nseg - 1);
+}
+
+template <int H, int K>
+__global__ __launch_bounds__(kWGThreads, K <= 14 ? 2 : 1) void hensel_fb_unit_factor_kernel(HenselFbUnitArgs A) {
+  using HG = Geo<H, K>;
+  constexpr int GS = 2 * H, IPW = kWave / GS, L2 = H * K, LQ = 2 * H * K;
+  const int lane = threadIdx.x % kWave, wv = threadIdx.x / kWave;
+  const int grp = lane / GS, xg = lane % GS, x = xg % H;
+  const uint32_t halfB = (uint32_t)(xg / H);
+  const int tsize = 1 << A.w, seg_len = A.seg_len, nseg = tsize / seg_len;
+  const size_t nsegs = (size_t)A.nwin * nseg;
+  size_t seg = ((size_t)blockIdx.x * kWavesPerWG + wv) * IPW + grp;
+  const bool live = seg < nsegs;
+  if (!live) seg = nsegs - 1;
+  const size_t inst = seg / nseg;
+  uint32_t* row = A.table + inst * (size_t)tsize * LQ + xg * K;
+  const uint32_t* pre = A.prefix + inst * (size_t)tsize * L2 + x * K;
+  uint32_t nt[K], u[K];
+#pragma unroll
+  for (int j = 0; j < K; ++j) {
+    nt[j] = A.n[x * K + j];
+    u[j] = A.uinit[seg * (size_t)L2 + x * K + j];
+  }
+  const uint32_t n0t = A.n0inv;
+  const int d0 = (int)(seg % nseg) * seg_len;
+#pragma unroll 1
+  for (int d = d0 + seg_len - 1; d >= d0; --d) {
+    uint32_t ent[K], r[K], be[K];
+#pragma unroll
+    for (int j = 0; j < K; ++j) ent[j] = row[(size_t)d * LQ + j];
+    if (d > d0) {
+      uint32_t mult[K];
+#pragma unroll
+      for (int j = 0; j < K; ++j) mult[j] = halfB ? pre[(size_t)(d - 1) * L2 + j] : ent[j];
+      montmul_reg<HG, false, false>(r, u, mult, nt, n0t);
+    } else {
+#pragma unroll
+      for (int j = 0; j < K; ++j) r[j] = u[j];
+    }
+    montmul_reg<HG, false, false>(be, ent, r, nt, n0t);
+    full_normalise<HG>(be, x);
+    cond_sub_limbs<HG>(be, nt, x, lane);
+    if (live && halfB) {
+#pragma unroll
+      for (int j = 0; j < K; ++j) row[(size_t)d * LQ + j] = be[j];
+    }
+#pragma unroll
+    for (int j = 0; j < K; ++j) {
+      const uint32_t below = dpp_from_below<H>(r[j]);
+      u[j] = halfB ? below : r[j];
     }
   }
 }
@@ -569,12 +676,13 @@
   auto& rows = rows_[wv];
   const int grp = lane / GS, xg = lane % GS, x = xg % H;
   const uint32_t halfB = (uint32_t)(xg / H);
+  const uint32_t maskB = 0u - halfB;
   uint32_t selB = xg == H ? 1u : 0u;
   asm("" : "+v"(selB));
   const size_t first_inst = ((size_t)blockIdx.x * kWavesPerWG + wv) * IPW;
   size_t inst = first_inst + grp;
   if (inst >= A.count) inst = A.count - 1;
-  uint32_t n[K], own[K], mreg[K], nxt[K];
+  uint32_t n[K], own[K], mreg[K], nxt[K], S[K];
 #pragma unroll
   for (int j = 0; j < K; ++j) n[j] = A.ctx.nhat[x * K + j];
   const int w = A.w, tsize = 1 << w;
@@ -590,23 +698,43 @@
     load_table_entry<K>(dst, A.table + (size_t)i * tsize * LQ + xg * K, digit(i), tsize, LQ, A.ct_gather != 0);
   };
   load_entry(own, 0);
+#pragma unroll
+  for (int j = 0; j < K; ++j) {
+    S[j] = own[j] & maskB;
+    own[j] &= ~maskB;
+  }
   if (A.nwin > 1) load_entry(mreg, 1);
 #pragma unroll 1
   for (int i = 1; i < A.nwin; ++i) {
     if (i + 1 < A.nwin) load_entry(nxt, i + 1);
-    pairmul<H, K, false, true>(own, own, mreg, n, 0, halfB, selB);
+    pairmul<H, K, false, true, true>(own, own, mreg, n, 0, halfB, selB);
+    uint32_t be[K];
+#pragma unroll
+    for (int j = 0; j < K; ++j) be[j] = mreg[j] & maskB;
+    if (i & 1) {
+#pragma unroll
+      for (int j = 0; j < K; ++j) S[j] += be[j];
+    } else {
+      add_normalise<HG>(S, be);
+    }
 #pragma unroll
     for (int j = 0; j < K; ++j) mreg[j] = nxt[j];
   }
+  stage_words<FG>(io, A.fm_words, A.fm_stride, 0, A.fm_nwords, first_inst, A.count, 1, lane);
+  wave_lds_sync();
+  {
+    uint32_t mv[K];
+#pragma unroll
+    for (int j = 0; j < K; ++j) mv[j] = limb_from_words(io[grp], x * K + j);
+    add_normalise<HG>(mv, S);
+    pair_times_gm_limbs<H, K>(own, A.ctx, mv, x, halfB);
+  }
   if (A.out_pair) {
-    stage_words<FG>(io, A.fm_words, A.fm_stride, 0, A.fm_nwords, first_inst, A.count, 1, lane);
-    wave_lds_sync();
-    pair_times_gm<H, K>(own, A.ctx, io[grp], x, halfB);
     if (first_inst + grp < A.count) store_pair_row<K>(A.out_pair + inst * (size_t)LQ, own, xg);
     return;
   }
-  pair_exit_store<H, K>(own, A.ctx, A.full, true, A.fm_words, A.fm_stride, A.fm_nwords, A.out, A.out_stride, first_inst,
-                        A.count, bl, io, rows, lane, grp, xg, halfB, selB);
+  pair_exit_store<H, K>(own, A.ctx, A.full, false, nullptr, 0, 0, A.out, A.out_stride, first_inst, A.count, bl, io, rows,
+                        lane, grp, xg, halfB, selB);
 }
 
 #ifndef PGPU_HM_WAVES18
diff --git a/pailliercryptolib_amd/csrc/hensel_seq.hpp b/pailliercryptolib_amd/csrc/hensel_seq.hpp
--- a/pailliercryptolib_amd/csrc/hensel_seq.hpp
+++ b/pailliercryptolib_amd/csrc/hensel_seq.hpp
@@ -40,7 +40,7 @@
   }
 }
 
-template <int G, int K, bool SQR, bool UNITQ, int S, bool QLDS = false>
+template <int G, int K, bool SQR, bool UNITQ, int S, bool QLDS = false, bool DZ = false>
 __device__ __forceinline__ void seq_b_blocks(uint64_t (&c0)[K], uint64_t (&c1)[K], const uint32_t (&mc)[K],
                                              const uint32_t (&md)[K], const uint32_t (&a)[K], const uint32_t (&c)[K],
                                              const uint32_t (&n)[K], uint32_t n0inv, uint32_t (&qd)[QLDS ? 1 : G][K],
@@ -59,7 +59,7 @@
         else c1[r + j - K] += p;
       }
     }
-    if constexpr (!SQR) {
+    if constexpr (!SQR && !DZ) {
 #pragma unroll
       for (int r = 0; r < K; ++r) row[r] = bcast_lane<G, S>(a[r]);
 #pragma unroll
@@ -79,16 +79,17 @@
     } else {
       mont_reduce_rows_q<HG, UNITQ, 2>(c0, c1, n, n0inv, qd[S], sel0);
     }
-    seq_b_blocks<G, K, SQR, UNITQ, S + 1, QLDS>(c1, c0, mc, md, a, c, n, n0inv, qd, sel0, qs);
-  }
-}
-
-template <int G, int K, bool SQR, bool UNITQ, bool QLDS = false>
+    seq_b_blocks<G, K, SQR, UNITQ, S + 1, QLDS, DZ>(c1, c0, mc, md, a, c, n, n0inv, qd, sel0, qs);
+  }
+}
+
+template <int G, int K, bool SQR, bool UNITQ, bool QLDS = false, bool DZ = false>
 __device__ __forceinline__ void seq_pairmul(uint32_t (&a)[K], uint32_t (&b)[K], const uint32_t (&c)[K],
                                             const uint32_t (&d)[K], const uint32_t (&n)[K], uint32_t n0inv, uint32_t sel0,
                                             uint32_t* qs = nullptr, uint32_t* ts = nullptr) {
   static_assert(3 * K + 6 < 64, "a column receives 3K products (+ relaxed limbs): must stay below 2^64");
   static_assert(G % 2 == 0, "blocks alternate between the two accumulator sets and end in the first");
+  static_assert(!(SQR && DZ), "a squaring has no zero operand");
   using HG = Geo<G, K>;
   uint32_t qd[QLDS ? 1 : G][K];
   uint32_t t[K];
@@ -115,9 +116,9 @@
       c0[j] = 0;
       c1[j] = 0;
       mc[j] = SQR ? b[j] << 1 : b[j];
-      md[j] = SQR ? 0u : d[j];
-    }
-    seq_b_blocks<G, K, SQR, UNITQ, 0, QLDS>(c0, c1, mc, md, a, c, n, n0inv, qd, sel0, qs);
+      md[j] = (SQR || DZ) ? 0u : d[j];
+    }
+    seq_b_blocks<G, K, SQR, UNITQ, 0, QLDS, DZ>(c0, c1, mc, md, a, c, n, n0inv, qd, sel0, qs);
     montmul_finish<HG>(b, c0);
   }
   if constexpr (QLDS) {
@@ -437,13 +438,22 @@
     load_pair_row<K>(da, e, x);
     load_pair_row<K>(db, e + L2, x);
   };
-  load_entry(a, b, 0);
+  uint32_t S[K];
+  load_entry(a, S, 0);
+#pragma unroll
+  for (int j = 0; j < K; ++j) b[j] = 0;
   if (A.nwin > 1) load_entry(ma, mb, 1);
 #pragma unroll 1
   for (int i = 1; i < A.nwin; ++i) {
     uint32_t na[K], nb[K];
     if (i + 1 < A.nwin) load_entry(na, nb, i + 1);
-    seq_pairmul<G, K, false, true, true>(a, b, ma, mb, n, 0, sel0, qs, ts);
+    seq_pairmul<G, K, false, true, true, true>(a, b, ma, mb, n, 0, sel0, qs, ts);
+    if (i & 1) {
+#pragma unroll
+      for (int j = 0; j < K; ++j) S[j] += mb[j];
+    } else {
+      add_normalise<HG>(S, mb);
+    }
 #pragma unroll
     for (int j = 0; j < K; ++j) {
       ma[j] = na[j];
@@ -460,6 +470,7 @@
       ma[j] = A.ctx.gm[x * K + j];
       mv[j] = limb_from_words(io[grp], x * K + j);
     }
+    add_normalise<HG>(mv, S);
     montmul_reg<HG, false, false>(u, mv, ma, n, A.ctx.n0inv);
     montmul_reg<HG, false, false>(v, u, a, n, A.ctx.n0inv);
     add_normalise<HG>(b, v);
diff --git a/pailliercryptolib_amd/csrc/hensel_wave_n2.hpp b/pailliercryptolib_amd/csrc/hensel_wave_n2.hpp
--- a/pailliercryptolib_amd/csrc/hensel_wave_n2.hpp
+++ b/pailliercryptolib_amd/csrc/hensel_wave_n2.hpp
@@ -24,7 +24,7 @@
 }
 
 #define WV_PIN __builtin_amdgcn_sched_barrier(0)
-template <int L2, int LPL, int LB, bool SQR, bool WIDEQ>
+template <int L2, int LPL, int LB, bool SQR, bool WIDEQ, bool DZ = false>
 __device__ __forceinline__ void wvn_pairop(uint32_t (&a)[LPL], uint32_t (&b)[LPL], const uint32_t (&cm)[LPL],
                                            const uint32_t (&dm)[LPL], const WaveCtxN<LPL>& c) {
   uint64_t acc1[LPL], acc2[LPL];
@@ -35,7 +35,7 @@
     a0[j] = a[j];
     b0[j] = b[j];
     m1[j] = SQR ? a[j] : cm[j];
-    m2[j] = SQR ? b[j] << 1 : dm[j];
+    m2[j] = SQR ? b[j] << 1 : (DZ ? 0u : dm[j]);
     lo1[j] = lo2[j] = 0;
   }
   uint32_t sa[L2 + 2], sb[L2 + 2];
@@ -69,9 +69,11 @@
       asm volatile("" : "+v"(acc2[0]) : "s"(q1));
       WV_PIN;
     }
-#pragma unroll
-    for (int j = 0; j < LPL; ++j) wv_mac(acc2[j], sa[i], m2[j]);
-    WV_PIN;
+    if constexpr (!DZ) {
+#pragma unroll
+      for (int j = 0; j < LPL; ++j) wv_mac(acc2[j], sa[i], m2[j]);
+      WV_PIN;
+    }
     if constexpr (!SQR) {
 #pragma unroll
       for (int j = 0; j < LPL; ++j) wv_mac(acc2[j], sb[i], m1[j]);
@@ -330,20 +332,38 @@
       }
     }
   };
-  uint32_t a[LPL], b[LPL], ma[LPL], mb[LPL], na[LPL], nb[LPL];
-  load_entry(a, b, 0);
+  uint32_t a[LPL], b[LPL], ma[LPL], mb[LPL], na[LPL], nb[LPL], S[LPL];
+  auto sum_beta = [&](const uint32_t (&y)[LPL]) {
+    uint32_t cy[LPL];
+#pragma unroll
+    for (int j = 0; j < LPL; ++j) {
+      S[j] += y[j];
+      cy[j] = S[j] >> LB;
+      S[j] &= c.maskv;
+    }
+    S[0] += wv_up(cy[LPL - 1]);
+#pragma unroll
+    for (int j = 1; j < LPL; ++j) S[j] += cy[j - 1];
+  };
+  load_entry(a, S, 0);
+#pragma unroll
+  for (int j = 0; j < LPL; ++j) b[j] = 0;
   if (A.nwin > 1) load_entry(ma, mb, 1);
 #pragma unroll 1
   for (int i = 1; i + 1 < A.nwin; ++i) {
     load_entry(na, nb, i + 1);
-    wvn_pairop<L2, LPL, LB, false, WIDEQ>(a, b, ma, mb, c);
+    wvn_pairop<L2, LPL, LB, false, WIDEQ, true>(a, b, ma, mb, c);
+    sum_beta(mb);
 #pragma unroll
     for (int j = 0; j < LPL; ++j) {
       ma[j] = na[j];
       mb[j] = nb[j];
     }
   }
-  if (A.nwin > 1) wvn_pairop<L2, LPL, LB, false, false>(a, b, ma, mb, c);
+  if (A.nwin > 1) {
+    wvn_pairop<L2, LPL, LB, false, false, true>(a, b, ma, mb, c);
+    sum_beta(mb);
+  }
   {
     uint32_t nt[LPL], gm[LPL], mv[LPL], u[LPL], v[LPL];
     const uint64_t* mw = A.fm_words + inst * A.fm_stride;
@@ -356,7 +376,8 @@
       if (in && sh > 64 - LB && word + 1 < A.fm_nwords) val |= mw[word + 1] << (64 - sh);
       mv[j] = (uint32_t)val & c.maskv;
     }
-    wvn_montmul_true<L2, LPL, LB>(u, mv, gm, nt, A.ctx.n0inv, c.maskv, c.onev);
+    sum_beta(mv);
+    wvn_montmul_true<L2, LPL, LB>(u, S, gm, nt, A.ctx.n0inv, c.maskv, c.onev);
     wvn_montmul_true<L2, LPL, LB>(v, u, a, nt, A.ctx.n0inv, c.maskv, c.onev);
     uint32_t cy[LPL];
 #pragma unroll
diff --git a/pailliercryptolib_amd/csrc/k_hensel.hip b/pailliercryptolib_amd/csrc/k_hensel.hip
--- a/pailliercryptolib_amd/csrc/k_hensel.hip
+++ b/pailliercryptolib_amd/csrc/k_hensel.hip
@@ -59,6 +59,13 @@
 bool PGPU_FB_NAME(launch_hensel_fb_build)(int H, int K, const HenselFbBuildArgs& a, unsigned blocks, hipStream_t s) {
   if (H == PGPU_FB_H && K == PGPU_FB_K) {
     hipLaunchKernelGGL((hensel_fb_build_kernel<PGPU_FB_H, PGPU_FB_K>), dim3(blocks), dim3(kWGThreads), 0, s, a);
+    return true;
+  }
+  return false;
+}
+bool PGPU_FB_NAME(launch_hensel_fb_unit_factor)(int H, int K, const HenselFbUnitArgs& a, unsigned blocks, hipStream_t s) {
+  if (H == PGPU_FB_H && K == PGPU_FB_K) {
+    hipLaunchKernelGGL((hensel_fb_unit_factor_kernel<PGPU_FB_H, PGPU_FB_K>), dim3(blocks), dim3(kWGThreads), 0, s, a);
     return true;
   }
   return false;
diff --git a/pailliercryptolib_amd/csrc/kargs.hpp b/pailliercryptolib_amd/csrc/kargs.hpp
--- a/pailliercryptolib_amd/csrc/kargs.hpp
+++ b/pailliercryptolib_amd/csrc/kargs.hpp
@@ -156,6 +156,20 @@
   uint32_t* table;
   int nwin;
   int w;
+  int seg_len;
+  uint32_t* prefix;
+  uint32_t* total;
+};
+
+struct HenselFbUnitArgs {
+  const uint32_t* n;
+  uint32_t n0inv;
+  uint32_t* table;
+  int nwin;
+  int w;
+  int seg_len;
+  const uint32_t* prefix;
+  const uint32_t* uinit;
 };
 
 struct HenselFullDev {
diff --git a/pailliercryptolib_amd/csrc/launch.hpp b/pailliercryptolib_amd/csrc/launch.hpp
--- a/pailliercryptolib_amd/csrc/launch.hpp
+++ b/pailliercryptolib_amd/csrc/launch.hpp
@@ -106,6 +106,10 @@
 bool launch_hensel_fb_build_part4(int H, int K, const HenselFbBuildArgs& a, unsigned blocks, hipStream_t s);
 bool launch_hensel_fb_build_part10(int H, int K, const HenselFbBuildArgs& a, unsigned blocks, hipStream_t s);
 bool launch_hensel_fb_build_part22(int H, int K, const HenselFbBuildArgs& a, unsigned blocks, hipStream_t s);
+bool launch_hensel_fb_unit_factor_part3(int H, int K, const HenselFbUnitArgs& a, unsigned blocks, hipStream_t s);
+bool launch_hensel_fb_unit_factor_part4(int H, int K, const HenselFbUnitArgs& a, unsigned blocks, hipStream_t s);
+bool launch_hensel_fb_unit_factor_part10(int H, int K, const HenselFbUnitArgs& a, unsigned blocks, hipStream_t s);
+bool launch_hensel_fb_unit_factor_part22(int H, int K, const HenselFbUnitArgs& a, unsigned blocks, hipStream_t s);
 bool launch_hensel_fb_encrypt_part22(int H, int K, const HenselFbArgs& a, unsigned blocks, hipStream_t s);
 bool launch_hensel_fb_encrypt_part3(int H, int K, const HenselFbArgs& a, unsigned blocks, hipStream_t s);
 bool launch_hensel_fb_encrypt_part4(int H, int K, const HenselFbArgs& a, unsigned blocks, hipStream_t s);
@@ -115,6 +119,14 @@
          launch_hensel_fb_build_part10(H, K, a, blocks, s)
 #if PGPU_WITH_4096
          || launch_hensel_fb_build_part22(H, K, a, blocks, s)
+#endif
+      ;
+}
+inline bool launch_hensel_fb_unit_factor(int H, int K, const HenselFbUnitArgs& a, unsigned blocks, hipStream_t s) {
+  return launch_hensel_fb_unit_factor_part3(H, K, a, blocks, s) || launch_hensel_fb_unit_factor_part4(H, K, a, blocks, s) ||
+         launch_hensel_fb_unit_factor_part10(H, K, a, blocks, s)
+#if PGPU_WITH_4096
+         || launch_hensel_fb_unit_factor_part22(H, K, a, blocks, s)
 #endif
       ;
 }
```

Result: faster. 5.958 million, median of 6 (+2.6%).
